# rust-bio/rust-bio

Measured on AMD Instinct MI355X. Metric: GCUPS (SW) + FM-index queries/sec, higher is better.
Workload: dtype int16; 1 GPU; 1000000 x 150 bp synthetic read pairs per GPU, Aligner::local affine-gap (-5,-1,+1,-1), score+coords+traceback ops (BASELINE configs[1]); pairs_per_gpu=1000000, read_len=150, parallelism=shard1

## Files before the change

include/biogpu.h:

```cpp
#ifndef BIOGPU_H
#define BIOGPU_H
#include <stdint.h>

#ifdef __cplusplus
extern "C" {
#endif

typedef enum {
    BG_OK = 0,
    BG_ERR_INVALID_ARG = -1,
    BG_ERR_NO_DEVICE = -2,
    BG_ERR_HIP = -3,
    BG_ERR_OOM = -4,
    BG_ERR_SENTINEL = -5,
    BG_ERR_POSITIVE_PENALTY = -6,
    BG_ERR_OUT_OF_ALPHABET = -7,
    BG_ERR_TOO_LARGE = -8,
    BG_ERR_OPS_CAP = -9,
    BG_ERR_TRACEBACK = -10,
    BG_ERR_UNSUPPORTED = -11,
    BG_ERR_IO = -12
} bg_status;

#define BG_MIN_SCORE (-858993459)
// ... 143 lines not shown
int bg_align_banded_batch(bg_ctx* ctx, const bg_scoring_t* sc, int mode, uint32_t k, uint32_t w,
                          uint64_t n_pairs, const uint8_t* x, const uint64_t* x_off,
                          const uint8_t* y, const uint64_t* y_off, bg_alignment_t* out,
                          uint8_t* ops_buf, uint64_t ops_cap, uint64_t* ops_used,
                          uint64_t* band_cells);

int bg_align_banded_batch_dev(bg_ctx* ctx, const bg_scoring_t* sc, int mode, uint32_t k, uint32_t w,
                              uint64_t n_pairs, const uint8_t* d_x, const uint64_t* d_x_off,
                              const uint8_t* d_y, const uint64_t* d_y_off, bg_alignment_t* d_out,
                              uint8_t* d_ops, uint64_t ops_stride, uint64_t* band_cells, void* stream);

int bg_band_create_batch(const bg_scoring_t* sc, int mode, uint32_t k, uint32_t w, uint64_t n_pairs,
                         const uint8_t* x, const uint64_t* x_off, const uint8_t* y, const uint64_t* y_off,
                         const uint64_t* band_off, uint32_t* start, uint32_t* end, uint64_t* band_cells);

int bg_align_banded_bands_batch(bg_ctx* ctx, const bg_scoring_t* sc, int mode, uint64_t n_pairs,
                                const uint8_t* x, const uint64_t* x_off, const uint8_t* y,
                                const uint64_t* y_off, const uint64_t* band_off,
                                const uint32_t* band_start, const uint32_t* band_end,
                                bg_alignment_t* out, uint8_t* ops_buf, uint64_t ops_cap,
                                uint64_t* ops_used, uint64_t* band_cells);

int bg_band_from_matches_batch(const bg_scoring_t* sc, int mode, uint32_t k, uint32_t w,
                               uint64_t n_pairs, const uint64_t* x_off, const uint64_t* y_off,
                               const uint32_t* matches_xy, const uint64_t* match_off,
                               const uint32_t* path, const uint64_t* path_off,
                               const uint64_t* band_off, uint32_t* start, uint32_t* end,
                               uint64_t* band_cells);

uint64_t bg_sparse_find_kmer_matches(const uint8_t* x, uint64_t m, const uint8_t* y, uint64_t n,
                                     uint32_t k, uint32_t* out_xy, uint64_t cap);
uint64_t bg_sparse_sdpkpp(const uint32_t* matches_xy, uint64_t n_matches, uint32_t k,
                          uint32_t match_score, int32_t gap_open, int32_t gap_extend,
                          uint32_t* path, uint64_t cap);
uint64_t bg_sparse_lcskpp(const uint32_t* matches_xy, uint64_t n_matches, uint32_t k, uint32_t* path,
                          uint64_t cap, uint32_t* score);
uint64_t bg_sparse_sdpkpp_union_lcskpp_path(const uint32_t* matches_xy, uint64_t n_matches, uint32_t k,
                                            uint32_t match_score, int32_t gap_open,
                                            int32_t gap_extend, uint32_t* path, uint64_t cap);
uint64_t bg_sparse_expand_kmer_matches(const uint8_t* x, uint64_t m, const uint8_t* y, uint64_t n,
                                       uint32_t k, const uint32_t* matches_xy, uint64_t n_matches,
                                       uint32_t allowed_mismatches, uint32_t* out_xy, uint64_t cap);

int bg_fm_set_text(bg_fm* fm, const uint8_t* text, uint64_t n);
int bg_fm_set_text_dev(bg_fm* fm, const uint8_t* d_text, uint64_t n);
typedef struct {
    uint32_t seed_len, stride;
    uint32_t max_occ;
    uint32_t pad;
} bg_seed_params_t;
typedef struct {
    bg_alignment_t aln;
    uint64_t window_start;
    uint64_t ref_start, ref_end;
    uint32_t n_candidates;
    uint32_t n_seed_hits;
} bg_seed_hit_t;
int bg_seed_extend_batch(bg_fm* fm, const bg_scoring_t* sc, const bg_seed_params_t* prm, uint64_t n_reads,
                         const uint8_t* reads, const uint64_t* read_off, bg_seed_hit_t* hits, uint8_t* ops_buf,
                         uint64_t ops_cap, uint64_t* ops_used);
int bg_seed_extend_batch_dev(bg_fm* fm, const bg_scoring_t* sc, const bg_seed_params_t* prm, uint64_t n_reads,
                             const uint8_t* d_reads, const uint64_t* d_read_off, uint32_t max_read_len,
                             bg_seed_hit_t* d_hits, uint8_t* d_ops, uint64_t ops_stride, uint64_t* totals,
                             void* stream);
enum { BG_STRAND_FORWARD = 1, BG_STRAND_REVERSE = 2, BG_STRAND_BOTH = 3 };
enum { BG_HIT_FORWARD = 0, BG_HIT_REVERSE = 1, BG_HIT_NONE = 255 };
int bg_seed_extend_strands_batch(bg_fm* fm, const bg_scoring_t* sc, const bg_seed_params_t* prm, uint32_t strands,
                                 uint64_t n_reads, const uint8_t* reads, const uint64_t* read_off, bg_seed_hit_t* hits,
                                 uint8_t* strand, uint8_t* ops_buf, uint64_t ops_cap, uint64_t* ops_used);
int bg_seed_extend_strands_batch_dev(bg_fm* fm, const bg_scoring_t* sc, const bg_seed_params_t* prm, uint32_t strands,
                                     uint64_t n_reads, const uint8_t* d_reads, const uint64_t* d_read_off,
                                     uint32_t max_read_len, bg_seed_hit_t* d_hits, uint8_t* d_strand, uint8_t* d_ops,
                                     uint64_t ops_stride, uint64_t* totals, void* stream);
typedef struct {
    uint32_t min_span, max_span;
    int32_t  pen_unpaired;
} bg_pair_params_t;
typedef struct {
    uint64_t span;
    uint32_t n_proper;
    uint8_t  proper;
    uint8_t  reserved[3];
} bg_pair_hit_t;
int bg_seed_extend_pairs_batch(bg_fm* fm, const bg_scoring_t* sc, const bg_seed_params_t* prm, const bg_pair_params_t* pp,
                               uint64_t n_pairs, const uint8_t* reads, const uint64_t* read_off, bg_seed_hit_t* hits,
                               uint8_t* strand, bg_pair_hit_t* pairs, uint8_t* ops_buf, uint64_t ops_cap, uint64_t* ops_used);
int bg_seed_extend_pairs_batch_dev(bg_fm* fm, const bg_scoring_t* sc, const bg_seed_params_t* prm, const bg_pair_params_t* pp,
                                   uint64_t n_pairs, const uint8_t* d_reads, const uint64_t* d_read_off, uint32_t max_read_len,
                                   bg_seed_hit_t* d_hits, uint8_t* d_strand, bg_pair_hit_t* d_pairs, uint8_t* d_ops,
                                   uint64_t ops_stride, uint64_t* totals, void* stream);
int bg_revcomp_batch_dev(bg_ctx* ctx, uint64_t n, const uint8_t* d_in, const uint64_t* d_off, uint8_t* d_out, void* stream);

enum { BG_FASTQ_OK = 0, BG_FASTQ_MISSING_AT = 1, BG_FASTQ_INCOMPLETE = 2, BG_FASTQ_IO = 3 };
enum { BG_FQCHECK_OK = 0, BG_FQCHECK_EMPTY_ID = 1, BG_FQCHECK_NONASCII_SEQ = 2, BG_FQCHECK_INVALID_SEQ = 3,
       BG_FQCHECK_NONASCII_QUAL = 4, BG_FQCHECK_UNEQUAL = 5 };
typedef struct {
    uint64_t id_off, desc_off;
    uint64_t seq_off, qual_off;
    uint32_t id_len, desc_len, seq_len, qual_len;
    int32_t has_desc;
    int32_t check;
} bg_fastq_record_t;
int bg_fastq_parse(bg_ctx* ctx, const uint8_t* text, uint64_t len, bg_fastq_record_t* recs, uint64_t rec_cap,
                   uint8_t* seq, uint64_t* seq_off, uint8_t* qual, uint64_t* qual_off, uint64_t* n_records,
                   int32_t* status, uint64_t* err_pos);
int bg_fastq_parse_dev(bg_ctx* ctx, const uint8_t* d_text, uint64_t len, bg_fastq_record_t* d_recs,
                       uint64_t rec_cap, uint8_t* d_seq, uint64_t* d_seq_off, uint8_t* d_qual,
                       uint64_t* d_qual_off, uint64_t* n_records, int32_t* status, uint64_t* err_pos,
                       void* stream);
int bg_cigar_batch(bg_ctx* ctx, uint64_t n, const bg_alignment_t* aln, const uint8_t* ops, uint64_t ops_bytes,
                   int hard_clip, char* out, uint64_t out_cap, uint64_t* out_off);
int bg_cigar_batch_dev(bg_ctx* ctx, uint64_t n, const bg_alignment_t* d_aln, const uint8_t* d_ops, int hard_clip,
                       char* d_out, uint64_t stride, int32_t* d_len, void* stream);

int bg_pretty_batch(bg_ctx* ctx, uint64_t n, const bg_alignment_t* aln, const uint8_t* ops, uint64_t ops_bytes,
                    const uint8_t* x, const uint64_t* x_off, const uint8_t* y, const uint64_t* y_off, uint32_t ncol,
                    char* out, uint64_t out_cap, uint64_t* out_off);

#define BG_COMM_ID_BYTES 128
typedef struct bg_comm bg_comm;
int bg_shard_range(uint64_t n_units, int rank, int world, uint64_t* lo, uint64_t* hi);
int bg_shard_balanced(const uint64_t* costs, uint64_t n, int world, uint64_t* bounds);
int bg_comm_unique_id(uint8_t* id );
int bg_comm_init(bg_ctx* ctx, int rank, int world, const uint8_t* id , bg_comm** out);
int bg_comm_init_host(bg_ctx* ctx, int rank, int world, const char* name, bg_comm** out);
int bg_gather_records(bg_comm* comm, const void* local, uint64_t n_local, uint32_t rec_bytes, void* all, uint64_t* counts_out,
                      void* stream);
int bg_gather_records_cap(bg_comm* comm, const void* local, uint64_t n_local, uint32_t rec_bytes, void* all, uint64_t all_cap,
                          uint64_t* counts_out, void* stream);
int bg_gather_records_host(bg_comm* comm, const void* local, uint64_t n_local, uint32_t rec_bytes, void* all, uint64_t all_cap,
                           uint64_t* counts_out);
int bg_comm_world(bg_comm* comm, int64_t* info);
int bg_comm_free(bg_comm* comm);

typedef struct {
    float fill_ms, traceback_ms, fm_ms;
    uint32_t fill_launches, traceback_launches, fm_launches;
} bg_timing_t;
int bg_get_timing(bg_ctx* ctx, bg_timing_t* out);
int bg_band_redo_pairs(bg_ctx* ctx, uint64_t* out);
enum {
    BG_FILL_K1_WIDE = 0x1,
    BG_FILL_K1_NARROW = 0x2,
    BG_FILL_K1_LF = 0x4,
    BG_FILL_K1P = 0x8,
    BG_FILL_K1P_LF = 0x10,
    BG_FILL_K3 = 0x20,
    BG_FILL_K3V2_WIDE = 0x40,
    BG_FILL_K3V2_NARROW = 0x80,
    BG_FILL_K3I = 0x100,
    BG_FILL_K3P = 0x200
};
int bg_last_fill_kernels(bg_ctx* ctx, uint32_t* mask);
int bg_enable_timing(bg_ctx* ctx, int on);

#ifdef __cplusplus
}
#endif
#endif
```

rust-bio_amd/_lib.py:

```python
import ctypes as C
import os
import subprocess

import numpy as np

_HERE = os.path.dirname(os.path.abspath(__file__))
SO_PATH = os.path.join(_HERE, "libbiogpu.so")
CSRC = os.path.join(_HERE, "csrc")

BG_OK = 0
ERRORS = {-1: "INVALID_ARG", -2: "NO_DEVICE", -3: "HIP", -4: "OOM", -5: "SENTINEL",
          -6: "POSITIVE_PENALTY", -7: "OUT_OF_ALPHABET", -8: "TOO_LARGE", -9: "OPS_CAP",
          -10: "TRACEBACK", -11: "UNSUPPORTED", -12: "IO"}
MIN_SCORE = -858993459
STRAND_FORWARD, STRAND_REVERSE, STRAND_BOTH = 1, 2, 3
HIT_FORWARD, HIT_REVERSE, HIT_NONE = 0, 1, 255
FILL = {"K1_WIDE": 0x1, "K1_NARROW": 0x2, "K1_LF": 0x4, "K1P": 0x8, "K1P_LF": 0x10, "K3": 0x20, "K3V2_WIDE": 0x40,
        "K3V2_NARROW": 0x80, "K3I": 0x100, "K3P": 0x200}


class BiogpuError(RuntimeError):
    def __init__(self, status, where=""):
        self.status = status
        msg = lib().bg_strerror(status).decode()
        last = lib().bg_last_error().decode()
        super().__init__(f"{where}: {ERRORS.get(status, status)}: {msg}" + (f" [{last}]" if last else ""))


class SentinelError(BiogpuError, ValueError):
    """suffix_array.rs:431-437 assert"""


class PenaltyError(BiogpuError, AssertionError):
    """pairwise/mod.rs:265-266,554-571 asserts"""


class AlphabetError(BiogpuError, IndexError):
    """fmindex.rs:229 / bwt.rs:158 index out of bounds"""


_EXC = {-5: SentinelError, -6: PenaltyError, -7: AlphabetError}


def check(status, where=""):
    if status != BG_OK:
        raise _EXC.get(status, BiogpuError)(status, where)


class ScoringC(C.Structure):
    _fields_ = [("gap_open", C.c_int32), ("gap_extend", C.c_int32),
                ("xclip_prefix", C.c_int32), ("xclip_suffix", C.c_int32),
                ("yclip_prefix", C.c_int32), ("yclip_suffix", C.c_int32),
                ("match_score", C.c_int32), ("mismatch_score", C.c_int32),
                ("match_scores_some", C.c_int32),
                ("matrix", C.POINTER(C.c_int32))]


class TimingC(C.Structure):
    _fields_ = [("fill_ms", C.c_float), ("traceback_ms", C.c_float), ("fm_ms", C.c_float),
                ("fill_launches", C.c_uint32), ("traceback_launches", C.c_uint32),
                ("fm_launches", C.c_uint32)]


ALN_DTYPE = np.dtype([("score", "<i4"), ("xstart", "<u4"), ("xend", "<u4"), ("ystart", "<u4"),
                      ("yend", "<u4"), ("xlen", "<u4"), ("ylen", "<u4"), ("n_ops", "<u4"),
                      ("ops_off", "<u8"), ("clip_len", "<u4", (4,)), ("n_clips", "u1"),
                      ("mode", "u1"), ("status", "i1"), ("_pad", "u1"), ("_tail", "<u4")])
assert ALN_DTYPE.itemsize == 64, ALN_DTYPE.itemsize
SEED_HIT_DTYPE = np.dtype([("aln", ALN_DTYPE), ("window_start", "<u8"), ("ref_start", "<u8"), ("ref_end", "<u8"),
                           ("n_candidates", "<u4"), ("n_seed_hits", "<u4")])
assert SEED_HIT_DTYPE.itemsize == 96, SEED_HIT_DTYPE.itemsize


class SeedParamsC(C.Structure):
    _fields_ = [("seed_len", C.c_uint32), ("stride", C.c_uint32), ("max_occ", C.c_uint32), ("pad", C.c_uint32)]


class PAIR_PARAMS(C.Structure):
    _fields_ = [("min_span", C.c_uint32), ("max_span", C.c_uint32), ("pen_unpaired", C.c_int32)]


assert C.sizeof(PAIR_PARAMS) == 12, C.sizeof(PAIR_PARAMS)
PAIR_HIT_DTYPE = np.dtype([("span", "<u8"), ("n_proper", "<u4"), ("proper", "u1"), ("reserved", "u1", (3,))])
assert PAIR_HIT_DTYPE.itemsize == 16, PAIR_HIT_DTYPE.itemsize


FQREC_DTYPE = np.dtype([("id_off", "<u8"), ("desc_off", "<u8"), ("seq_off", "<u8"), ("qual_off", "<u8"),
                        ("id_len", "<u4"), ("desc_len", "<u4"), ("seq_len", "<u4"), ("qual_len", "<u4"),
                        ("has_desc", "<i4"), ("check", "<i4")])
assert FQREC_DTYPE.itemsize == 56, FQREC_DTYPE.itemsize

SYMBOLS = ["bg_device_count", "bg_init", "bg_free", "bg_strerror", "bg_last_error",
           "bg_set_option", "bg_suffix_array", "bg_bwt", "bg_less", "bg_fm_build", "bg_fm_free",
           "bg_fm_device_bytes", "bg_fm_set_option", "bg_fm_backward_search_batch", "bg_fm_backward_search_batch_dev",
           "bg_fm_set_suffix_array", "bg_fm_set_sampled_suffix_array", "bg_sa_get_batch", "bg_sa_get_batch_dev",
           "bg_interval_occ_batch", "bg_interval_occ_batch_dev", "bg_fmd_smems_batch", "bg_fmd_smems_batch_dev", "bg_fmd_interval_batch",
           "bg_align_batch", "bg_align_batch_dev", "bg_align_banded_batch", "bg_align_banded_batch_dev", "bg_band_create_batch",
           "bg_align_banded_bands_batch", "bg_band_from_matches_batch", "bg_sparse_find_kmer_matches", "bg_sparse_sdpkpp",
           "bg_sparse_lcskpp", "bg_sparse_sdpkpp_union_lcskpp_path", "bg_sparse_expand_kmer_matches", "bg_fastq_parse",
           "bg_fastq_parse_dev", "bg_cigar_batch", "bg_cigar_batch_dev", "bg_get_timing", "bg_enable_timing", "bg_band_redo_pairs", "bg_last_fill_kernels", "bg_pack2_host",
           "bg_pretty_batch", "bg_suffix_array_dev", "bg_bwt_dev", "bg_sa_sample_dev", "bg_suffix_array_dev64", "bg_bwt_dev64", "bg_sa_sample_dev64", "bg_fm_build_dev", "bg_fm_set_text", "bg_fm_set_text_dev", "bg_seed_extend_batch", "bg_seed_extend_batch_dev",
           "bg_seed_extend_strands_batch", "bg_seed_extend_strands_batch_dev", "bg_revcomp_batch_dev",
           "bg_seed_extend_pairs_batch", "bg_seed_extend_pairs_batch_dev",
           "bg_pack2_dev", "bg_unpack2_dev", "bg_fm_pattern_codes", "bg_fm_backward_search_packed_dev",
           "bg_fm_backward_search_count_lines_dev", "bg_align_batch_packed_dev", "bg_fm_step2_bytes",
           "bg_shard_range", "bg_shard_balanced", "bg_comm_unique_id", "bg_comm_init", "bg_comm_init_host",
           "bg_gather_records", "bg_gather_records_cap", "bg_gather_records_host", "bg_comm_free", "bg_fm_save", "bg_fm_load",
           "bg_fm_len", "bg_fm_less", "bg_fm_bwt", "bg_fm_bwt_dev", "bg_comm_world",
           "bg_fmd_smems_batch64", "bg_fmd_smems_batch64_dev", "bg_fmd_interval_batch64"]


def build(force=False):
    if force:
        subprocess.check_call(["make", "-C", CSRC, "clean", "-s"])
    subprocess.check_call(["make", "-C", CSRC, "-j8", "-s"])
    return SO_PATH


_lib = None


def lib():
    global _lib
    if _lib is None:
        if not os.path.exists(SO_PATH):
            raise RuntimeError(f"{SO_PATH} is missing: run `python -c 'import __graft_entry__ as g; "
                               "g.build()'` (the engine has no CPU fallback)")
        L = C.CDLL(SO_PATH)
        vp, u64, u32, i32 = C.c_void_p, C.c_uint64, C.c_uint32, C.c_int
        L.bg_strerror.restype = C.c_char_p
        L.bg_strerror.argtypes = [i32]
        L.bg_last_error.restype = C.c_char_p
        L.bg_device_count.restype = i32
        L.bg_init.argtypes = [i32, C.POINTER(vp)]
        L.bg_free.argtypes = [vp]
        L.bg_set_option.argtypes = [vp, C.c_char_p, C.c_int64]
        L.bg_suffix_array.argtypes = [vp, u64, vp]
        L.bg_bwt.argtypes = [vp, vp, u64, vp]
        L.bg_less.argtypes = [vp, u64, vp, u32, vp, C.POINTER(u32)]
        L.bg_fm_build.argtypes = [vp, vp, u64, vp, u32, u32, vp, u32, C.POINTER(vp)]
        L.bg_fm_free.argtypes = [vp]
        L.bg_fm_save.argtypes = [vp, C.c_char_p]
        L.bg_fm_load.argtypes = [vp, C.c_char_p, C.POINTER(vp)]
        L.bg_fm_len.argtypes = [vp, C.POINTER(u64)]
        L.bg_fm_less.argtypes = [vp, vp, C.POINTER(u32)]
        L.bg_fm_bwt.argtypes = [vp, vp]
        L.bg_fm_bwt_dev.argtypes = [vp, vp, vp]
        L.bg_fm_build_dev.argtypes = [vp, vp, u64, u32, vp, u32, vp, C.POINTER(vp), vp]
        L.bg_fm_set_option.argtypes = [vp, C.c_char_p, C.c_int64]
        L.bg_fm_device_bytes.restype = u64
        L.bg_fm_device_bytes.argtypes = [vp]
        L.bg_fm_step2_bytes.restype = u64
        L.bg_fm_step2_bytes.argtypes = [vp]
        L.bg_shard_range.argtypes = [u64, i32, i32, C.POINTER(u64), C.POINTER(u64)]
        L.bg_shard_balanced.argtypes = [vp, u64, i32, vp]
        L.bg_comm_unique_id.argtypes = [vp]
        L.bg_comm_init.argtypes = [vp, i32, i32, vp, C.POINTER(vp)]
        L.bg_comm_init_host.argtypes = [vp, i32, i32, C.c_char_p, C.POINTER(vp)]
        L.bg_gather_records.argtypes = [vp, vp, u64, u32, vp, vp, vp]
        L.bg_gather_records_cap.argtypes = [vp, vp, u64, u32, vp, u64, vp, vp]
        L.bg_gather_records_host.argtypes = [vp, vp, u64, u32, vp, u64, vp]
        L.bg_comm_free.argtypes = [vp]
        L.bg_comm_world.argtypes = [vp, vp]
        L.bg_fm_backward_search_batch.argtypes = [vp, u64, vp, vp, vp, vp, vp, vp]
        L.bg_fm_backward_search_batch_dev.argtypes = [vp, u64, vp, vp, vp, vp, vp, vp, vp]
        L.bg_fmd_interval_batch.argtypes = [vp, u64, vp, vp, vp, vp]
        L.bg_fmd_smems_batch.argtypes = [vp, i32, u64, vp, vp, vp, u32, u32, vp, vp]
        L.bg_fmd_smems_batch_dev.argtypes = [vp, i32, u64, vp, vp, vp, u32, u32, u32, vp, vp, vp]
        L.bg_fmd_interval_batch64.argtypes = [vp, u64, vp, vp, vp, vp]
        L.bg_fmd_smems_batch64.argtypes = [vp, i32, u64, vp, vp, vp, u32, u32, vp, vp]
        L.bg_fmd_smems_batch64_dev.argtypes = [vp, i32, u64, vp, vp, vp, u32, u32, u32, vp, vp, vp]
        L.bg_fm_set_suffix_array.argtypes = [vp, vp, u64]
        L.bg_fm_set_sampled_suffix_array.argtypes = [vp, vp, u64, u32, C.c_uint8, vp, vp, u64]
        L.bg_sa_get_batch.argtypes = [vp, u64, vp, vp]
        L.bg_fastq_parse.argtypes = [vp, vp, u64, vp, u64, vp, vp, vp, vp, C.POINTER(u64), C.POINTER(i32), C.POINTER(u64)]
        L.bg_fastq_parse_dev.argtypes = [vp, vp, u64, vp, u64, vp, vp, vp, vp, C.POINTER(u64), C.POINTER(i32), C.POINTER(u64), vp]
        L.bg_cigar_batch.argtypes = [vp, u64, vp, vp, u64, i32, vp, u64, vp]
        L.bg_cigar_batch_dev.argtypes = [vp, u64, vp, vp, i32, vp, u64, vp, vp]
        L.bg_sa_get_batch_dev.argtypes = [vp, u64, vp, vp, vp]
        L.bg_interval_occ_batch.argtypes = [vp, u64, vp, vp, vp, vp, u64]
        L.bg_interval_occ_batch_dev.argtypes = [vp, u64, vp, vp, u64, vp, vp]
        L.bg_align_batch.argtypes = [vp, C.POINTER(ScoringC), i32, u64, vp, vp, vp, vp, vp, vp,
                                     u64, C.POINTER(u64)]
        L.bg_align_batch_dev.argtypes = [vp, C.POINTER(ScoringC), i32, u64, vp, vp, vp, vp, u32,
                                         u32, vp, vp, u64, vp]
        L.bg_align_banded_batch.argtypes = [vp, C.POINTER(ScoringC), i32, u32, u32, u64, vp, vp,
                                            vp, vp, vp, vp, u64, C.POINTER(u64), vp]
        L.bg_align_banded_batch_dev.argtypes = [vp, C.POINTER(ScoringC), i32, u32, u32, u64, vp, vp, vp, vp, vp, vp, u64, vp, vp]
        L.bg_band_create_batch.argtypes = [C.POINTER(ScoringC), i32, u32, u32, u64, vp, vp, vp, vp, vp, vp, vp, vp]
        L.bg_align_banded_bands_batch.argtypes = [vp, C.POINTER(ScoringC), i32, u64, vp, vp, vp, vp, vp, vp, vp, vp, vp,
                                                  u64, C.POINTER(u64), vp]
        L.bg_band_from_matches_batch.argtypes = [C.POINTER(ScoringC), i32, u32, u32, u64, vp, vp, vp, vp, vp, vp, vp, vp,
                                                 vp, vp]
        for name, args in [("bg_sparse_find_kmer_matches", [vp, u64, vp, u64, u32, vp, u64]),
                           ("bg_sparse_sdpkpp", [vp, u64, u32, u32, C.c_int32, C.c_int32, vp, u64]),
                           ("bg_sparse_lcskpp", [vp, u64, u32, vp, u64, C.POINTER(u32)]),
                           ("bg_sparse_sdpkpp_union_lcskpp_path", [vp, u64, u32, u32, C.c_int32, C.c_int32, vp, u64]),
                           ("bg_sparse_expand_kmer_matches", [vp, u64, vp, u64, u32, vp, u64, u32, vp, u64])]:
            getattr(L, name).restype = u64
            getattr(L, name).argtypes = args
        L.bg_pretty_batch.argtypes = [vp, u64, vp, vp, u64, vp, vp, vp, vp, u32, vp, u64, vp]
        L.bg_suffix_array_dev.argtypes = [vp, vp, u64, vp, vp]
        L.bg_bwt_dev.argtypes = [vp, vp, vp, u64, vp, vp]
        L.bg_sa_sample_dev.argtypes = [vp, vp, vp, u64, u32, C.c_uint8, vp, vp, vp, u64, C.POINTER(u64), vp]
        L.bg_suffix_array_dev64.argtypes = [vp, vp, u64, vp, vp]
        L.bg_bwt_dev64.argtypes = [vp, vp, vp, u64, vp, vp]
        L.bg_sa_sample_dev64.argtypes = [vp, vp, vp, u64, u32, C.c_uint8, vp, vp, vp, u64, C.POINTER(u64), vp]
        L.bg_fm_set_text.argtypes = [vp, vp, u64]
        L.bg_fm_set_text_dev.argtypes = [vp, vp, u64]
        L.bg_seed_extend_batch.argtypes = [vp, C.POINTER(ScoringC), C.POINTER(SeedParamsC), u64, vp, vp, vp, vp, u64, C.POINTER(u64)]
        L.bg_seed_extend_batch_dev.argtypes = [vp, C.POINTER(ScoringC), C.POINTER(SeedParamsC), u64, vp, vp, u32, vp, vp, u64, vp, vp]
        L.bg_seed_extend_strands_batch.argtypes = [vp, C.POINTER(ScoringC), C.POINTER(SeedParamsC), u32, u64, vp, vp, vp, vp, vp, u64,
                                                   C.POINTER(u64)]
        L.bg_seed_extend_strands_batch_dev.argtypes = [vp, C.POINTER(ScoringC), C.POINTER(SeedParamsC), u32, u64, vp, vp, u32, vp, vp,
                                                       vp, u64, vp, vp]
        L.bg_seed_extend_pairs_batch.argtypes = [vp, C.POINTER(ScoringC), C.POINTER(SeedParamsC), C.POINTER(PAIR_PARAMS), u64, vp, vp, vp,
                                                 vp, vp, vp, u64, C.POINTER(u64)]
        L.bg_seed_extend_pairs_batch_dev.argtypes = [vp, C.POINTER(ScoringC), C.POINTER(SeedParamsC), C.POINTER(PAIR_PARAMS), u64, vp, vp,
                                                     u32, vp, vp, vp, vp, u64, vp, vp]
        L.bg_revcomp_batch_dev.argtypes = [vp, u64, vp, vp, vp, vp]
        L.bg_pack2_dev.argtypes = [vp, vp, u64, vp, vp, vp, vp]
        L.bg_unpack2_dev.argtypes = [vp, vp, u64, vp, vp, vp]
        L.bg_fm_pattern_codes.argtypes = [vp, vp]
        L.bg_fm_backward_search_packed_dev.argtypes = [vp, u64, vp, vp, vp, vp, vp, vp, vp]
        L.bg_fm_backward_search_count_lines_dev.argtypes = [vp, u64, vp, vp, vp, vp, vp, vp, C.POINTER(u64), vp]
        L.bg_align_batch_packed_dev.argtypes = [vp, C.POINTER(ScoringC), i32, u64, vp, vp, vp, vp, vp, u32, u32, vp, vp, u64, vp]
        L.bg_get_timing.argtypes = [vp, C.POINTER(TimingC)]
        L.bg_enable_timing.argtypes = [vp, i32]
        L.bg_band_redo_pairs.argtypes = [vp, C.POINTER(u64)]
        L.bg_last_fill_kernels.argtypes = [vp, C.POINTER(u32)]
        L.bg_pack2_host.argtypes = [vp, u64, vp, vp]
        for s in SYMBOLS:
            if getattr(L, s).restype is C.c_int or s.startswith("bg_") and getattr(L, s).restype is None:
                pass
        _lib = L
    return _lib


class Context:

    def __init__(self, device=0):
        self.h = C.c_void_p()
        check(lib().bg_init(device, C.byref(self.h)), "bg_init")
        self.device = device

    def set_option(self, key, value):
        check(lib().bg_set_option(self.h, key.encode(), int(value)), "bg_set_option")

    def enable_timing(self, on=True):
        check(lib().bg_enable_timing(self.h, 1 if on else 0))

    def timing(self):
        t = TimingC()
        check(lib().bg_get_timing(self.h, C.byref(t)))
        return {k: getattr(t, k) for k, _ in TimingC._fields_}

    def band_redo_pairs(self):
        v = C.c_uint64(0)
        check(lib().bg_band_redo_pairs(self.h, C.byref(v)))
        return int(v.value)

    def last_fill_kernels(self):
        v = C.c_uint32(0)
        check(lib().bg_last_fill_kernels(self.h, C.byref(v)))
        return int(v.value)

    def close(self):
        if self.h:
            lib().bg_free(self.h)
            self.h = C.c_void_p()

    def __del__(self):
        try:
            self.close()
        except Exception:
            pass


_default_ctx = {}


def default_context(device=None):
    if device is None:
        device = int(os.environ.get("LOCAL_RANK", "0")) if lib().bg_device_count() > 1 else 0
    if device not in _default_ctx:
        _default_ctx[device] = Context(device)
    return _default_ctx[device]


def as_u8(b):
    if isinstance(b, np.ndarray):
        return np.ascontiguousarray(b, dtype=np.uint8)
    return np.frombuffer(bytes(b), dtype=np.uint8)


def concat(seqs):
    off = np.zeros(len(seqs) + 1, dtype=np.uint64)
    if seqs:
        off[1:] = np.cumsum([len(s) for s in seqs], dtype=np.uint64)
    buf = np.frombuffer(b"".join(bytes(s) for s in seqs), dtype=np.uint8)
    return buf, off
```

rust-bio_amd/csrc/banded_api.hip:

```cpp
#include <algorithm>
#include <atomic>
#include <functional>
#include <thread>

#include "band_host.h"
#include <sched.h>

#include <chrono>

#include "band_device.h"
#include "banded_kernels.h"

using namespace bgband_dev;

int bg_compact_matrix(const int32_t* matrix, std::vector<uint8_t>& code_map, std::vector<int32_t>& table);

namespace bgband { extern std::atomic<uint64_t> g_prof[4]; }
namespace {

constexpr uint64_t kMaxCells = 5000000;

struct HostPair {
    uint32_t m = 0, n = 0, flags = BP_OK;
    uint32_t start_0 = 0, end_0 = 0, start_n = 0, end_n = 0;
// ... 107 lines not shown
        size_t dc_pairs = 0, dc_rowc = 0, dc_roff = 0, dc_tb = 0, dc_aux = 0;
        hipEvent_t copied = nullptr, filled = nullptr, traced = nullptr, built = nullptr, matched = nullptr;
        bool built_valid = false;
        hipEvent_t fill_gone = nullptr;
        hipEvent_t pre_done = nullptr;
        hipEvent_t cleared = nullptr;
        bool busy = false;
    } set[2];
    void* db[2][17] = {};
    size_t db_cap[2][17] = {};
    hipStream_t build_stream = nullptr;
    hipEvent_t seq_ready = nullptr;
    void* h_state = nullptr;
    size_t h_state_cap = 0;
    void* io[6] = {};
    size_t io_cap[6] = {};
    void* h_ops = nullptr;
    size_t h_ops_cap = 0;
    void *d_cmp = nullptr, *d_cscan = nullptr;
    size_t d_cmp_cap = 0, d_cscan_cap = 0;
    uint64_t* d_cell = nullptr;
    uint64_t* d_dlslot = nullptr;
    hipStream_t dl_stream = nullptr;
    static constexpr uint64_t kDlSlots = 1024;
    hipStream_t tb_stream = nullptr;
    hipStream_t aux_stream = nullptr;
    hipStream_t copy_stream = nullptr;
    uint32_t* d_started = nullptr;
    uint32_t started_target = 0;
};

extern "C" int bg_band_redo_pairs(bg_ctx* ctx, uint64_t* out) {
    if (!ctx || !out) return BG_ERR_INVALID_ARG;
    *out = 0;
    if (!ctx->band || !ctx->band->d_started) return BG_OK;
    BG_HIP(hipSetDevice(ctx->device));
    BG_HIP(hipDeviceSynchronize());
    uint32_t v = 0;
    BG_HIP(hipMemcpy(&v, ctx->band->d_started + 1, 4, hipMemcpyDeviceToHost));
    *out = v;
    return BG_OK;
}

void bg_band_scratch_free(bg_band_scratch* b) {
    if (!b) return;
    for (auto& s : b->set) {
        hipHostFree(s.h_pairs); hipHostFree(s.h_rowc); hipHostFree(s.h_roff);
        hipFree(s.d_pairs); hipFree(s.d_rowc); hipFree(s.d_roff); hipFree(s.d_tb); hipFree(s.d_aux);
        hipFree(b->d_started);
        b->d_started = nullptr;
        if (s.copied) hipEventDestroy(s.copied);
        if (s.filled) hipEventDestroy(s.filled);
        if (s.traced) hipEventDestroy(s.traced);
        if (s.built) hipEventDestroy(s.built);
        if (s.matched) hipEventDestroy(s.matched);
        if (s.fill_gone) hipEventDestroy(s.fill_gone);
        if (s.pre_done) hipEventDestroy(s.pre_done);
        if (s.cleared) hipEventDestroy(s.cleared);
    }
    for (void* p : b->io) hipFree(p);
    hipFree(b->d_cmp);
    hipFree(b->d_cscan);
    hipFree(b->d_cell);
    hipFree(b->d_dlslot);
    if (b->dl_stream) hipStreamDestroy(b->dl_stream);
    for (auto& set : b->db)
        for (void* p : set) hipFree(p);
    hipHostFree(b->h_state);
    hipHostFree(b->h_ops);
    if (b->tb_stream) hipStreamDestroy(b->tb_stream);
    if (b->aux_stream) hipStreamDestroy(b->aux_stream);
    if (b->copy_stream) hipStreamDestroy(b->copy_stream);
    if (b->build_stream) hipStreamDestroy(b->build_stream);
    if (b->seq_ready) hipEventDestroy(b->seq_ready);
    delete b;
}

namespace {

template <typename F>
void parallel_for(uint64_t n, uint64_t grain, F&& fn) {
    unsigned nt = host_threads();
    nt = (unsigned)std::min<uint64_t>(nt, std::max<uint64_t>(1, n / grain));
    if (nt <= 1) {
        fn(0, 0, n);
        return;
    }
    std::atomic<uint64_t> next{0};
    bg_pool_run(nt, [&](unsigned t) {
        for (;;) {
            const uint64_t lo = next.fetch_add(grain);
            if (lo >= n) break;
            fn(t, lo, std::min<uint64_t>(n, lo + grain));
        }
    });
}

int check_scoring(const bg_scoring_t* sc) {
    if (sc->gap_open > 0 || sc->gap_extend > 0 || sc->xclip_prefix > 0 || sc->xclip_suffix > 0 ||
        sc->yclip_prefix > 0 || sc->yclip_suffix > 0)
        return BG_ERR_POSITIVE_PENALTY;
    return BG_OK;
}

}

extern "C" int bg_band_create_batch(const bg_scoring_t* sc, int mode, uint32_t k, uint32_t w, uint64_t n_pairs,
                                    const uint8_t* x, const uint64_t* x_off, const uint8_t* y, const uint64_t* y_off,
                                    const uint64_t* band_off, uint32_t* start, uint32_t* end, uint64_t* band_cells) {
    if (!sc || !x_off || !y_off || (n_pairs && (!band_off || !start || !end))) return BG_ERR_INVALID_ARG;
    int rc = check_scoring(sc);
    if (rc) return rc;
    const bgband::ClipScores cs = clip_scores(sc, mode);
    parallel_for(n_pairs, 4, [&](unsigned, uint64_t lo, uint64_t hi) {
        bgband::Band band;
        bgband::Workspace ws;
        for (uint64_t p = lo; p < hi; p++) {
            const uint32_t m = (uint32_t)(x_off[p + 1] - x_off[p]), n = (uint32_t)(y_off[p + 1] - y_off[p]);
            band.create(x + x_off[p], m, y + y_off[p], n, k, w, cs, ws);
            memcpy(start + band_off[p], band.start.data(), (size_t)(n + 1) * 4);
            memcpy(end + band_off[p], band.end.data(), (size_t)(n + 1) * 4);
            if (band_cells) band_cells[p] = band.num_cells();
        }
    });
    if (getenv("BG_TRACE")) fprintf(stderr, "[bg banded] cpu-ms: kmers %.1f sdp %.1f band %.1f (threads %u)\n", bgband::g_prof[0] / 1e6, bgband::g_prof[1] / 1e6, bgband::g_prof[2] / 1e6, host_threads());
    return BG_OK;
}

using BandMaker = std::function<bool(uint64_t, bgband::Band&, bgband::Workspace&)>;

int band_stream_create(hipStream_t* s, int level) {
    int lo = 0, hi = 0;
    if (level == 0 || hipDeviceGetStreamPriorityRange(&lo, &hi) != hipSuccess || lo == hi)
        return hipStreamCreateWithFlags(s, hipStreamNonBlocking) == hipSuccess ? BG_OK : BG_ERR_HIP;
    return hipStreamCreateWithPriority(s, hipStreamNonBlocking, level > 0 ? hi : lo) == hipSuccess ? BG_OK : BG_ERR_HIP;
}

struct BandDevIO {
    const uint8_t* d_x;
    const uint64_t* d_xo;
    const uint8_t* d_y;
    const uint64_t* d_yo;
    bg_alignment_t* d_out;
    uint8_t* d_ops;
    uint64_t ops_stride;
};

static int banded_batch_impl(bg_ctx* ctx, const bg_scoring_t* sc, int mode, uint64_t n_pairs, const uint8_t* x,
                             const uint64_t* x_off, const uint8_t* y, const uint64_t* y_off, bg_alignment_t* out,
                             uint8_t* ops_buf, uint64_t ops_cap, uint64_t* ops_used, uint64_t* band_cells,
                             const BandMaker& make_band, const uint32_t* dev_kw = nullptr, const BandDevIO* dio = nullptr) {
    if (!ctx || !sc || mode < BG_MODE_CUSTOM || mode > BG_MODE_LOCAL) return BG_ERR_INVALID_ARG;
    ctx->fill_mask = 0;
    int rc = check_scoring(sc);
    if (rc) return rc;
    if (ops_used) *ops_used = 0;
    if (n_pairs == 0) return BG_OK;
    if (!x_off || !y_off || (!out && !dio)) return BG_ERR_INVALID_ARG;
    BG_HIP(hipSetDevice(ctx->device));
    hipStream_t st = ctx->stream;
    if (!ctx->band) {
        ctx->band = new bg_band_scratch;
        BG_HIP(hipStreamCreateWithFlags(&ctx->band->tb_stream, hipStreamNonBlocking));
        for (auto& s : ctx->band->set) {
            BG_HIP(hipEventCreateWithFlags(&s.copied, hipEventDisableTiming));
            BG_HIP(hipEventCreateWithFlags(&s.filled, hipEventDisableTiming));
            BG_HIP(hipEventCreateWithFlags(&s.traced, hipEventDisableTiming));
        }
    }
    bg_band_scratch& B = *ctx->band;
    hipStream_t st_tb = B.tb_stream;

    const bgband::ClipScores cs = clip_scores(sc, mode);
    uint64_t max_x = 0, max_y = 0;
    for (uint64_t p = 0; p < n_pairs; p++) {
        max_x = std::max(max_x, x_off[p + 1] - x_off[p]);
        max_y = std::max(max_y, y_off[p + 1] - y_off[p]);
    }
    if (max_x > (1u << 24) || max_y > (1u << 24)) return BG_ERR_TOO_LARGE;
    const uint64_t stride = dio ? dio->ops_stride : ((max_x + max_y + 4 + 3) & ~3ull);
    if (dio && dio->d_ops && stride < max_x + max_y + 4) return BG_ERR_OPS_CAP;

    BandArgs a = {};
    a.sc = {cs.gap_open, cs.gap_extend, cs.xclip_prefix, cs.xclip_suffix, cs.yclip_prefix, cs.yclip_suffix,
            sc->match_score, sc->mismatch_score};
    a.mode = mode;
    a.filter_clips = (mode == BG_MODE_SEMIGLOBAL || mode == BG_MODE_LOCAL);
    a.ops_stride = stride;
    int sm = SCORE_PARAMS;
    std::vector<uint8_t> code_map;
    std::vector<int32_t> table;
    if (sc->matrix) {
        const int A = bg_compact_matrix(sc->matrix, code_map, table);
        sm = A <= kMaxLdsAlphabet ? SCORE_LDS : SCORE_GLOBAL;
        if ((rc = bg_reserve(&ctx->table, &ctx->table_bytes, 256 + table.size() * 4))) return rc;
        BG_HIP(hipMemcpy((uint8_t*)ctx->table + 256, table.data(), table.size() * 4, hipMemcpyHostToDevice));
        BG_HIP(hipMemcpy(ctx->table, code_map.data(), 256, hipMemcpyHostToDevice));
        a.code_map = (const uint8_t*)ctx->table;
        a.table = (const int32_t*)((uint8_t*)ctx->table + 256);
        a.alpha = A;
    }
    band_fill_fn fill = get_band_fill(sm);
    const int64_t mag = std::max<int64_t>({std::abs((int64_t)cs.gap_open), std::abs((int64_t)cs.gap_extend),
                                           std::abs((int64_t)sc->match_score), std::abs((int64_t)sc->mismatch_score), 1});
    auto clip_ok = [](int32_t c) { return c <= kNarrowNegClip || c >= -(1 << 22); };
    const bool narrow = !ctx->force_wide && mag * ((int64_t)max_x + (int64_t)max_y + 8) < (1 << 24) && clip_ok(cs.xclip_prefix) &&
                        clip_ok(cs.xclip_suffix) && clip_ok(cs.yclip_prefix) && clip_ok(cs.yclip_suffix);

    const bool trace = getenv("BG_TRACE") != nullptr;
    auto now = []() { return std::chrono::steady_clock::now(); };
    auto t_last = now();
    auto lap = [&](const char* what) {
        if (!trace) return;
        const auto t1 = now();
        fprintf(stderr, "[bg banded] %-18s %8.2f ms\n", what, std::chrono::duration<double, std::milli>(t1 - t_last).count());
        t_last = t1;
    };

    const uint64_t xb = x_off[n_pairs], yb = y_off[n_pairs];
    const uint8_t *d_x, *d_y;
    const uint64_t *d_xo, *d_yo;
    uint8_t* d_ops;
    bg_alignment_t* d_out;
    if (dio) {
        d_x = dio->d_x;
        d_y = dio->d_y;
        d_xo = dio->d_xo;
        d_yo = dio->d_yo;
        d_out = dio->d_out;
        d_ops = dio->d_ops;
    } else {
        const size_t io_need[6] = {std::max<uint64_t>(xb, 16), std::max<uint64_t>(yb, 16), (n_pairs + 1) * 8, (n_pairs + 1) * 8,
                                   n_pairs * sizeof(bg_alignment_t), ops_buf ? n_pairs * stride : 16};
        for (int i = 0; i < 6; i++)
            if ((rc = bg_reserve(&B.io[i], &B.io_cap[i], io_need[i]))) return rc;
        d_x = (uint8_t*)B.io[0];
        d_y = (uint8_t*)B.io[1];
        d_ops = ops_buf ? (uint8_t*)B.io[5] : nullptr;
        d_xo = (uint64_t*)B.io[2];
        d_yo = (uint64_t*)B.io[3];
        d_out = (bg_alignment_t*)B.io[4];
        BG_HIP(hipMemcpyAsync((void*)d_xo, x_off, (n_pairs + 1) * 8, hipMemcpyHostToDevice, st));
        BG_HIP(hipMemcpyAsync((void*)d_yo, y_off, (n_pairs + 1) * 8, hipMemcpyHostToDevice, st));
    }
    a.x = d_x;
    a.x_off = d_xo;
    a.y = d_y;
    a.y_off = d_yo;
    a.out = d_out;
    a.ops = d_ops;
    lap("h2d sequences");
    const bool compact_on_device = !dio && ops_buf != nullptr;
    if (compact_on_device) {
        if ((rc = bg_reserve(&B.d_cmp, &B.d_cmp_cap, xb + yb + 4 * n_pairs + 256))) return rc;
        if ((rc = bg_reserve(&B.d_cscan, &B.d_cscan_cap,
                             bg_compact_ops_scratch(std::min<uint64_t>(n_pairs, ctx->chunk_pairs > 0 ? (uint64_t)ctx->chunk_pairs : 16384)))))
            return rc;
        if (!B.d_cell) BG_HIP(hipMalloc((void**)&B.d_cell, 64));
        BG_HIP(hipMemsetAsync(B.d_cell, 0, 8, st));
        if ((rc = pinned_reserve(&B.h_ops, &B.h_ops_cap, xb + yb + 4 * n_pairs + 256))) return rc;
        if (!B.d_dlslot) BG_HIP(hipMalloc((void**)&B.d_dlslot, bg_band_scratch::kDlSlots * 16));
        if (!B.dl_stream) {
            int lo = 0, hi = 0;
            BG_HIP(hipDeviceGetStreamPriorityRange(&lo, &hi));
            BG_HIP(hipStreamCreateWithPriority(&B.dl_stream, hipStreamNonBlocking, hi));
        }
    }

    const uint64_t chunk_pairs = ctx->chunk_pairs > 0 ? (uint64_t)ctx->chunk_pairs : 16384;
    struct SliceEvents {
        std::vector<hipEvent_t> ev;
        ~SliceEvents() {
            for (hipEvent_t e : ev)
                if (e) hipEventDestroy(e);
        }
    } slices;
    const uint64_t n_slices = dio ? 0 : (n_pairs + chunk_pairs - 1) / chunk_pairs;
    uint64_t slices_up = 0, waited_fill = 0;
    if (n_slices && !B.copy_stream && (rc = band_stream_create(&B.copy_stream, -1))) return rc;
    auto upload_slices = [&](uint64_t upto) -> int {
        for (; slices_up < std::min(upto, n_slices); slices_up++) {
            const uint64_t q0 = slices_up * chunk_pairs, q1 = std::min(n_pairs, q0 + chunk_pairs);
            if (slices_up == 0) {
                hipEvent_t e0;
                BG_HIP(hipEventCreateWithFlags(&e0, hipEventDisableTiming));
                slices.ev.push_back(e0);
                BG_HIP(hipEventRecord(e0, st));
                BG_HIP(hipStreamWaitEvent(B.copy_stream, e0, 0));
            }
            if (x_off[q1] > x_off[q0])
                BG_HIP(bg_copy_pieces((uint8_t*)d_x + x_off[q0], x + x_off[q0], x_off[q1] - x_off[q0], hipMemcpyHostToDevice, B.copy_stream));
            if (y_off[q1] > y_off[q0])
                BG_HIP(bg_copy_pieces((uint8_t*)d_y + y_off[q0], y + y_off[q0], y_off[q1] - y_off[q0], hipMemcpyHostToDevice, B.copy_stream));
            hipEvent_t e;
            BG_HIP(hipEventCreateWithFlags(&e, hipEventDisableTiming));
            slices.ev.push_back(e);
            BG_HIP(hipEventRecord(e, B.copy_stream));
        }
        return BG_OK;
    };
    auto need_seq = [&](hipStream_t s, uint64_t& waited, uint64_t upto) -> int {
        if (!n_slices) return BG_OK;
        const uint64_t k1 = std::min(n_slices, (upto + chunk_pairs - 1) / chunk_pairs);
        int rcu = upload_slices(k1);
        if (rcu) return rcu;
        for (; waited < k1; waited++) BG_HIP(hipStreamWaitEvent(s, slices.ev[waited + 1], 0));
// ... 589 lines not shown
```

rust-bio_amd/csrc/bg_common.h:

```cpp
#ifndef BG_COMMON_H
#define BG_COMMON_H
#include <functional>
#include <hip/hip_runtime.h>

#include <cstdint>
#include <cstdlib>
#include <cstdio>
#include <cstring>
#include <string>
#include <vector>

#include "biogpu.h"

extern thread_local std::string bg_tls_error;

#define BG_HIP(call)                                                                     \
    do {                                                                                 \
        hipError_t e__ = (call);                                                         \
        if (e__ != hipSuccess) {                                                         \
            bg_tls_error = std::string(#call) + ": " + hipGetErrorString(e__);           \
            return e__ == hipErrorOutOfMemory ? BG_ERR_OOM : BG_ERR_HIP;                 \
        }                                                                                \
    } while (0)

struct bg_band_scratch;
void bg_band_scratch_free(bg_band_scratch*);
struct bg_seed_scratch;
void bg_seed_scratch_free(bg_seed_scratch*);
struct bg_host_pipe;
void bg_host_pipe_free(bg_host_pipe*);
struct bg_fm_pipe;
void bg_fm_pipe_free(bg_fm_pipe*);

struct bg_ctx {
    int device = 0;
    hipStream_t stream = nullptr;
    void* tb = nullptr;
    size_t tb_bytes = 0;
    void* aux = nullptr;
    size_t aux_bytes = 0;
    void* bnd = nullptr;
    size_t bnd_bytes = 0;
    void* io[6] = {};
    size_t io_cap[6] = {};
    void* h_ops = nullptr;
    size_t h_ops_cap = 0;
    void* unpk[2] = {};
    size_t unpk_cap[2] = {};
    void* table = nullptr;
    size_t table_bytes = 0;
    void* sw_table = nullptr;
    size_t sw_table_bytes = 0;
    uint64_t table_hash = 0;
    int table_alpha = 0;
    int32_t* table_matrix = nullptr;
    bg_band_scratch* band = nullptr;
    bg_host_pipe* pipe = nullptr;
    bg_seed_scratch* seed = nullptr;
    bg_fm_pipe* fm_pipe = nullptr;
    uint64_t fm_wide_from = 0xFFFFFFFFull;
    uint32_t fm_wide_sb_shift = 17;
    bool fm_host_bytes = false;
    int64_t host_chunk_pairs = 0;
    int64_t chunk_pairs = 0;
    int64_t seed_chunk_reads = 0;
    bool force_wide = false;
    bool no_pk16 = false;
    bool no_local_fast = false;
    bool no_couples = false;
    int band_chain_global = -1;
    bool fq_no_fused = false;
    int64_t sa_chunk_symbols = 0;
    bool band_chain_rows = true;
    bool band_join_global = false;
    int band_fill_v1 = 0;
    bool band_interior_off = false;
    bool band_packed_off = false;
    int64_t band_packed_thresh = 0;
    int64_t band_budget_gb = 0;
    bool band_on_host = false;
    hipEvent_t scratch_done = nullptr;
    hipStream_t scratch_stream = nullptr;
    bool scratch_used = false;
    bool timing = false;
    hipEvent_t ev[2] = {nullptr, nullptr};
    bg_timing_t last = {};
    uint32_t fill_mask = 0;
};

int bg_reserve(void** p, size_t* cur, size_t need);
int bg_scan_u32(const uint32_t* d_len, uint64_t n, uint64_t* d_off, uint64_t* d_sums, hipStream_t st);
int bg_align_batch_dev_hint(bg_ctx* ctx, const bg_scoring_t* sc, int mode, uint64_t n_pairs, const uint8_t* d_x,
                            const uint64_t* d_x_off, const uint8_t* d_y, const uint64_t* d_y_off, uint32_t max_xlen,
                            uint32_t max_ylen, bg_alignment_t* d_out, uint8_t* d_ops, uint64_t ops_stride, void* stream,
                            int len_hint);

size_t bg_compact_ops_scratch(uint64_t n);
int bg_range_to_host(const uint8_t* d_src, uint8_t* h_dst, const uint64_t* d_slot , hipStream_t st);
int bg_compact_ops_dev(bg_alignment_t* d_rec, uint64_t n, const uint8_t* d_ops, uint8_t* d_compact, bool global_offsets, uint64_t* d_cell,
                       uint64_t* d_batch_total, void* d_scratch, bool long_ops, hipStream_t st);

struct bg_scratch_guard {
    bg_ctx* ctx;
    hipStream_t st;
    bg_scratch_guard(bg_ctx* c, hipStream_t s) : ctx(c), st(s) {
        if (ctx->scratch_used && ctx->scratch_stream != st) hipStreamWaitEvent(st, ctx->scratch_done, 0);
    }
    ~bg_scratch_guard() {
        if (hipEventRecord(ctx->scratch_done, st) == hipSuccess) {
            ctx->scratch_stream = st;
            ctx->scratch_used = true;
        }
    }
};
inline hipError_t bg_copy_pieces(void* dst, const void* src, size_t bytes, hipMemcpyKind kind, hipStream_t st) {
    static const size_t piece = [] {
        const char* e = getenv("BG_COPY_PIECE");
        const long long v = e ? atoll(e) : 0;
        return v > 0 ? (size_t)v : (size_t)(8u << 20);
    }();
    for (size_t o = 0; o < bytes; o += piece) {
        const hipError_t rc = hipMemcpyAsync((uint8_t*)dst + o, (const uint8_t*)src + o, bytes - o < piece ? bytes - o : piece, kind, st);
        if (rc != hipSuccess) return rc;
    }
    return hipSuccess;
}
unsigned bg_host_threads();
namespace bgpack {
bool pack2_host(const uint8_t* src, uint64_t n, const uint8_t codes[4], uint32_t* dst);
}
void bg_pool_run(unsigned nt, const std::function<void(unsigned)>& fn);

__device__ __forceinline__ int wave_shr1(int v, int old = 0) {
    return __builtin_amdgcn_update_dpp(old, v, 0x138 , 0xf, 0xf, false);
}
__device__ __forceinline__ int wave_shl1(int v, int old = 0) {
    return __builtin_amdgcn_update_dpp(old, v, 0x130 , 0xf, 0xf, false);
}
__device__ __forceinline__ int wave_shr1z(int v) { return __builtin_amdgcn_update_dpp(0, v, 0x138, 0xf, 0xf, true); }
__device__ __forceinline__ int wave_shl1z(int v) { return __builtin_amdgcn_update_dpp(0, v, 0x130, 0xf, 0xf, true); }
__device__ __forceinline__ unsigned quad_sum(unsigned v) {
    v += (unsigned)__builtin_amdgcn_update_dpp(0, (int)v, 0xB1 , 0xf, 0xf, true);
    v += (unsigned)__builtin_amdgcn_update_dpp(0, (int)v, 0x4E , 0xf, 0xf, true);
    return v;
}

#endif
```

rust-bio_amd/csrc/core.hip:

```cpp
#include <sched.h>

#include <algorithm>
#include <condition_variable>
#include <deque>
#include <mutex>
#include <thread>

#include <cstdlib>

#include "bg_common.h"

thread_local std::string bg_tls_error;

int bg_reserve(void** p, size_t* cur, size_t need) {
    if (need <= *cur) return BG_OK;
    if (*p) {
        hipFree(*p);
        *p = nullptr;
        *cur = 0;
    }
    need = (need + 255) & ~(size_t)255;
    BG_HIP(hipMalloc(p, need));
    *cur = need;
    return BG_OK;
// ... 85 lines not shown
    hipDeviceProp_t prop;
    BG_HIP(hipGetDeviceProperties(&prop, device));
    if (std::string(prop.gcnArchName).rfind("gfx950", 0) != 0) {
        bg_tls_error = std::string("device is ") + prop.gcnArchName + ", library is built for gfx950";
        return BG_ERR_NO_DEVICE;
    }
    bg_ctx* ctx = new bg_ctx;
    ctx->device = device;
    if (const char* e = getenv("BG_BAND_FILL_V1")) ctx->band_fill_v1 = atoi(e) > 0 ? 1 : atoi(e) < 0 ? -1 : 0;
    {
        int lo = 0, hi = 0;
        const char* e = getenv("BG_STREAM_PRIO");
        if ((!e || atoi(e) != 0) && hipDeviceGetStreamPriorityRange(&lo, &hi) == hipSuccess && hi != lo)
            BG_HIP(hipStreamCreateWithPriority(&ctx->stream, hipStreamNonBlocking, hi));
        else
            BG_HIP(hipStreamCreateWithFlags(&ctx->stream, hipStreamNonBlocking));
    }
    BG_HIP(hipEventCreate(&ctx->ev[0]));
    BG_HIP(hipEventCreate(&ctx->ev[1]));
    BG_HIP(hipEventCreateWithFlags(&ctx->scratch_done, hipEventDisableTiming));
    *out = ctx;
    return BG_OK;
}

extern "C" int bg_free(bg_ctx* ctx) {
    if (!ctx) return BG_OK;
    hipSetDevice(ctx->device);
    hipFree(ctx->tb);
    hipFree(ctx->aux);
    hipFree(ctx->bnd);
    hipFree(ctx->table);
    hipFree(ctx->sw_table);
    free(ctx->table_matrix);
    hipFree(ctx->unpk[0]);
    hipFree(ctx->unpk[1]);
    for (void* p : ctx->io) hipFree(p);
    if (ctx->h_ops) hipHostFree(ctx->h_ops);
    bg_band_scratch_free(ctx->band);
    bg_host_pipe_free(ctx->pipe);
    bg_seed_scratch_free(ctx->seed);
    bg_fm_pipe_free(ctx->fm_pipe);
    if (ctx->ev[0]) hipEventDestroy(ctx->ev[0]);
    if (ctx->ev[1]) hipEventDestroy(ctx->ev[1]);
    if (ctx->scratch_done) hipEventDestroy(ctx->scratch_done);
    if (ctx->stream) hipStreamDestroy(ctx->stream);
    delete ctx;
    return BG_OK;
}

extern "C" const char* bg_strerror(int s) {
    switch (s) {
        case BG_OK: return "ok";
        case BG_ERR_INVALID_ARG: return "invalid argument";
        case BG_ERR_NO_DEVICE: return "no usable gfx950 device";
        case BG_ERR_HIP: return "HIP runtime error";
        case BG_ERR_OOM: return "out of device memory";
        case BG_ERR_SENTINEL:
            return "Expecting extra sentinel symbol being lexicographically smallest at the end of the text.";
        case BG_ERR_POSITIVE_PENALTY: return "gap/clip penalty can't be positive";
        case BG_ERR_OUT_OF_ALPHABET: return "symbol outside the alphabet (index out of bounds in the reference)";
        case BG_ERR_TOO_LARGE: return "input too large for the engine";
        case BG_ERR_OPS_CAP: return "operations buffer too small";
        case BG_ERR_TRACEBACK: return "traceback did not terminate";
        case BG_ERR_UNSUPPORTED: return "not supported by the device layout";
        case BG_ERR_IO: return "index file cannot be opened, is truncated or fails its checksum";
        default: return "unknown status";
    }
}

extern "C" const char* bg_last_error(void) { return bg_tls_error.c_str(); }

extern "C" int bg_set_option(bg_ctx* ctx, const char* key, int64_t value) {
    if (!ctx || !key) return BG_ERR_INVALID_ARG;
    if (!strcmp(key, "chunk_pairs")) {
        ctx->chunk_pairs = value;
        return BG_OK;
    }
    if (!strcmp(key, "seed_chunk_reads")) {
        ctx->seed_chunk_reads = value;
        return BG_OK;
    }
    if (!strcmp(key, "band_join_global")) {
        ctx->band_join_global = value != 0;
        return BG_OK;
    }
    if (!strcmp(key, "fm_wide_from")) {
        ctx->fm_wide_from = value > 0 ? (uint64_t)value : 0xFFFFFFFFull;
        return BG_OK;
    }
    if (!strcmp(key, "fm_wide_sb_shift")) {
        if (value < 0 || value > 24) return BG_ERR_INVALID_ARG;
        ctx->fm_wide_sb_shift = (uint32_t)value;
        return BG_OK;
    }
    if (!strcmp(key, "fq_no_fused")) {
        ctx->fq_no_fused = value != 0;
        return BG_OK;
    }
    if (!strcmp(key, "sa_chunk_symbols")) {
        if (value < 0) return BG_ERR_INVALID_ARG;
        ctx->sa_chunk_symbols = value;
        return BG_OK;
    }
    if (!strcmp(key, "band_chain_rows")) {
        ctx->band_chain_rows = value != 0;
        return BG_OK;
    }
    if (!strcmp(key, "band_chain_global")) {
        ctx->band_chain_global = (int)value;
        return BG_OK;
    }
    if (!strcmp(key, "band_fill_v1")) {
        ctx->band_fill_v1 = value > 0 ? 1 : value < 0 ? -1 : 0;
        return BG_OK;
    }
    if (!strcmp(key, "band_interior_off")) {
        ctx->band_interior_off = value != 0;
        return BG_OK;
    }
    if (!strcmp(key, "band_packed_off")) {
        ctx->band_packed_off = value != 0;
        return BG_OK;
    }
    if (!strcmp(key, "band_packed_thresh")) {
        if (value < 0 || value > 0xffff) return BG_ERR_INVALID_ARG;
        ctx->band_packed_thresh = value;
        return BG_OK;
    }
    if (!strcmp(key, "band_budget_gb")) {
        if (value < 0 || value > 256) return BG_ERR_INVALID_ARG;
        ctx->band_budget_gb = value;
        return BG_OK;
    }
    if (!strcmp(key, "band_on_host")) {
        ctx->band_on_host = value != 0;
        return BG_OK;
    }
    if (!strcmp(key, "fm_host_bytes")) {
        ctx->fm_host_bytes = value != 0;
        return BG_OK;
    }
    if (!strcmp(key, "host_chunk_pairs")) {
        ctx->host_chunk_pairs = value;
        return BG_OK;
    }
    if (!strcmp(key, "no_couples")) {
        ctx->no_couples = value != 0;
        return BG_OK;
    }
    if (!strcmp(key, "no_local_fast")) {
        ctx->no_local_fast = value != 0;
        return BG_OK;
    }
    if (!strcmp(key, "no_pk16")) {
        ctx->no_pk16 = value != 0;
        return BG_OK;
    }
    if (!strcmp(key, "force_wide")) {
        ctx->force_wide = value != 0;
        return BG_OK;
    }
    return BG_ERR_INVALID_ARG;
}

extern "C" int bg_enable_timing(bg_ctx* ctx, int on) {
    if (!ctx) return BG_ERR_INVALID_ARG;
    ctx->timing = on != 0;
    ctx->last = {};
    return BG_OK;
}

extern "C" int bg_last_fill_kernels(bg_ctx* ctx, uint32_t* mask) {
    if (!ctx || !mask) return BG_ERR_INVALID_ARG;
    *mask = ctx->fill_mask;
    return BG_OK;
}

extern "C" int bg_get_timing(bg_ctx* ctx, bg_timing_t* out) {
    if (!ctx || !out) return BG_ERR_INVALID_ARG;
    *out = ctx->last;
    ctx->last = {};
    return BG_OK;
}

namespace {
__global__ __launch_bounds__(256) void ops_counts_kernel(const bg_alignment_t* __restrict__ rec, uint64_t n, uint32_t* __restrict__ cnt) {
    const uint64_t p = (uint64_t)blockIdx.x * blockDim.x + threadIdx.x;
    if (p < n) cnt[p] = rec[p].status == BG_OK ? rec[p].n_ops : 0u;
}
template <int LANES>
__global__ __launch_bounds__(256) void ops_compact_kernel(bg_alignment_t* __restrict__ rec, uint64_t n, const uint8_t* __restrict__ ops,
                                                          const uint64_t* __restrict__ off, const uint64_t* __restrict__ cell,
                                                          uint8_t* __restrict__ compact, int global_offsets) {
    const uint64_t p = ((uint64_t)blockIdx.x * blockDim.x + threadIdx.x) / LANES;
    const uint32_t l = threadIdx.x % LANES;
    if (p >= n) return;
    const uint32_t k = rec[p].status == BG_OK ? rec[p].n_ops : 0u;
    const uint64_t base = *cell;
    const uint8_t* src = ops + rec[p].ops_off;
    uint8_t* dst = compact + (global_offsets ? base : 0ull) + off[p];
    for (uint32_t i = l; i < k; i += LANES) dst[i] = src[i];
    if (l == 0) rec[p].ops_off = base + off[p];
}
__global__ void ops_advance_kernel(uint64_t* cell, const uint64_t* __restrict__ off, uint64_t n, uint64_t* __restrict__ batch_total) {
    if (batch_total) *batch_total = off[n];
    cell[0] += off[n];
}
inline size_t a256(size_t v) { return (v + 255) & ~(size_t)255; }
}

typedef uint32_t bg_u32x4 __attribute__((ext_vector_type(4)));
__global__ __launch_bounds__(256) void range_to_host_kernel(const uint8_t* __restrict__ d_src, uint8_t* __restrict__ h_dst,
                                                            const uint64_t* __restrict__ slot) {
    const uint64_t end = slot[1], start = end - slot[0];
    const uint64_t a = start >> 4, b = (end + 15) >> 4;
    const bg_u32x4* src = (const bg_u32x4*)d_src;
    bg_u32x4* dst = (bg_u32x4*)h_dst;
    for (uint64_t i = a + (uint64_t)blockIdx.x * 256 + threadIdx.x; i < b; i += (uint64_t)gridDim.x * 256)
        __builtin_nontemporal_store(src[i], &dst[i]);
}
int bg_range_to_host(const uint8_t* d_src, uint8_t* h_dst, const uint64_t* d_slot, hipStream_t st) {
    range_to_host_kernel<<<dim3(8), dim3(256), 0, st>>>(d_src, h_dst, d_slot);
    BG_HIP(hipGetLastError());
    return BG_OK;
}

size_t bg_compact_ops_scratch(uint64_t n) { return a256(n * 4) + a256((n + 1) * 8) + 2 * (n / 2048 + 2) * 8 + 256; }

int bg_compact_ops_dev(bg_alignment_t* d_rec, uint64_t n, const uint8_t* d_ops, uint8_t* d_compact, bool global_offsets, uint64_t* d_cell,
                       uint64_t* d_batch_total, void* d_scratch, bool long_ops, hipStream_t st) {
    if (n == 0) {
        if (d_batch_total) BG_HIP(hipMemsetAsync(d_batch_total, 0, 8, st));
        return BG_OK;
    }
    uint32_t* d_cnt = (uint32_t*)d_scratch;
    uint64_t* d_off = (uint64_t*)((uint8_t*)d_scratch + a256(n * 4));
    uint64_t* d_sums = (uint64_t*)((uint8_t*)d_off + a256((n + 1) * 8));
    ops_counts_kernel<<<dim3((unsigned)((n + 255) / 256)), dim3(256), 0, st>>>(d_rec, n, d_cnt);
    int rc = bg_scan_u32(d_cnt, n, d_off, d_sums, st);
    if (rc) return rc;
    if (long_ops)
        ops_compact_kernel<64><<<dim3((unsigned)((n * 64 + 255) / 256)), dim3(256), 0, st>>>(d_rec, n, d_ops, d_off, d_cell, d_compact, global_offsets);
    else
        ops_compact_kernel<16><<<dim3((unsigned)((n * 16 + 255) / 256)), dim3(256), 0, st>>>(d_rec, n, d_ops, d_off, d_cell, d_compact, global_offsets);
    ops_advance_kernel<<<dim3(1), dim3(1), 0, st>>>(d_cell, d_off, n, d_batch_total);
    BG_HIP(hipGetLastError());
    return BG_OK;
}
```

rust-bio_amd/csrc/sw_api.hip:

```cpp
#include <algorithm>
#include <chrono>
#include <map>
#include <type_traits>

#include <atomic>
#include <condition_variable>
#include <mutex>
#include <thread>

#include "sw_kernels.h"

namespace bgsw {
sw_fill_fn get_fill_params_narrow(int lp, int r, bool local);
sw_fill_fn get_fill_params_wide(int lp, int r, bool local);
sw_fill_fn get_fill_params_lf(int lp, int r);
sw_fill_fn get_fill_matrix(int lp, int r, int sm, bool narrow, bool local);
sw_fill_fn get_fill_pk16_local(int lp, int r, int which);
sw_fill_fn get_fill_pk16_localfast(int lp, int r, int which);
sw_fill_fn get_fill_pk16_semiglobal(int lp, int r, int which);
sw_fill_fn get_fill_pk16_global(int lp, int r, int which);
sw_fill_fn get_fill_pk16_custom(int lp, int r, int which);
void launch_traceback(const SwArgs& a, int nw, hipStream_t st);

struct Config {
    int lp, r;
};
static Config pick_config(uint32_t m_cap, int sm) {
    if (sm == SCORE_PARAMS) {
        if (m_cap <= 192) return {16, std::max(2, 2 * (int)((m_cap + 31) / 32))};
        if (m_cap <= 384) return {32, std::max(8, 2 * (int)((m_cap + 63) / 64))};
        return {64, 8};
    }
    if (m_cap <= 96) return {16, 6};
    if (m_cap <= 128) return {16, 8};
    if (m_cap <= 160) return {16, 10};
    if (m_cap <= 192) return {16, 12};
    if (m_cap <= 384) return {32, 12};
    return {64, 8};
}

static int compact_matrix(const int32_t* matrix, std::vector<uint8_t>& code_map,
                          std::vector<int32_t>& table) {
    std::map<std::vector<int32_t>, int> classes;
    code_map.assign(256, 0);
    std::vector<int> rep;
    for (int b = 0; b < 256; b++) {
        std::vector<int32_t> sig(512);
        for (int c = 0; c < 256; c++) {
            sig[c] = matrix[b * 256 + c];
            sig[256 + c] = matrix[c * 256 + b];
        }
        auto it = classes.find(sig);
        if (it == classes.end()) {
            it = classes.emplace(std::move(sig), (int)rep.size()).first;
            rep.push_back(b);
        }
        code_map[b] = (uint8_t)it->second;
    }
    const int A = (int)rep.size();
    table.assign((size_t)A * A, 0);
    for (int p = 0; p < A; p++)
        for (int q = 0; q < A; q++) table[(size_t)p * A + q] = matrix[rep[p] * 256 + rep[q]];
    return A;
}
}

namespace bgsw {
constexpr uint32_t kLenKeys = 1u << 20;
__global__ __launch_bounds__(256) void sw_len_stats_kernel(const uint64_t* __restrict__ x_off, const uint64_t* __restrict__ y_off, uint64_t pair0,
                                                           uint32_t n, uint32_t* __restrict__ st ) {
    uint32_t m = 0, nn = 0, m_lo = ~0u, n_lo = ~0u;
    for (uint32_t p = blockIdx.x * blockDim.x + threadIdx.x; p < n; p += gridDim.x * blockDim.x) {
        const uint32_t a = (uint32_t)(x_off[pair0 + p + 1] - x_off[pair0 + p]), b = (uint32_t)(y_off[pair0 + p + 1] - y_off[pair0 + p]);
        m = max(m, a);
        m_lo = min(m_lo, a);
        nn = max(nn, b);
        n_lo = min(n_lo, b);
    }
#pragma unroll
    for (int o = 32; o; o >>= 1) {
        m = max(m, (uint32_t)__shfl_xor((int)m, o));
        nn = max(nn, (uint32_t)__shfl_xor((int)nn, o));
        m_lo = min(m_lo, (uint32_t)__shfl_xor((int)m_lo, o));
        n_lo = min(n_lo, (uint32_t)__shfl_xor((int)n_lo, o));
    }
    __shared__ uint32_t s[4][4];
    if ((threadIdx.x & 63) == 0) {
        s[threadIdx.x >> 6][0] = m_lo;
        s[threadIdx.x >> 6][1] = m;
        s[threadIdx.x >> 6][2] = n_lo;
        s[threadIdx.x >> 6][3] = nn;
    }
    __syncthreads();
    if (threadIdx.x == 0) {
        atomicMin(&st[0], min(min(s[0][0], s[1][0]), min(s[2][0], s[3][0])));
        atomicMax(&st[2], max(max(s[0][1], s[1][1]), max(s[2][1], s[3][1])));
        atomicMin(&st[1], min(min(s[0][2], s[1][2]), min(s[2][2], s[3][2])));
        atomicMax(&st[3], max(max(s[0][3], s[1][3]), max(s[2][3], s[3][3])));
    }
}
__device__ __forceinline__ uint32_t len_key(const uint64_t* x_off, const uint64_t* y_off, uint64_t r) {
    const uint32_t m = (uint32_t)(x_off[r + 1] - x_off[r]), n = (uint32_t)(y_off[r + 1] - y_off[r]);
    return min(m, 511u) << 11 | min(n, 2047u);
}
__device__ __forceinline__ uint32_t wave_key_add(uint32_t* counter, uint32_t key, bool valid, uint32_t& base) {
    const int lane = threadIdx.x & 63;
    uint32_t rank = 0;
    base = 0;
    uint64_t todo = __ballot(valid);
    while (todo) {
        const int leader = __ffsll((long long)todo) - 1;
        const uint32_t k = (uint32_t)__shfl((int)key, leader);
        const uint64_t same = __ballot(valid && key == k) & todo;
        uint32_t b = 0;
        if (lane == leader) b = atomicAdd(&counter[k], (uint32_t)__popcll(same));
        b = (uint32_t)__shfl((int)b, leader);
        if (valid && key == k) {
            base = b;
            rank = (uint32_t)__popcll(same & ((1ull << lane) - 1));
        }
        todo &= ~same;
    }
    return rank;
}
__global__ __launch_bounds__(256) void sw_key_hist_kernel(const uint64_t* __restrict__ x_off, const uint64_t* __restrict__ y_off, uint64_t pair0,
                                                          uint32_t n, uint32_t* __restrict__ cnt, const uint32_t* __restrict__ st) {
    if (st && st[0] == st[2] && st[1] == st[3]) return;
    const uint32_t p = blockIdx.x * blockDim.x + threadIdx.x;
    const bool valid = p < n;
    uint32_t base;
    wave_key_add(cnt, valid ? len_key(x_off, y_off, pair0 + p) : 0u, valid, base);
}
__global__ __launch_bounds__(256) void sw_key_block_sums_kernel(const uint32_t* __restrict__ cnt, uint32_t* __restrict__ sums,
                                                                const uint32_t* __restrict__ st) {
    if (st && st[0] == st[2] && st[1] == st[3]) return;
    uint32_t v = 0;
    for (int i = 0; i < 4; i++) v += cnt[blockIdx.x * 1024u + i * 256u + threadIdx.x];
    __shared__ uint32_t s[4];
#pragma unroll
    for (int o = 32; o; o >>= 1) v += __shfl_xor(v, o);
    if ((threadIdx.x & 63) == 0) s[threadIdx.x >> 6] = v;
    __syncthreads();
    if (threadIdx.x == 0) sums[blockIdx.x] = s[0] + s[1] + s[2] + s[3];
}
__global__ __launch_bounds__(1024) void sw_key_scan_kernel(uint32_t* __restrict__ cnt, const uint32_t* __restrict__ sums,
                                                           const uint32_t* __restrict__ st) {
    if (st && st[0] == st[2] && st[1] == st[3]) return;
    __shared__ uint32_t s[1024];
    s[threadIdx.x] = sums[threadIdx.x];
    __syncthreads();
    for (int o = 1; o < 1024; o <<= 1) {
        const uint32_t u = threadIdx.x >= (unsigned)o ? s[threadIdx.x - o] : 0;
        __syncthreads();
        s[threadIdx.x] += u;
        __syncthreads();
    }
    const uint32_t base = blockIdx.x ? s[blockIdx.x - 1] : 0;
    __syncthreads();
    const uint32_t v = cnt[blockIdx.x * 1024u + threadIdx.x];
    s[threadIdx.x] = v;
    __syncthreads();
    for (int o = 1; o < 1024; o <<= 1) {
        const uint32_t u = threadIdx.x >= (unsigned)o ? s[threadIdx.x - o] : 0;
        __syncthreads();
        s[threadIdx.x] += u;
        __syncthreads();
    }
    cnt[blockIdx.x * 1024u + threadIdx.x] = base + s[threadIdx.x] - v;
}
__global__ __launch_bounds__(256) void sw_key_scatter_kernel(const uint64_t* __restrict__ x_off, const uint64_t* __restrict__ y_off, uint64_t pair0,
                                                             uint32_t n, uint32_t* __restrict__ cursor, uint32_t* __restrict__ perm,
                                                             const uint32_t* __restrict__ st) {
    if (st && st[0] == st[2] && st[1] == st[3]) return;
    const uint32_t p = blockIdx.x * blockDim.x + threadIdx.x;
    const bool valid = p < n;
    uint32_t base;
    const uint32_t rank = wave_key_add(cursor, valid ? len_key(x_off, y_off, pair0 + p) : 0u, valid, base);
    if (valid) perm[base + rank] = p;
}
__global__ void sw_decide_kernel(const uint32_t* __restrict__ st, uint32_t n, int forced, uint32_t* __restrict__ n_eff) {
    const bool uniform = forced < 0 && st[0] == st[2] && st[1] == st[3];
    n_eff[0] = uniform ? n : 0u;
    n_eff[1] = uniform ? 0u : n;
}
}

using namespace bgsw;

int bg_compact_matrix(const int32_t* matrix, std::vector<uint8_t>& code_map, std::vector<int32_t>& table) {
    return compact_matrix(matrix, code_map, table);
}

static int check_scoring(const bg_scoring_t* sc) {
    if (sc->gap_open > 0 || sc->gap_extend > 0 || sc->xclip_prefix > 0 || sc->xclip_suffix > 0 ||
        sc->yclip_prefix > 0 || sc->yclip_suffix > 0)
        return BG_ERR_POSITIVE_PENALTY;
    return BG_OK;
}

static int align_batch_dev_impl(bg_ctx* ctx, const bg_scoring_t* sc, int mode, uint64_t n_pairs,
                                const uint8_t* d_x, const uint64_t* d_x_off, const uint8_t* d_y,
                                const uint64_t* d_y_off, uint32_t max_xlen, uint32_t max_ylen,
                                bg_alignment_t* d_out, uint8_t* d_ops, uint64_t ops_stride,
                                void* stream, int len_hint, const uint8_t* packed_codes = nullptr) {
    if (!ctx || !sc || mode < BG_MODE_CUSTOM || mode > BG_MODE_LOCAL) return BG_ERR_INVALID_ARG;
    int rc = check_scoring(sc);
    if (rc) return rc;
    if (n_pairs == 0) return BG_OK;
    if (!d_x_off || !d_y_off || !d_out) return BG_ERR_INVALID_ARG;
    if (d_ops && ops_stride < (uint64_t)max_xlen + max_ylen + 4) return BG_ERR_OPS_CAP;
    if (max_xlen > (1u << 24) || max_ylen > (1u << 24)) return BG_ERR_TOO_LARGE;
    hipStream_t st = (hipStream_t)stream;
    BG_HIP(hipSetDevice(ctx->device));
    bg_scratch_guard guard(ctx, st);

    SwArgs a = {};
    a.x = d_x;
    a.x_off = d_x_off;
    a.y = d_y;
    a.y_off = d_y_off;
    a.sc = {sc->gap_open,     sc->gap_extend,   sc->xclip_prefix, sc->xclip_suffix,
            sc->yclip_prefix, sc->yclip_suffix, sc->match_score,  sc->mismatch_score};
    if (mode == BG_MODE_GLOBAL) a.sc.xp = a.sc.xs = a.sc.yp = a.sc.ys = BG_MIN_SCORE;
    if (mode == BG_MODE_SEMIGLOBAL) {
        a.sc.xp = a.sc.xs = BG_MIN_SCORE;
        a.sc.yp = a.sc.ys = 0;
    }
    if (mode == BG_MODE_LOCAL) a.sc.xp = a.sc.xs = a.sc.yp = a.sc.ys = 0;
    a.mode = mode;
    a.filter_clips = (mode == BG_MODE_SEMIGLOBAL || mode == BG_MODE_LOCAL);
    a.out = d_out;
    a.ops = d_ops;
    a.ops_stride = ops_stride;

    int sm = SCORE_PARAMS;
    if (sc->matrix) {
        uint64_t h = 0xcbf29ce484222325ull;
        {
            const uint64_t* w = (const uint64_t*)sc->matrix;
            uint64_t h2 = 0x9e3779b97f4a7c15ull;
            for (size_t t = 0; t < 32768; t += 2) {
                h = (h ^ w[t]) * 0x100000001b3ull;
                h2 = (h2 + w[t + 1]) * 0xff51afd7ed558ccdull;
                h2 ^= h2 >> 32;
            }
            h ^= h2;
            if (h == 0) h = 1;
        }
        if (ctx->table_hash != h || !ctx->table_matrix || memcmp(ctx->table_matrix, sc->matrix, 65536 * sizeof(int32_t)) != 0) {
            std::vector<uint8_t> code_map;
            std::vector<int32_t> table;
            const int A = compact_matrix(sc->matrix, code_map, table);
            const size_t bytes = 256 + table.size() * 4;
            ctx->table_hash = 0;
            if (!ctx->table_matrix && !(ctx->table_matrix = (int32_t*)malloc(65536 * sizeof(int32_t)))) return BG_ERR_OOM;
            if ((rc = bg_reserve(&ctx->sw_table, &ctx->sw_table_bytes, bytes))) return rc;
            BG_HIP(hipMemcpyAsync((uint8_t*)ctx->sw_table + 256, table.data(), table.size() * 4,
                                  hipMemcpyHostToDevice, st));
            BG_HIP(hipMemcpyAsync(ctx->sw_table, code_map.data(), 256, hipMemcpyHostToDevice, st));
            BG_HIP(hipStreamSynchronize(st));
            memcpy(ctx->table_matrix, sc->matrix, 65536 * sizeof(int32_t));
            ctx->table_hash = h;
            ctx->table_alpha = A;
        }
        const int A = ctx->table_alpha;
        sm = A <= kMaxLdsAlphabet ? SCORE_LDS : SCORE_GLOBAL;
        a.code_map = (const uint8_t*)ctx->sw_table;
        a.table = (const int32_t*)((uint8_t*)ctx->sw_table + 256);
        a.alpha = A;
    }

    Config cfg = pick_config(max_xlen, sm);
    const bool all_zero_clips = a.sc.xp == 0 && a.sc.xs == 0 && a.sc.yp == 0 && a.sc.ys == 0;
    int64_t mag = std::max<int64_t>(std::abs((int64_t)a.sc.go), std::abs((int64_t)a.sc.ge));
    for (int32_t c : {a.sc.xp, a.sc.xs, a.sc.yp, a.sc.ys})
        if (c != BG_MIN_SCORE) mag = std::max<int64_t>(mag, std::abs((int64_t)c));
    if (sc->matrix) {
        for (size_t t = 0; t < 65536; t++) mag = std::max<int64_t>(mag, std::abs((int64_t)sc->matrix[t]));
    } else {
        mag = std::max<int64_t>(mag, std::max(std::abs((int64_t)a.sc.match), std::abs((int64_t)a.sc.mismatch)));
    }
    const bool narrow = !ctx->force_wide && mag * ((int64_t)max_xlen + max_ylen + 8) < (1 << 24);
    sw_fill_fn fill = sm == SCORE_PARAMS
                          ? (narrow ? get_fill_params_narrow(cfg.lp, cfg.r, all_zero_clips)
                                    : get_fill_params_wide(cfg.lp, cfg.r, all_zero_clips))
                          : get_fill_matrix(cfg.lp, cfg.r, sm, narrow, all_zero_clips);
    if (!fill && sm != SCORE_PARAMS && cfg.lp == 16 && cfg.r < 12) {
        cfg.r = 12;
        fill = get_fill_matrix(cfg.lp, cfg.r, sm, narrow, all_zero_clips);
    }
    a.g.tb_fmt = 0;
    if (fill && sm == SCORE_PARAMS && narrow && all_zero_clips && a.sc.go < 0 && a.sc.mismatch < 0 && a.sc.match >= 0 &&
        !ctx->no_local_fast && max_xlen <= (uint32_t)(cfg.lp * cfg.r)) {
        if (sw_fill_fn lf = get_fill_params_lf(cfg.lp, cfg.r)) {
            fill = lf;
            a.g.tb_fmt = 3;
        }
    }
    sw_fill_fn fill_rest = nullptr, fill_second = nullptr;
    bool pk16 = !ctx->no_pk16 && sm == SCORE_PARAMS && cfg.lp <= 32 && max_xlen >= 1 &&
                      mag * ((int64_t)std::max(max_xlen, max_ylen) + 2) <= 2040;
    if (pk16) {
        const SwScoring& c = a.sc;
        const int32_t M = BG_MIN_SCORE;
        const bool local_fast = all_zero_clips && c.go < 0 && c.mismatch < 0 && c.match >= 0 && !ctx->no_local_fast;
        auto getter = local_fast ? get_fill_pk16_localfast
                      : all_zero_clips ? get_fill_pk16_local
                      : (c.xp == M && c.xs == M && c.yp == 0 && c.ys == 0) ? get_fill_pk16_semiglobal
                      : (c.xp == M && c.xs == M && c.yp == M && c.ys == M) ? get_fill_pk16_global
                                                                           : get_fill_pk16_custom;
        int r_pick = 0;
        for (int r = (int)((max_xlen + cfg.lp - 1) / cfg.lp); r <= 12 && !r_pick; r++)
            if (max_xlen % r == 0 && getter(cfg.lp, r, 0)) r_pick = r;
        for (int r = (int)((max_xlen + cfg.lp - 1) / cfg.lp); r <= 12 && !r_pick; r++)
            if (getter(cfg.lp, r, 0)) r_pick = r;
        if (!r_pick) {
            pk16 = false;
        } else {
            cfg.r = r_pick;
            fill = getter(cfg.lp, cfg.r, 0);
            fill_rest = local_fast ? nullptr : getter(cfg.lp, cfg.r, 1);
            fill_second = getter(cfg.lp, cfg.r, 2);
            a.g.tb_fmt = local_fast ? 2 : 1;
        }
    }
    if (!fill) return BG_ERR_UNSUPPORTED;
    ctx->fill_mask |= pk16 ? (a.g.tb_fmt == 2 ? BG_FILL_K1P_LF : BG_FILL_K1P)
                           : a.g.tb_fmt == 3 ? BG_FILL_K1_LF : narrow ? BG_FILL_K1_NARROW : BG_FILL_K1_WIDE;
    if (packed_codes) {
        if (pk16) {
            a.packed = 1;
        } else {
            uint64_t tot[2] = {0, 0};
            BG_HIP(hipMemcpyAsync(&tot[0], d_x_off + n_pairs, 8, hipMemcpyDeviceToHost, st));
            BG_HIP(hipMemcpyAsync(&tot[1], d_y_off + n_pairs, 8, hipMemcpyDeviceToHost, st));
            BG_HIP(hipStreamSynchronize(st));
            for (int k = 0; k < 2; k++)
                if ((rc = bg_reserve(&ctx->unpk[k], &ctx->unpk_cap[k], std::max<uint64_t>(tot[k], 16)))) return rc;
            if ((rc = bg_unpack2_dev(ctx, (const uint32_t*)d_x, tot[0], packed_codes, (uint8_t*)ctx->unpk[0], st))) return rc;
            if ((rc = bg_unpack2_dev(ctx, (const uint32_t*)d_y, tot[1], packed_codes, (uint8_t*)ctx->unpk[1], st))) return rc;
            a.x = (const uint8_t*)ctx->unpk[0];
            a.y = (const uint8_t*)ctx->unpk[1];
        }
    }
    const int nw = tb_words(cfg.r);
    const uint32_t pw = 64 / cfg.lp;
    SwGeom& g = a.g;
    g.lp = cfg.lp;
    g.r = cfg.r;
    g.r_inv = (uint32_t)(((1ull << 32) + cfg.r - 1) / cfg.r);
    g.lp_shift = cfg.lp == 16 ? 4 : cfg.lp == 32 ? 5 : 6;
    g.m_cap = max_xlen;
    g.n_cap = max_ylen;
    g.nsteps = max_ylen ? max_ylen + cfg.lp - 1 : 0;
    g.nstrips = std::max<uint32_t>(1, (max_xlen + cfg.lp * cfg.r - 1) / (cfg.lp * cfg.r));
    g.aux_stride = SwGeom::stride_for(max_xlen, max_ylen);

    const size_t tb_per_job = (size_t)tb_job_words(g.nstrips, g.nsteps, nw) * 4;
    const size_t aux_per_pair = (size_t)g.aux_stride * 4;
    const size_t bnd_per_pair = g.nstrips > 1 ? (size_t)(g.n_cap + 1) * 16 : 0;
    const size_t per_pair = tb_per_job / pw + aux_per_pair + bnd_per_pair + 1;
    uint64_t chunk = ctx->chunk_pairs > 0 ? (uint64_t)ctx->chunk_pairs : (1u << 20);
    const uint64_t budget = 48ull << 30;
    chunk = std::min<uint64_t>(chunk, std::max<uint64_t>(pw, budget / per_pair));
    chunk = std::min<uint64_t>(chunk, n_pairs);
    chunk = (chunk + pw - 1) / pw * pw;
    const uint64_t jobs = chunk / pw;
    if ((rc = bg_reserve(&ctx->tb, &ctx->tb_bytes, std::max<size_t>(jobs * tb_per_job, 64)))) return rc;
    if ((rc = bg_reserve(&ctx->aux, &ctx->aux_bytes, chunk * aux_per_pair))) return rc;
    if ((rc = bg_reserve(&ctx->bnd, &ctx->bnd_bytes, std::max<size_t>(chunk * bnd_per_pair, 64)))) return rc;
    a.tb = ctx->tb;
    a.aux = (int32_t*)ctx->aux;
    a.bnd = (int4*)ctx->bnd;
    uint32_t *d_keycnt = nullptr, *d_keysum = nullptr, *d_perm = nullptr, *d_lenst = nullptr;
    if (pk16 && !ctx->no_couples) {
        const size_t need = (size_t)kLenKeys * 4 + 1024 * 4 + 64 + chunk * 4;
        if ((rc = bg_reserve(&ctx->bnd, &ctx->bnd_bytes, need))) return rc;
        a.bnd = (int4*)ctx->bnd;
        d_keycnt = (uint32_t*)ctx->bnd;
        d_keysum = d_keycnt + kLenKeys;
        d_lenst = d_keysum + 1024;
        d_perm = d_lenst + 16;
    }

    for (uint64_t p0 = 0; p0 < n_pairs; p0 += chunk) {
        a.pair0 = p0;
        a.n_pairs = (uint32_t)std::min<uint64_t>(chunk, n_pairs - p0);
        const uint32_t njobs = (a.n_pairs + pw - 1) / pw;
        a.perm = nullptr;
        a.len_stats = nullptr;
        a.n_eff = nullptr;
        if (d_perm && a.n_pairs >= 64 && len_hint != 1) {
            const uint32_t* d_st = nullptr;
            if (len_hint < 0) {
                BG_HIP(hipMemsetAsync(d_lenst, 0xff, 8, st));
                BG_HIP(hipMemsetAsync(d_lenst + 2, 0, 8, st));
                sw_len_stats_kernel<<<dim3(std::min<uint32_t>((a.n_pairs + 255) / 256, 256)), dim3(256), 0, st>>>(d_x_off, d_y_off, p0, a.n_pairs, d_lenst);
                d_st = d_lenst;
            }
            BG_HIP(hipMemsetAsync(d_keycnt, 0, (size_t)kLenKeys * 4, st));
            sw_key_hist_kernel<<<dim3((a.n_pairs + 255) / 256), dim3(256), 0, st>>>(d_x_off, d_y_off, p0, a.n_pairs, d_keycnt, d_st);
            sw_key_block_sums_kernel<<<dim3(1024), dim3(256), 0, st>>>(d_keycnt, d_keysum, d_st);
            sw_key_scan_kernel<<<dim3(1024), dim3(1024), 0, st>>>(d_keycnt, d_keysum, d_st);
            sw_key_scatter_kernel<<<dim3((a.n_pairs + 255) / 256), dim3(256), 0, st>>>(d_x_off, d_y_off, p0, a.n_pairs, d_keycnt, d_perm, d_st);
            BG_HIP(hipGetLastError());
            sw_decide_kernel<<<dim3(1), dim3(1), 0, st>>>(d_lenst, a.n_pairs, len_hint < 0 ? -1 : 0, d_lenst + 4);
            a.perm = d_perm;
            a.len_stats = d_st;
            a.n_eff = d_lenst + 4;
        }
        if (ctx->timing) BG_HIP(hipEventRecord(ctx->ev[0], st));
        const uint32_t nwaves = pk16 ? (njobs + 1) / 2 : njobs;
        fill<<<dim3((nwaves + 3) / 4), dim3(256), 0, st>>>(a);
        BG_HIP(hipGetLastError());
        if (ctx->timing) BG_HIP(hipEventRecord(ctx->ev[1], st));
        if (fill_rest) fill_rest<<<dim3((nwaves + 3) / 4), dim3(256), 0, st>>>(a);
        if (fill_second && len_hint != 1) fill_second<<<dim3((nwaves + 3) / 4), dim3(256), 0, st>>>(a);
        BG_HIP(hipGetLastError());
        if (ctx->timing) {
            BG_HIP(hipEventSynchronize(ctx->ev[1]));
            float ms = 0;
            BG_HIP(hipEventElapsedTime(&ms, ctx->ev[0], ctx->ev[1]));
            ctx->last.fill_ms += ms;
            ctx->last.fill_launches += 1;
            BG_HIP(hipEventRecord(ctx->ev[0], st));
        }
        launch_traceback(a, nw, st);
        BG_HIP(hipGetLastError());
        if (ctx->timing) {
            BG_HIP(hipEventRecord(ctx->ev[1], st));
            BG_HIP(hipEventSynchronize(ctx->ev[1]));
            float ms = 0;
            BG_HIP(hipEventElapsedTime(&ms, ctx->ev[0], ctx->ev[1]));
            ctx->last.traceback_ms += ms;
            ctx->last.traceback_launches += 1;
        }
    }
    return BG_OK;
}

int bg_align_batch_dev_hint(bg_ctx* ctx, const bg_scoring_t* sc, int mode, uint64_t n_pairs, const uint8_t* d_x,
                            const uint64_t* d_x_off, const uint8_t* d_y, const uint64_t* d_y_off, uint32_t max_xlen,
                            uint32_t max_ylen, bg_alignment_t* d_out, uint8_t* d_ops, uint64_t ops_stride, void* stream,
                            int len_hint) {
    return align_batch_dev_impl(ctx, sc, mode, n_pairs, d_x, d_x_off, d_y, d_y_off, max_xlen, max_ylen, d_out, d_ops, ops_stride,
                                stream, len_hint);
}

extern "C" int bg_align_batch_dev(bg_ctx* ctx, const bg_scoring_t* sc, int mode, uint64_t n_pairs,
                                  const uint8_t* d_x, const uint64_t* d_x_off, const uint8_t* d_y,
                                  const uint64_t* d_y_off, uint32_t max_xlen, uint32_t max_ylen,
                                  bg_alignment_t* d_out, uint8_t* d_ops, uint64_t ops_stride,
                                  void* stream) {
    if (ctx) ctx->fill_mask = 0;
    return align_batch_dev_impl(ctx, sc, mode, n_pairs, d_x, d_x_off, d_y, d_y_off, max_xlen, max_ylen, d_out, d_ops, ops_stride, stream, -1);
}

extern "C" int bg_align_batch_packed_dev(bg_ctx* ctx, const bg_scoring_t* sc, int mode, uint64_t n_pairs, const uint32_t* d_x,
                                         const uint64_t* d_x_off, const uint32_t* d_y, const uint64_t* d_y_off,
                                         const uint8_t codes[4], uint32_t max_xlen, uint32_t max_ylen, bg_alignment_t* d_out,
                                         uint8_t* d_ops, uint64_t ops_stride, void* stream) {
    if (!codes || (n_pairs && (!d_x || !d_y))) return BG_ERR_INVALID_ARG;
    for (int a = 0; a < 4; a++)
        for (int b = a + 1; b < 4; b++)
            if (codes[a] == codes[b]) return BG_ERR_INVALID_ARG;
    if (ctx) ctx->fill_mask = 0;
    return align_batch_dev_impl(ctx, sc, mode, n_pairs, (const uint8_t*)d_x, d_x_off, (const uint8_t*)d_y, d_y_off, max_xlen, max_ylen,
                                d_out, d_ops, ops_stride, stream, -1, codes);
}

struct bg_host_pipe {
    static constexpr int NSET = 3;
    struct Set {
        uint8_t *h_in = nullptr, *h_out = nullptr;
        uint8_t *d_in = nullptr, *d_out = nullptr;
        uint8_t *d_cmp = nullptr, *d_scan = nullptr;
        size_t in_cap = 0, out_cap = 0, cmp_cap = 0, scan_cap = 0;
        hipEvent_t in_done = nullptr, k_done = nullptr, out_done = nullptr;
    } set[NSET];
    uint64_t* d_cell = nullptr;
    hipStream_t s_in = nullptr, s_out = nullptr;
};
void bg_host_pipe_free(bg_host_pipe* p) {
    if (!p) return;
    for (auto& s : p->set) {
        if (s.h_in) hipHostFree(s.h_in);
        if (s.h_out) hipHostFree(s.h_out);
        hipFree(s.d_in);
        hipFree(s.d_out);
        hipFree(s.d_cmp);
        hipFree(s.d_scan);
        for (hipEvent_t e : {s.in_done, s.k_done, s.out_done})
            if (e) hipEventDestroy(e);
    }
    hipFree(p->d_cell);
    if (p->s_in) hipStreamDestroy(p->s_in);
    if (p->s_out) hipStreamDestroy(p->s_out);
    delete p;
}
namespace {
typedef uint32_t u32x4 __attribute__((ext_vector_type(4)));
template <bool NT>
__global__ __launch_bounds__(256) void stage_to_host_kernel(const u32x4* __restrict__ rec, u32x4* __restrict__ h_rec, uint64_t rec_n16,
                                                            const u32x4* __restrict__ ops, u32x4* __restrict__ h_ops,
                                                            const uint64_t* __restrict__ d_total, uint64_t* __restrict__ h_total) {
    const uint64_t tid = (uint64_t)blockIdx.x * 256 + threadIdx.x, nth = (uint64_t)gridDim.x * 256;
    for (uint64_t i = tid; i < rec_n16; i += nth) {
        if (NT) __builtin_nontemporal_store(rec[i], &h_rec[i]);
        else h_rec[i] = rec[i];
    }
    const uint64_t T = d_total ? *d_total : 0, n16 = (T + 15) / 16;
    for (uint64_t i = tid; i < n16; i += nth) {
        if (NT) __builtin_nontemporal_store(ops[i], &h_ops[i]);
        else h_ops[i] = ops[i];
    }
    if (tid == 0) *h_total = T;
}

template <typename F>
void parallel_for(uint64_t n, uint64_t grain, F&& f) {
    const unsigned nt = (unsigned)std::max<uint64_t>(1, std::min<uint64_t>(bg_host_threads(), n / std::max<uint64_t>(grain, 1) + 1));
    if (nt == 1) {
        f((uint64_t)0, n);
        return;
    }
    bg_pool_run(nt, [&](unsigned t) { f(n * t / nt, n * (t + 1) / nt); });
}
void parallel_memcpy(uint8_t* dst, const uint8_t* src, uint64_t n) {
    parallel_for(n, 1 << 20, [&](uint64_t a, uint64_t b) { memcpy(dst + a, src + a, b - a); });
}

int align_batch_pipelined(bg_ctx* ctx, const bg_scoring_t* sc, int mode, uint64_t n_pairs, const uint8_t* x, const uint64_t* x_off,
                          const uint8_t* y, const uint64_t* y_off, uint32_t max_x, uint32_t max_y, uint64_t chunk, bg_alignment_t* out,
                          uint8_t* ops_buf, uint64_t ops_cap, uint64_t* ops_used) {
    if (!ctx->pipe) {
        ctx->pipe = new bg_host_pipe();
        BG_HIP(hipStreamCreateWithFlags(&ctx->pipe->s_in, hipStreamNonBlocking));
        {
            int lo = 0, hi = 0;
            BG_HIP(hipDeviceGetStreamPriorityRange(&lo, &hi));
            BG_HIP(hipStreamCreateWithPriority(&ctx->pipe->s_out, hipStreamNonBlocking, hi));
        }
        BG_HIP(hipMalloc((void**)&ctx->pipe->d_cell, 64));
        for (auto& s : ctx->pipe->set)
            for (hipEvent_t* e : {&s.in_done, &s.k_done, &s.out_done}) BG_HIP(hipEventCreateWithFlags(e, hipEventDisableTiming));
    }
    bg_host_pipe& P = *ctx->pipe;
    const uint64_t stride = ops_buf ? (uint64_t)max_x + max_y + 4 : 0;
    std::vector<uint64_t> cut{0};
    while (cut.back() < n_pairs) cut.push_back(std::min(n_pairs, cut.back() + chunk));
    const uint64_t nch = cut.size() - 1;
    uint64_t max_xb = 0, max_yb = 0;
    for (uint64_t c = 0; c < nch; c++) {
        const uint64_t p0 = cut[c], p1 = cut[c + 1];
        max_xb = std::max(max_xb, x_off[p1] - x_off[p0]);
        max_yb = std::max(max_yb, y_off[p1] - y_off[p0]);
    }
    const uint64_t o_y = (max_xb + 255) & ~255ull, o_xo = o_y + ((max_yb + 255) & ~255ull), o_yo = o_xo + (chunk + 1) * 8;
    const size_t in_need = o_yo + (chunk + 1) * 8 + 256;
    const uint64_t o_tot = chunk * sizeof(bg_alignment_t), o_ops = o_tot + 256;
    const size_t out_need = o_ops + chunk * stride + 256;
    const size_t cmp_need = chunk * stride + 256;
    const size_t scan_need = bg_compact_ops_scratch(chunk);
    for (auto& s : P.set) {
        if (s.in_cap < in_need) {
            if (s.h_in) hipHostFree(s.h_in);
            hipFree(s.d_in);
            s.h_in = s.d_in = nullptr;
            s.in_cap = 0;
            BG_HIP(hipHostMalloc((void**)&s.h_in, in_need, hipHostMallocDefault));
            BG_HIP(hipMalloc((void**)&s.d_in, in_need));
            s.in_cap = in_need;
        }
        if (s.out_cap < out_need) {
            if (s.h_out) hipHostFree(s.h_out);
            hipFree(s.d_out);
            s.h_out = s.d_out = nullptr;
            s.out_cap = 0;
            BG_HIP(hipHostMalloc((void**)&s.h_out, out_need, hipHostMallocDefault));
            BG_HIP(hipMalloc((void**)&s.d_out, out_need));
            s.out_cap = out_need;
        }
        if (stride && s.cmp_cap < cmp_need) {
            hipFree(s.d_cmp);
            s.d_cmp = nullptr;
            s.cmp_cap = 0;
            BG_HIP(hipMalloc((void**)&s.d_cmp, cmp_need));
            s.cmp_cap = cmp_need;
        }
        if (stride && s.scan_cap < scan_need) {
            hipFree(s.d_scan);
            s.d_scan = nullptr;
            s.scan_cap = 0;
            BG_HIP(hipMalloc((void**)&s.d_scan, scan_need));
            s.scan_cap = scan_need;
        }
    }
    hipStream_t s_k = ctx->stream;
    BG_HIP(hipMemsetAsync(P.d_cell, 0, 8, s_k));
    uint64_t used = 0;
    int status = BG_OK;
    const bool trace = getenv("BG_TRACE_HOST") != nullptr;
    double t_pack = 0, t_launch = 0, t_wait_set = 0, t_d_wait_rec = 0, t_d_rec = 0, t_d_ops = 0;
    auto now = [] { return std::chrono::duration<double, std::milli>(std::chrono::steady_clock::now().time_since_epoch()).count(); };
    auto drain = [&](uint64_t c) -> int {
        bg_host_pipe::Set& S = P.set[c % bg_host_pipe::NSET];
        double t0 = now();
        BG_HIP(hipEventSynchronize(S.out_done));
        t_d_wait_rec += now() - t0;
        const uint64_t p0 = cut[c], np = cut[c + 1] - p0;
        const bg_alignment_t* h_rec = (const bg_alignment_t*)S.h_out;
        const uint64_t T = stride ? *(const uint64_t*)(S.h_out + o_tot) : 0;
        std::atomic<int> st_rec{BG_OK};
        t0 = now();
        parallel_for(np, 16384, [&](uint64_t a, uint64_t b) {
            memcpy(out + p0 + a, h_rec + a, (b - a) * sizeof(bg_alignment_t));
            int sr = BG_OK;
            for (uint64_t p = a; p < b; p++)
                if (h_rec[p].status) sr = h_rec[p].status;
            if (sr) st_rec = sr;
        });
        if (st_rec) status = st_rec;
        t_d_rec += now() - t0;
        if (T) {
            t0 = now();
            uint64_t fit = T;
            if (used + T > ops_cap) {
                if (status == BG_OK) status = BG_ERR_OPS_CAP;
                fit = 0;
                for (uint64_t p = 0; p < np; p++) {
                    if (h_rec[p].ops_off + h_rec[p].n_ops > ops_cap) break;
                    fit = h_rec[p].ops_off + h_rec[p].n_ops - used;
                }
            }
            if (fit) parallel_memcpy(ops_buf + used, S.h_out + o_ops, fit);
            t_d_ops += now() - t0;
        }
        used += T;
        return BG_OK;
    };
    std::mutex mu;
    std::condition_variable cv;
    uint64_t submitted = 0, drained = 0;
    bool abort_drain = false;
    int drain_rc = BG_OK;
    std::string drain_err;
    const int device = ctx->device;
    std::thread drainer([&] {
        if (hipSetDevice(device) != hipSuccess) {
            std::lock_guard<std::mutex> lk(mu);
            drain_rc = BG_ERR_HIP;
            drained = nch;
            cv.notify_all();
            return;
        }
        for (uint64_t c = 0; c < nch; c++) {
            {
                std::unique_lock<std::mutex> lk(mu);
                cv.wait(lk, [&] { return submitted > c || abort_drain; });
                if (submitted <= c) break;
            }
            const int r = drain(c);
            std::lock_guard<std::mutex> lk(mu);
            if (r && drain_rc == BG_OK) {
                drain_rc = r;
                drain_err = bg_tls_error;
            }
            drained = c + 1;
            cv.notify_all();
        }
        std::lock_guard<std::mutex> lk(mu);
        drained = nch;
        cv.notify_all();
    });
    auto stop_drainer = [&] {
        {
            std::lock_guard<std::mutex> lk(mu);
            abort_drain = true;
        }
        cv.notify_all();
        drainer.join();
    };
    int rc;
    for (uint64_t c = 0; c < nch; c++) {
        double t0 = now();
        if (c >= bg_host_pipe::NSET) {
            std::unique_lock<std::mutex> lk(mu);
            cv.wait(lk, [&] { return drained >= c - bg_host_pipe::NSET + 1; });
        }
        t_wait_set += now() - t0;
        t0 = now();
        bg_host_pipe::Set& S = P.set[c % bg_host_pipe::NSET];
        const uint64_t p0 = cut[c], np = cut[c + 1] - p0;
        const uint64_t xb = x_off[p0 + np] - x_off[p0], yb = y_off[p0 + np] - y_off[p0];
        parallel_memcpy(S.h_in, x + x_off[p0], xb);
        parallel_memcpy(S.h_in + o_y, y + y_off[p0], yb);
        uint64_t *hxo = (uint64_t*)(S.h_in + o_xo), *hyo = (uint64_t*)(S.h_in + o_yo);
        std::atomic<bool> ragged{false};
        const uint64_t len_x = np ? x_off[p0 + 1] - x_off[p0] : 0, len_y = np ? y_off[p0 + 1] - y_off[p0] : 0;
        parallel_for(np + 1, 16384, [&](uint64_t a, uint64_t b) {
            bool rag = false;
            for (uint64_t p = a; p < b; p++) {
                hxo[p] = x_off[p0 + p] - x_off[p0];
                hyo[p] = y_off[p0 + p] - y_off[p0];
                if (p < np) rag = rag || x_off[p0 + p + 1] - x_off[p0 + p] != len_x || y_off[p0 + p + 1] - y_off[p0 + p] != len_y;
            }
            if (rag) ragged = true;
        });
        t_pack += now() - t0;
        t0 = now();
        bool in_ok = true;
        if (xb) in_ok = in_ok && bg_copy_pieces(S.d_in, S.h_in, xb, hipMemcpyHostToDevice, P.s_in) == hipSuccess;
        if (yb) in_ok = in_ok && bg_copy_pieces(S.d_in + o_y, S.h_in + o_y, yb, hipMemcpyHostToDevice, P.s_in) == hipSuccess;
        in_ok = in_ok && hipMemcpyAsync(S.d_in + o_xo, S.h_in + o_xo, 2 * (chunk + 1) * 8, hipMemcpyHostToDevice, P.s_in) == hipSuccess;
        in_ok = in_ok && hipEventRecord(S.in_done, P.s_in) == hipSuccess && hipStreamWaitEvent(s_k, S.in_done, 0) == hipSuccess;
        const bool uniform = !ragged;
        bg_alignment_t* d_rec = (bg_alignment_t*)S.d_out;
        rc = !in_ok ? BG_ERR_HIP : align_batch_dev_impl(ctx, sc, mode, np, S.d_in, (const uint64_t*)(S.d_in + o_xo), S.d_in + o_y, (const uint64_t*)(S.d_in + o_yo),
                                  max_x, max_y, d_rec, stride ? S.d_out + o_ops : nullptr, stride, s_k, uniform ? 1 : 0);
        if (rc == BG_OK && stride)
            rc = bg_compact_ops_dev(d_rec, np, S.d_out + o_ops, S.d_cmp, false, P.d_cell, (uint64_t*)(S.d_out + o_tot), S.d_scan, false, s_k);
        if (rc == BG_OK && (hipEventRecord(S.k_done, s_k) != hipSuccess || hipStreamWaitEvent(P.s_out, S.k_done, 0) != hipSuccess))
            rc = BG_ERR_HIP;
        if (rc == BG_OK) {
            static const int d2h_blocks = getenv("BG_D2H_BLOCKS") ? std::max(1, atoi(getenv("BG_D2H_BLOCKS"))) : 8;
            static const bool d2h_nt = !(getenv("BG_D2H_NT") && atoi(getenv("BG_D2H_NT")) == 0);
            (d2h_nt ? stage_to_host_kernel<true> : stage_to_host_kernel<false>)<<<dim3(d2h_blocks), dim3(256), 0, P.s_out>>>((const u32x4*)S.d_out, (u32x4*)S.h_out, np * sizeof(bg_alignment_t) / 16,
                                                                     (const u32x4*)S.d_cmp, (u32x4*)(S.h_out + o_ops),
                                                                     stride ? (const uint64_t*)(S.d_out + o_tot) : nullptr, (uint64_t*)(S.h_out + o_tot));
            if (hipGetLastError() != hipSuccess || hipEventRecord(S.out_done, P.s_out) != hipSuccess) rc = BG_ERR_HIP;
        }
        if (rc) {
            hipDeviceSynchronize();
            stop_drainer();
            return rc;
        }
        t_launch += now() - t0;
        {
            std::lock_guard<std::mutex> lk(mu);
            submitted = c + 1;
        }
        cv.notify_all();
    }
    double t0j = now();
    drainer.join();
    if (trace)
        fprintf(stderr, "[bg host] %llu stages: pack %.2f launch %.2f wait-for-set %.2f join %.2f | drainer: wait-stage %.2f copy-records %.2f copy-ops %.2f ms\n",
                (unsigned long long)nch, t_pack, t_launch, t_wait_set, now() - t0j, t_d_wait_rec, t_d_rec, t_d_ops);
    if (drain_rc) {
        bg_tls_error = drain_err;
        return drain_rc;
    }
    if (ops_used) *ops_used = used;
    return status;
}
}

extern "C" int bg_align_batch(bg_ctx* ctx, const bg_scoring_t* sc, int mode, uint64_t n_pairs,
                              const uint8_t* x, const uint64_t* x_off, const uint8_t* y,
                              const uint64_t* y_off, bg_alignment_t* out, uint8_t* ops_buf,
                              uint64_t ops_cap, uint64_t* ops_used) {
    if (!ctx || !sc) return BG_ERR_INVALID_ARG;
    ctx->fill_mask = 0;
    int rc = check_scoring(sc);
    if (rc) return rc;
    if (ops_used) *ops_used = 0;
    if (n_pairs == 0) return BG_OK;
    if (!x_off || !y_off || !out) return BG_ERR_INVALID_ARG;
    BG_HIP(hipSetDevice(ctx->device));
    uint64_t max_x = 0, max_y = 0, max_sum = 0;
    bool uniform_len = true;
    {
        std::mutex mu;
        bool bad = false;
        parallel_for(n_pairs, 1 << 16, [&](uint64_t a, uint64_t b) {
            uint64_t mx = 0, my = 0, ms = 0;
            bool uni = true, neg = false;
            for (uint64_t p = a; p < b; p++) {
                neg = neg || x_off[p + 1] < x_off[p] || y_off[p + 1] < y_off[p];
                const uint64_t lx = x_off[p + 1] - x_off[p], ly = y_off[p + 1] - y_off[p];
                mx = std::max(mx, lx);
                my = std::max(my, ly);
                ms = std::max(ms, lx + ly);
                uni = uni && lx == x_off[1] - x_off[0] && ly == y_off[1] - y_off[0];
            }
            std::lock_guard<std::mutex> lk(mu);
            max_x = std::max(max_x, mx);
            max_y = std::max(max_y, my);
            max_sum = std::max(max_sum, ms);
            uniform_len = uniform_len && uni;
            bad = bad || neg;
        });
        if (bad) return BG_ERR_INVALID_ARG;
    }
    if (max_x > (1u << 24) || max_y > (1u << 24)) return BG_ERR_TOO_LARGE;
    {
        const uint64_t chunk = ctx->host_chunk_pairs > 0 ? (uint64_t)ctx->host_chunk_pairs : 122880;
        if (n_pairs >= 2 * chunk && !sc->matrix)
            return align_batch_pipelined(ctx, sc, mode, n_pairs, x, x_off, y, y_off, (uint32_t)max_x, (uint32_t)max_y, chunk, out, ops_buf, ops_cap,
                                         ops_used);
    }
    const uint64_t xb = x_off[n_pairs], yb = y_off[n_pairs];
    const uint64_t stride = ops_buf ? max_x + max_y + 4 : 0;
    (void)max_sum;
    const size_t need[6] = {std::max<uint64_t>(xb, 16), std::max<uint64_t>(yb, 16), (n_pairs + 1) * 8, (n_pairs + 1) * 8,
                            n_pairs * sizeof(bg_alignment_t), std::max<uint64_t>(n_pairs * stride, 16)};
    for (int i = 0; i < 6; i++)
        if ((rc = bg_reserve(&ctx->io[i], &ctx->io_cap[i], need[i]))) return rc;
    uint8_t *d_x = (uint8_t*)ctx->io[0], *d_y = (uint8_t*)ctx->io[1], *d_ops = stride ? (uint8_t*)ctx->io[5] : nullptr;
    uint64_t *d_xo = (uint64_t*)ctx->io[2], *d_yo = (uint64_t*)ctx->io[3];
    bg_alignment_t* d_out = (bg_alignment_t*)ctx->io[4];
    if (stride && n_pairs * stride > ctx->h_ops_cap) {
        if (ctx->h_ops) hipHostFree(ctx->h_ops);
        ctx->h_ops = nullptr;
        ctx->h_ops_cap = 0;
        BG_HIP(hipHostMalloc(&ctx->h_ops, n_pairs * stride, hipHostMallocDefault));
        ctx->h_ops_cap = n_pairs * stride;
    }
    hipStream_t st = ctx->stream;
    if (xb) BG_HIP(hipMemcpyAsync(d_x, x, xb, hipMemcpyHostToDevice, st));
    if (yb) BG_HIP(hipMemcpyAsync(d_y, y, yb, hipMemcpyHostToDevice, st));
    BG_HIP(hipMemcpyAsync(d_xo, x_off, (n_pairs + 1) * 8, hipMemcpyHostToDevice, st));
    BG_HIP(hipMemcpyAsync(d_yo, y_off, (n_pairs + 1) * 8, hipMemcpyHostToDevice, st));
    rc = align_batch_dev_impl(ctx, sc, mode, n_pairs, d_x, d_xo, d_y, d_yo, (uint32_t)max_x, (uint32_t)max_y, d_out, d_ops, stride, st,
                              uniform_len ? 1 : 0);
    if (rc) return rc;
    BG_HIP(hipMemcpyAsync(out, d_out, n_pairs * sizeof(bg_alignment_t), hipMemcpyDeviceToHost, st));
    if (stride) BG_HIP(hipMemcpyAsync(ctx->h_ops, d_ops, n_pairs * stride, hipMemcpyDeviceToHost, st));
    BG_HIP(hipStreamSynchronize(st));
    const uint8_t* h_ops = (const uint8_t*)ctx->h_ops;
    uint64_t used = 0;
    int status = BG_OK;
    std::vector<uint64_t> src(n_pairs);
    for (uint64_t p = 0; p < n_pairs; p++) {
        if (out[p].status) status = out[p].status;
        src[p] = out[p].ops_off;
        out[p].ops_off = used;
        if (ops_buf && used + out[p].n_ops > ops_cap && status == BG_OK) status = BG_ERR_OPS_CAP;
        used += out[p].n_ops;
    }
    if (ops_buf) {
        unsigned nt = std::max(1u, std::min(bg_host_threads(), (unsigned)(n_pairs / 4096 + 1)));
        std::vector<std::thread> th;
        for (unsigned t = 0; t < nt; t++)
            th.emplace_back([&, t] {
                for (uint64_t p = n_pairs * t / nt, pe = n_pairs * (t + 1) / nt; p < pe; p++)
                    if (out[p].ops_off + out[p].n_ops <= ops_cap) memcpy(ops_buf + out[p].ops_off, h_ops + src[p], out[p].n_ops);
            });
        for (auto& t : th) t.join();
    }
    if (ops_used) *ops_used = used;
    return status;
}
```

rust-bio_amd/csrc/sw_fill_pk16.inc:

```
#include <type_traits>

#include "sw_kernels.h"

namespace bgsw {
namespace pk16 {

typedef uint32_t pk;

typedef short s16x2 __attribute__((ext_vector_type(2)));
typedef unsigned short u16x2 __attribute__((ext_vector_type(2)));
__device__ __forceinline__ s16x2 as_s(pk v) { return __builtin_bit_cast(s16x2, v); }
__device__ __forceinline__ u16x2 as_u(pk v) { return __builtin_bit_cast(u16x2, v); }
__device__ __forceinline__ pk bits(s16x2 v) { return __builtin_bit_cast(pk, v); }
__device__ __forceinline__ pk bits(u16x2 v) { return __builtin_bit_cast(pk, v); }
__device__ __forceinline__ pk pk_adds(pk a, pk b) { return bits(__builtin_elementwise_add_sat(as_s(a), as_s(b))); }
__device__ __forceinline__ pk pk_max(pk a, pk b) { return bits(__builtin_elementwise_max(as_s(a), as_s(b))); }
__device__ __forceinline__ pk pk_min(pk a, pk b) { return bits(__builtin_elementwise_min(as_s(a), as_s(b))); }
__device__ __forceinline__ pk pk_add_u16(pk a, pk b) { return bits((u16x2)(as_u(a) + as_u(b))); }
__device__ __forceinline__ pk pk_sub_u16(pk a, pk b) { return bits((u16x2)(as_u(a) - as_u(b))); }
__device__ __forceinline__ pk pk_subs_u16(pk a, pk b) { return bits(__builtin_elementwise_sub_sat(as_u(a), as_u(b))); }
__device__ __forceinline__ pk pk_mad_u16(pk a, pk b, pk c) { return bits((u16x2)(as_u(a) * as_u(b) + as_u(c))); }
__device__ __forceinline__ pk dup16(int32_t v) { return ((uint32_t)v & 0xffffu) | ((uint32_t)v << 16); }
__device__ __forceinline__ pk bfi(pk mask, pk a, pk b) { return (a & mask) | (b & ~mask); }
__device__ __forceinline__ pk nz_mask(pk v, pk one) { return pk_sub_u16(pk_subs_u16(one, v), one); }

template <int LP>
__device__ __forceinline__ void scan_first_max(int ll, int64_t& v, uint32_t& idx) {
#pragma unroll
    for (int off = 1; off < LP; off <<= 1) {
        const int64_t ov = __shfl_up(v, off, LP);
        const uint32_t oi = (uint32_t)__shfl_up((int)idx, off, LP);
        if (ll >= off && !(v > ov)) {
            v = ov;
            idx = oi;
        }
    }
}

constexpr int32_t kFloor16 = -2048;

enum { CZ = 0, CF = 1, CI = 2 };
template <int R, int LP, int MODE, int XP, int XS, int YP, int YS, bool LF = false>
__device__ __forceinline__ void sw_fill_pk16_body(const SwArgs& a) {
    constexpr bool FAST = MODE == 0;
    constexpr int PW = 64 / LP;
    constexpr int NW = tb_words(R);
    constexpr int NH = (R + 2) / 3;
    constexpr bool NARROW = true, LOCAL = XP == CZ && XS == CZ && YP == CZ && YS == CZ;
    constexpr bool ROW0_ZERO = YP == CZ && YS == CZ;
    constexpr int SH = 4;
    constexpr int32_t NEGS = kFloor16 * 16;
    constexpr pk CLEAN = 0xfff0fff0u, FLOORK = 0x80008000u, ONE = 0x00010001u;
    static_assert(LP == 16 || LP == 32, "lanes per pair");
    static_assert(R >= 1 && R <= 12, "rows per lane");
    static_assert(!LF || LOCAL, "LF is a flavour of the local kernel");
    (void)NARROW;
    (void)LOCAL;
    constexpr int kTileStride = 20;
    constexpr int kParkDw = 64 * (4 * R + NH + 1), kTileDw = 2 * 64 * kTileStride;
    constexpr int kWaveDw = kParkDw > kTileDw ? kParkDw : kTileDw;
    __shared__ __align__(16) pk s_lds[4 * kWaveDw];
    pk* const wave_lds = s_lds + (threadIdx.x >> 6) * kWaveDw;

    const int lane = threadIdx.x & 63;
    const uint32_t wv = blockIdx.x * (blockDim.x >> 6) + (threadIdx.x >> 6);
    if ((uint64_t)wv * 2 * PW >= a.n_pairs) return;
    if (MODE == 2 && a.len_stats && a.len_stats[0] == a.len_stats[2] && a.len_stats[1] == a.len_stats[3]) return;
    const int g = lane / LP, ll = lane % LP;
    const SwScoring sc = a.sc;
    const SwGeom geo = a.g;
    auto scl = [](int32_t v) -> int32_t { return max(v, kFloor16) * 16; };
    const int32_t go_s = sc.go * 16, xs_s = sc.xs <= kFloor16 ? -(1 << 30) : sc.xs * 16;
    (void)xs_s;
    constexpr int32_t K_XS = C_XS << 1, K_MATCH = C_MATCH << 1, K_SUBST = C_SUBST << 1, K_INS = C_INS << 1,
                      K_DEL = C_DEL << 1, K_XP = C_XP << 1;
    constexpr pk NOFLAG = 0xfffefffeu;
    const pk GE = dup16(sc.ge * 16);
    const pk GOT_I = dup16(sc.go * 16 + K_INS + 1), GOT_D = dup16(sc.go * 16 + K_DEL + 1);
    const pk MISK = dup16((sc.mismatch * 16) | K_SUBST);
    const pk DELTA = dup16(((sc.match * 16) | K_MATCH) - ((sc.mismatch * 16) | K_SUBST));
    const pk XS16 = dup16(scl(sc.xs)), YS16 = dup16(scl(sc.ys));
    const pk XSCAP = sc.xs <= kFloor16 ? FLOORK : 0x7fff7fffu, YSCAP = sc.ys <= kFloor16 ? FLOORK : 0x7fff7fffu;
    (void)XS16; (void)YS16; (void)XSCAP; (void)YSCAP;
    const pk MISC = dup16(-((sc.mismatch * 16) | K_SUBST));
    (void)MISC;
    pk C16 = dup16(16), C32 = dup16(32), C1024 = dup16(1024);
    asm volatile("" : "+s"(C16), "+s"(C32), "+s"(C1024));

    const uint32_t pA = (2 * wv) * PW + g, pB = (2 * wv + 1) * PW + g;
    const bool okA = pA < a.n_pairs, okB = pB < a.n_pairs;
    uint32_t mA = 0, nA = 0, mB = 0, nB = 0;
    uint64_t xoA = 0, yoA = 0, xoB = 0, yoB = 0;
    const uint32_t* perm = a.slot_perm();
    if (okA) {
        const uint64_t r = a.pair0 + (perm ? perm[pA] : pA);
        xoA = a.x_off[r];
        yoA = a.y_off[r];
        mA = (uint32_t)(a.x_off[r + 1] - xoA);
        nA = (uint32_t)(a.y_off[r + 1] - yoA);
        if (len_over(geo, mA, nA)) mA = nA = 0;
    }
    if (okB) {
        const uint64_t r = a.pair0 + (perm ? perm[pB] : pB);
        xoB = a.x_off[r];
        yoB = a.y_off[r];
        mB = (uint32_t)(a.x_off[r + 1] - xoB);
        nB = (uint32_t)(a.y_off[r + 1] - yoB);
        if (len_over(geo, mB, nB)) mB = nB = 0;
    }
    const bool same = okA && okB && mA == mB && nA == nB;
    const bool two = okA && okB && !same;
    const bool m_last0 = LF || __all(!okA || mA % R == 0);
    if (MODE == 0 && !m_last0) return;
    if (MODE == 1 && m_last0) return;
    if (MODE == 2 && !__any(two)) return;
    const uint64_t job_words = tb_job_words(geo.nstrips, geo.nsteps, NW);

    auto do_pass = [&](const int pass) {
        const bool pair_ok = pass == 0 ? okA : two;
        const uint32_t P0 = pass == 0 ? pA : pB, P1 = (pass == 0 && !same) ? pA : pB;
        const uint32_t m = !pair_ok ? 0 : (pass == 0 ? mA : mB), n = !pair_ok ? 0 : (pass == 0 ? nA : nB);
        const uint64_t xs0 = pass == 0 ? xoA : xoB, ys0 = pass == 0 ? yoA : yoB;
        const uint64_t xs1 = (pass == 0 && !same) ? xoA : xoB, ys1 = (pass == 0 && !same) ? yoA : yoB;
        const uint8_t* x0 = a.x + xs0;
        const uint8_t* x1 = a.x + xs1;
        const bool packed = a.packed != 0;
        auto y_pair = [&](uint32_t col) -> pk {
            if (packed) return sym2(a.y, ys0 + col) | (sym2(a.y, ys1 + col) << 16);
            return (uint32_t)a.y[ys0 + col] | ((uint32_t)a.y[ys1 + col] << 16);
        };
        const uint32_t Q0 = pair_ok ? P0 : 0, Q1 = pair_ok ? P1 : 0;
        uint32_t* tb0 = (uint32_t*)a.tb + (size_t)(Q0 / PW) * job_words + ((Q0 % PW) * LP + ll) * 16u;
        uint32_t* tb1 = (uint32_t*)a.tb + (size_t)(Q1 / PW) * job_words + ((Q1 % PW) * LP + ll) * 16u;
        int32_t* aux0 = a.aux + (size_t)Q0 * geo.aux_stride;
        int32_t* aux1 = a.aux + (size_t)Q1 * geo.aux_stride;
        int32_t* gLx0 = aux0 + geo.off_Lx();
        int32_t* gLx1 = aux1 + geo.off_Lx();

        uint32_t m_w = m, n_w = n;
#pragma unroll
        for (int o = 32; o; o >>= 1) {
            m_w = max(m_w, (uint32_t)__shfl_xor((int)m_w, o));
            n_w = max(n_w, (uint32_t)__shfl_xor((int)n_w, o));
        }
        (void)m_w;
        n_w = (uint32_t)__builtin_amdgcn_readfirstlane((int)n_w);
        const uint32_t nsteps_w = n_w ? n_w + LP - 1 : 0;

        int32_t fold0;
        uint32_t lx0;
        col0_fold(sc, m, fold0, lx0);
        int32_t Sn0 = sc.ys;
        uint32_t Ly0 = n;
        int32_t S0n = 0;
        uint32_t sb0n = (ROW0_ZERO && n) ? row0_cell(sc, n).sbits : (uint32_t)TB_START;
        if (pair_ok && ll == 0) {
            const int32_t v = m ? (int32_t)col0_cell(sc, m, m, fold0).sbits : (int32_t)TB_START;
            aux0[0] = v;
            aux1[0] = v;
            if (m == 0) {
                if (LP == 16) {
                    *(uint8_t*)gLx0 = (uint8_t)lx0;
                    *(uint8_t*)gLx1 = (uint8_t)lx0;
                } else {
                    *(uint16_t*)gLx0 = (uint16_t)lx0;
                    *(uint16_t*)gLx1 = (uint16_t)lx0;
                }
            }
        }

        const uint32_t rb = (uint32_t)ll * R;
        const int32_t mrow = (int32_t)m - (int32_t)rb - 1;
        pk Sl[R], Dl[R], Il[R], SnR[R], SnB[R], Ly[R], px[R];
        uint64_t nib0S = 0, nib0I = 0;
        uint64_t xw0 = 0, xw1 = 0;
        if (packed && pair_ok && rb < m) {
            const uint32_t* p0 = (const uint32_t*)a.x + ((xs0 + rb) >> 4);
            const uint32_t* p1 = (const uint32_t*)a.x + ((xs1 + rb) >> 4);
            xw0 = (((uint64_t)p0[1] << 32) | p0[0]) >> (2 * ((uint32_t)(xs0 + rb) & 15u));
            xw1 = (((uint64_t)p1[1] << 32) | p1[0]) >> (2 * ((uint32_t)(xs1 + rb) & 15u));
        }
#pragma unroll
        for (int r = 0; r < R; r++) {
            const uint32_t i = rb + r + 1;
            px[r] = 0;
            Sl[r] = Dl[r] = Il[r] = SnR[r] = SnB[r] = FLOORK;
            Ly[r] = 0;
            if (pair_ok && i <= m) {
                px[r] = packed ? (((uint32_t)(xw0 >> (2 * r)) & 3u) | (((uint32_t)(xw1 >> (2 * r)) & 3u) << 16))
                               : ((uint32_t)x0[i - 1] | ((uint32_t)x1[i - 1] << 16));
                const Col0 c = col0_cell(sc, i, m, fold0);
                Sl[r] = dup16(scl(c.S));
                Il[r] = dup16(scl(c.I) | K_INS);
                nib0S |= (uint64_t)c.sbits << (4 * r);
                nib0I |= (uint64_t)c.ibits << (4 * r);
                if (YS != CI && c.S + sc.ys > NEG) {
                    SnR[r] = dup16(scl(c.S + sc.ys));
                    Ly[r] = dup16((int32_t)n);
                }
            }
        }
        pk diag0 = dup16((pair_ok && rb < m) ? scl(col0_S(sc, rb, m, fold0)) : NEGS);

        pk S_out = FLOORK, I_out = FLOORK, cm_out = FLOORK, ca_out = 0, q_out = 0;
        pk ychunk = 0, ychunk_nx = 0;
        pk hwlast[NH];
#pragma unroll
        for (int k = 0; k < NH; k++) hwlast[k] = 0;
        pk lx_n = dup16((int32_t)lx0);
        pk* tileA = wave_lds + (0 * 64 + lane) * kTileStride;
        pk* tileB = wave_lds + (1 * 64 + lane) * kTileStride;
        uint32_t lxaccA = lx0 << (LP == 16 ? 24 : 16), lxaccB = lxaccA;
        if (pair_ok && (uint32_t)ll < n) ychunk_nx = y_pair((uint32_t)ll);

        auto merge_rows = [&](uint32_t blockbase) {
            const pk lybase = dup16((int32_t)(n - blockbase - 16u + (uint32_t)ll));
#pragma unroll
            for (int r = 0; r < R; r++) {
                const pk nr = pk_max(SnR[r], SnB[r] & CLEAN);
                const pk msk = nz_mask(nr ^ SnR[r], ONE);
                Ly[r] = bfi(msk, pk_add_u16(lybase, SnB[r] & 0x000f000fu), Ly[r]);
                SnR[r] = nr;
                SnB[r] = FLOORK;
            }
        };

        constexpr uint32_t tsteps = tb_tile_steps(NW);
        auto store_tile = [&](uint32_t s_any) {
            if (!pair_ok) return;
            const uint32_t off = (s_any / tsteps) * 1024u;
#pragma unroll
            for (int k = 0; k < 4; k++) {
                *(uint4*)&tb0[off + 4 * k] = *(const uint4*)&tileA[4 * k];
                *(uint4*)&tb1[off + 4 * k] = *(const uint4*)&tileB[4 * k];
            }
        };
        uint32_t s_all = pair_ok ? n + (uint32_t)ll : 0u;
#pragma unroll
        for (int o = 32; o; o >>= 1) s_all = min(s_all, (uint32_t)__shfl_xor((int)s_all, o));
        s_all = (uint32_t)__builtin_amdgcn_readfirstlane((int)s_all);
        auto run_steps = [&](auto mr_tag) {
        constexpr int MRk = decltype(mr_tag)::value;
        auto step = [&](auto allon_tag, auto fast_tag, const uint32_t s) {
            constexpr bool ALLON = decltype(allon_tag)::value;
            constexpr bool FB = decltype(fast_tag)::value;
            constexpr bool FOLD = XS != CI && !FB;
            if ((s & (LP - 1)) == 0) {
                ychunk = ychunk_nx;
                const uint32_t nb = s + LP + ll;
                if (pair_ok && nb < n) ychunk_nx = y_pair(nb);
            }
            pk S_up = (pk)wave_shr1((int)S_out, (int)S_out), I_up = (pk)wave_shr1((int)I_out, (int)I_out);
            pk cm = FLOORK, ca = 0;
            if (FOLD) {
                cm = (pk)wave_shr1((int)cm_out, (int)cm_out);
                ca = (pk)wave_shr1((int)ca_out, (int)ca_out);
            }
            pk q = (pk)wave_shr1((int)q_out, (int)q_out);
            const uint32_t j = s + 1 - (uint32_t)ll;
            const bool col_ok = ALLON || (pair_ok && (j - 1) < n);
            if (ll == 0) {
                q = ychunk;
                S_up = 0;
                I_up = FLOORK;
                cm = FLOORK;
                ca = 0;
                if (!ROW0_ZERO && col_ok) {
                    const Row0 c = row0_cell(sc, j);
                    int32_t S0 = c.S;
                    uint32_t sb = c.sbits;
                    if (j == n && Sn0 > S0) {
                        S0 = Sn0;
                        sb = TB_YCLIP_SUFFIX;
                    } else if (S0 + sc.ys > Sn0) {
                        Sn0 = S0 + sc.ys;
                        Ly0 = n - j;
                    }
                    S0n = S0;
                    sb0n = sb;
                    S_up = dup16(scl(S0));
                }
            }
            ychunk = (pk)wave_shl1((int)ychunk, (int)ychunk);

            if (col_ok) {
                const pk sprio = dup16((int32_t)(15u - (s & 15u)));
                pk diag = diag0;
                diag0 = S_up;
                pk hw[NH];
                const pk ca_in = ca;
                pk cmk = cm | 0x000f000fu;
                pk snap = cmk;
                pk XKEY = dup16(K_XP);
                if (XP == CF || (XP == CZ && YP != CZ))
                    XKEY = dup16(scl(sc.xp + max(sc.yp, sc.go + sc.ge * ((int32_t)j - 1))) | K_XP);
#pragma unroll
                    for (int r = 0; r < R; r++) {
                        const bool maybe_m = MRk < 0 || r == MRk;
                        const bool is_m = MRk < 0 ? (r == mrow) : (r == MRk && mrow == MRk);
                        const pk e = pk_subs_u16(ONE, px[r] ^ q);
                        const pk m_key = LF ? pk_subs_u16(pk_mad_u16(e, DELTA, diag), MISC) : pk_adds(diag, pk_mad_u16(e, DELTA, MISK));
                        const pk Iv_t = pk_max(pk_adds(I_up, GE), pk_adds(S_up, GOT_I));
                        const pk Dv_t = pk_max(pk_adds(Dl[r], GE), pk_adds(Sl[r], GOT_D));
                        const pk Iv = Iv_t & NOFLAG, Dv = Dv_t & NOFLAG;
                        pk kb = pk_max(m_key, Dv_t);
                        if (XP != CI && !LF) kb = pk_max(kb, XKEY);
                        kb = pk_max(kb, Iv_t);
                        if (FOLD && maybe_m)
                            kb = pk_max(kb, is_m ? ((cmk & CLEAN) | (0x00010001u * K_XS)) : FLOORK);
                        const pk best = kb & CLEAN;
                        diag = Sl[r];
                        Sl[r] = best;
                        Dl[r] = Dv;
                        Il[r] = Iv;
                        S_up = best;
                        I_up = Iv;
                        if (FOLD) {
                            if (maybe_m) snap = is_m ? cmk : snap;
                            const pk fv = XS == CZ ? best : pk_min(pk_adds(best, XS16), XSCAP);
                            cmk = pk_max(cmk, fv | (0x00010001u * (uint32_t)(14 - r)));
                        }
                        if (YS != CI) {
                            const pk t1 = YS == CZ ? best : pk_min(pk_adds(best, YS16), YSCAP);
                            SnB[r] = pk_max(SnB[r], t1 | sprio);
                        }
                        const pk c5 = pk_mad_u16(Dv_t & ONE, C16, (kb & 0x000e000eu) | (Iv_t & ONE));
                        if (r % 3 == 0)
                            hw[r / 3] = c5;
                        else
                            hw[r / 3] = pk_mad_u16(c5, r % 3 == 1 ? C32 : C1024, hw[r / 3]);
                    }
                if (FOLD) {
                    const pk mbase = dup16(mrow - 14);
                    const pk lo = cmk & 0x000f000fu, slo = snap & 0x000f000fu;
                    if (mrow >= 0 && mrow < R) {
                        const pk is15 = nz_mask(slo ^ 0x000f000fu, ONE);
                        lx_n = bfi(is15, pk_add_u16(slo, mbase), ca_in);
                        if (LP == 16) {
                            lxaccA = __builtin_amdgcn_perm(lx_n, lxaccA, 0x04030201u);
                            lxaccB = __builtin_amdgcn_perm(lx_n, lxaccB, 0x06030201u);
                            if ((j & 3u) == 3u || j == n) {
                                const uint32_t sh = 8u * (3u - (j & 3u));
                                ((uint32_t*)gLx0)[j >> 2] = lxaccA >> sh;
                                ((uint32_t*)gLx1)[j >> 2] = lxaccB >> sh;
                            }
                        } else {
                            lxaccA = __builtin_amdgcn_perm(lx_n, lxaccA, 0x05040302u);
                            lxaccB = __builtin_amdgcn_perm(lx_n, lxaccB, 0x07060302u);
                            if ((j & 1u) == 1u || j == n) {
                                const uint32_t sh = 16u * (1u - (j & 1u));
                                ((uint32_t*)gLx0)[j >> 1] = lxaccA >> sh;
                                ((uint32_t*)gLx1)[j >> 1] = lxaccB >> sh;
                            }
                        }
                    }
                    {
                        const pk is15 = nz_mask(lo ^ 0x000f000fu, ONE);
                        ca = bfi(is15, pk_add_u16(lo, mbase), ca_in);
                    }
                    cm = cmk & CLEAN;
                }
                constexpr pk INV = 0x00010001u * (17u | (17u << 5) | (17u << 10));
                constexpr pk INV_LAST = 0x00010001u * ((R % 3 == 0) ? (17u | (17u << 5) | (17u << 10))
                                                      : (R % 3 == 1) ? 17u : (17u | (17u << 5)));
#pragma unroll
                for (int k = 0; k < NH; k++) {
                    hw[k] ^= (k == NH - 1) ? INV_LAST : INV;
                    hwlast[k] = hw[k];
                }
                const pk h0 = hw[0], h1 = NH > 1 ? hw[NH > 1 ? 1 : 0] : 0u;
                const uint32_t slot = (s % tsteps) * NW;
                if (NW == 1) {
                    tileA[slot] = __builtin_amdgcn_perm(h1, h0, 0x05040100u);
                    tileB[slot] = __builtin_amdgcn_perm(h1, h0, 0x07060302u);
                } else {
                    const pk h2 = hw[NH > 2 ? 2 : 0], h3 = NH > 3 ? hw[NH > 3 ? 3 : 0] : 0u;
                    *(uint2*)&tileA[slot] = make_uint2(__builtin_amdgcn_perm(h1, h0, 0x05040100u),
                                                       __builtin_amdgcn_perm(h3, h2, 0x05040100u));
                    *(uint2*)&tileB[slot] = make_uint2(__builtin_amdgcn_perm(h1, h0, 0x07060302u),
                                                       __builtin_amdgcn_perm(h3, h2, 0x07060302u));
                }
                S_out = S_up;
                I_out = I_up;
                if (FOLD) {
                    cm_out = cm;
                    ca_out = ca;
                }
                q_out = q;
            }
            if (s % tsteps == tsteps - 1) store_tile(s);
            if (YS != CI && (s & 15u) == 15u) merge_rows(s & ~15u);
        };
        uint32_t s = 0;
        const uint32_t s_on = min((uint32_t)(LP - 1), nsteps_w), s_off = max(s_on, min(s_all, nsteps_w));
        constexpr std::false_type no{};
        constexpr std::true_type yes{};
        constexpr std::bool_constant<LF> fast{};
        for (; s < s_on; s++) step(no, fast, s);
        for (; s + 1 < s_off; s += 2) {
            step(yes, fast, s);
            step(yes, fast, s + 1);
        }
        for (; s < s_off; s++) step(yes, fast, s);
        for (; s < nsteps_w; s++) step(no, fast, s);
        };
        run_steps(std::integral_constant<int, (FAST && !LF) ? R - 1 : -1>{});
        if (nsteps_w % tsteps) store_tile(nsteps_w - 1);
        if (YS != CI && nsteps_w) merge_rows((nsteps_w - 1) & ~15u);

        pk* park = wave_lds + lane;
#pragma unroll
        for (int r = 0; r < R; r++) {
            park[(0 * R + r) * 64] = Sl[r];
            park[(1 * R + r) * 64] = Il[r];
            park[(2 * R + r) * 64] = SnR[r];
            park[(3 * R + r) * 64] = Ly[r];
        }
#pragma unroll
        for (int k = 0; k < NH; k++) park[(4 * R + k) * 64] = hwlast[k];
        park[(4 * R + NH) * 64] = lx_n;
        const int nhalf = (pair_ok && P1 != P0) ? 2 : 1;
        const int nhalf_w = __any(nhalf == 2) ? 2 : 1;
#pragma unroll 1
        for (int h = 0; h < nhalf_w; h++) {
            if (h >= nhalf) continue;
            const uint32_t hs = 16u * (uint32_t)h;
            int32_t* aux = h ? aux1 : aux0;
            int32_t* gLy = aux + geo.off_Ly();
            uint8_t* gBits = (uint8_t*)(aux + geo.off_bits());
            const uint32_t strip = 0;
            struct HalfS {
                const pk* p;
                uint32_t hs;
                __device__ int32_t operator[](int r) const { return (int32_t)(int16_t)(p[r * 64] >> hs); }
            };
            struct HalfU {
                const pk* p;
                uint32_t hs;
                __device__ uint32_t operator[](int r) const { return (p[r * 64] >> hs) & 0xffffu; }
            };
            int32_t Sl_u[R];
#pragma unroll
            for (int r = 0; r < R; r++) Sl_u[r] = (int32_t)(int16_t)(park[r * 64] >> hs);
            const HalfS Il_u{park + 1 * R * 64, hs}, Sn_u{park + 2 * R * 64, hs};
            const HalfU Ly_u{park + 3 * R * 64, hs};
            const uint32_t lx_n_u = (park[(4 * R + NH) * 64] >> hs) & 0xffffu;
            int64_t e_carry = INT64_MIN;
            uint32_t sbf_carry = TB_START, sb2_carry = TB_START;
            int64_t c1v = INT64_MIN, c2v = INT64_MIN;
            uint32_t c1i = 0, c2i = 0;
            auto cell_of = [&](int r) -> uint32_t {
                const uint32_t c = (park[(4 * R + r / 3) * 64] >> (hs + 5 * (r % 3))) & 31u;
                const uint32_t mv = (c >> 1) & 7u;
                return ((LF && mv == 0) ? (uint32_t)C_XP : mv) | ((c & 1u) << 3) | (c & 16u);
            };
            {
                constexpr bool EPI_FOLD_PRE = LF;
                int32_t(&Sl)[R] = Sl_u;
                const HalfS& Il = Il_u;
                const HalfS& Sn = Sn_u;
                const HalfU& Ly = Ly_u;
                const uint32_t lx_n = lx_n_u;
#include "sw_epilogue.inc"
            }
        }
    };
    do_pass(MODE == 2 ? 1 : 0);
}

template <int R, int LP, int XP, int XS, int YP, int YS, bool LF>
__global__ __launch_bounds__(256) __attribute__((amdgpu_waves_per_eu(R <= 10 ? 3 : 2, R <= 10 ? 3 : 2))) void sw_fill_pk16_kernel(const SwArgs a) {
    sw_fill_pk16_body<R, LP, 0, XP, XS, YP, YS, LF>(a);
}
template <int R, int LP, int XP, int XS, int YP, int YS, bool LF>
__global__ __launch_bounds__(256) __attribute__((amdgpu_waves_per_eu(R <= 10 ? 3 : 2, R <= 10 ? 3 : 2))) void sw_fill_pk16_rest_kernel(const SwArgs a) {
    sw_fill_pk16_body<R, LP, 1, XP, XS, YP, YS, LF>(a);
}
template <int R, int LP, int XP, int XS, int YP, int YS, bool LF>
__global__ __launch_bounds__(256) __attribute__((amdgpu_waves_per_eu(R <= 10 ? 3 : 2, R <= 10 ? 3 : 2))) void sw_fill_pk16_second_kernel(const SwArgs a) {
    sw_fill_pk16_body<R, LP, 2, XP, XS, YP, YS, LF>(a);
}

}
}

#define BG_PK16_CASE(LP_, R_)                                                                          \
    if (lp == LP_ && r == R_)                                                                         \
        return which == 0   ? pk16::sw_fill_pk16_kernel<R_, LP_, XP_, XS_, YP_, YS_, LF_>             \
               : which == 1 ? pk16::sw_fill_pk16_rest_kernel<R_, LP_, XP_, XS_, YP_, YS_, LF_>        \
                            : pk16::sw_fill_pk16_second_kernel<R_, LP_, XP_, XS_, YP_, YS_, LF_>;
```

rust-bio_amd/csrc/sw_fill_pk16_custom.hip:

```cpp
#include "sw_fill_pk16.inc"
namespace bgsw {
sw_fill_fn get_fill_pk16_custom(int lp, int r, int which) {
    constexpr int XP_ = pk16::CF, XS_ = pk16::CF, YP_ = pk16::CF, YS_ = pk16::CF;
    constexpr bool LF_ = false;
    BG_PK16_CASE(16, 2) BG_PK16_CASE(16, 4) BG_PK16_CASE(16, 5) BG_PK16_CASE(16, 6) BG_PK16_CASE(16, 8) BG_PK16_CASE(16, 10) BG_PK16_CASE(16, 12)
    BG_PK16_CASE(32, 8) BG_PK16_CASE(32, 10) BG_PK16_CASE(32, 12)
    return nullptr;
}
}
```

rust-bio_amd/csrc/sw_fill_pk16_global.hip:

```cpp
#include "sw_fill_pk16.inc"
namespace bgsw {
sw_fill_fn get_fill_pk16_global(int lp, int r, int which) {
    constexpr int XP_ = pk16::CI, XS_ = pk16::CI, YP_ = pk16::CI, YS_ = pk16::CI;
    constexpr bool LF_ = false;
    BG_PK16_CASE(16, 2) BG_PK16_CASE(16, 4) BG_PK16_CASE(16, 5) BG_PK16_CASE(16, 6) BG_PK16_CASE(16, 8) BG_PK16_CASE(16, 10) BG_PK16_CASE(16, 12)
    BG_PK16_CASE(32, 8) BG_PK16_CASE(32, 10) BG_PK16_CASE(32, 12)
    return nullptr;
}
}
```

rust-bio_amd/csrc/sw_fill_pk16_local.hip:

```cpp
#include "sw_fill_pk16.inc"
namespace bgsw {
sw_fill_fn get_fill_pk16_local(int lp, int r, int which) {
    constexpr int XP_ = pk16::CZ, XS_ = pk16::CZ, YP_ = pk16::CZ, YS_ = pk16::CZ;
    constexpr bool LF_ = false;
    BG_PK16_CASE(16, 2) BG_PK16_CASE(16, 3) BG_PK16_CASE(16, 4) BG_PK16_CASE(16, 5) BG_PK16_CASE(16, 6) BG_PK16_CASE(16, 7)
    BG_PK16_CASE(16, 8) BG_PK16_CASE(16, 9) BG_PK16_CASE(16, 10) BG_PK16_CASE(16, 11) BG_PK16_CASE(16, 12)
    BG_PK16_CASE(32, 7) BG_PK16_CASE(32, 8) BG_PK16_CASE(32, 9) BG_PK16_CASE(32, 10) BG_PK16_CASE(32, 11) BG_PK16_CASE(32, 12)
    return nullptr;
}
}
```

rust-bio_amd/csrc/sw_fill_pk16_localfast.hip:

```cpp
#include "sw_fill_pk16.inc"
namespace bgsw {
sw_fill_fn get_fill_pk16_localfast(int lp, int r, int which) {
    constexpr int XP_ = pk16::CZ, XS_ = pk16::CZ, YP_ = pk16::CZ, YS_ = pk16::CZ;
    constexpr bool LF_ = true;
    BG_PK16_CASE(16, 2) BG_PK16_CASE(16, 3) BG_PK16_CASE(16, 4) BG_PK16_CASE(16, 5) BG_PK16_CASE(16, 6) BG_PK16_CASE(16, 7)
    BG_PK16_CASE(16, 8) BG_PK16_CASE(16, 9) BG_PK16_CASE(16, 10) BG_PK16_CASE(16, 11) BG_PK16_CASE(16, 12)
    BG_PK16_CASE(32, 7) BG_PK16_CASE(32, 8) BG_PK16_CASE(32, 9) BG_PK16_CASE(32, 10) BG_PK16_CASE(32, 11) BG_PK16_CASE(32, 12)
    return nullptr;
}
}
```

rust-bio_amd/csrc/sw_fill_pk16_semiglobal.hip:

```cpp
#include "sw_fill_pk16.inc"
namespace bgsw {
sw_fill_fn get_fill_pk16_semiglobal(int lp, int r, int which) {
    constexpr int XP_ = pk16::CI, XS_ = pk16::CI, YP_ = pk16::CZ, YS_ = pk16::CZ;
    constexpr bool LF_ = false;
    BG_PK16_CASE(16, 2) BG_PK16_CASE(16, 4) BG_PK16_CASE(16, 5) BG_PK16_CASE(16, 6) BG_PK16_CASE(16, 8) BG_PK16_CASE(16, 10) BG_PK16_CASE(16, 12)
    BG_PK16_CASE(32, 8) BG_PK16_CASE(32, 10) BG_PK16_CASE(32, 12)
    return nullptr;
}
}
```

rust-bio_amd/csrc/sw_kernels.h:

```cpp
#ifndef BG_SW_KERNELS_H
#define BG_SW_KERNELS_H
#include <type_traits>

#include "bg_common.h"

namespace bgsw {

constexpr int32_t NEG = BG_MIN_SCORE;

enum : uint32_t {
    TB_START = 0, TB_INS = 1, TB_DEL = 2, TB_SUBST = 3, TB_MATCH = 4,
    TB_XCLIP_PREFIX = 5, TB_XCLIP_SUFFIX = 6, TB_YCLIP_PREFIX = 7, TB_YCLIP_SUFFIX = 8
};
enum : uint32_t { C_XS = 7, C_MATCH = 6, C_SUBST = 5, C_INS = 3, C_DEL = 2, C_XP = 1, C_YP = 0 };
constexpr int32_t kNarrowFloor = -(1 << 26);
constexpr int32_t kNarrowKeyFloor = (int32_t)0x80000000;

enum { SCORE_PARAMS = 0, SCORE_LDS = 1, SCORE_GLOBAL = 2 };
constexpr int kMaxLdsAlphabet = 64;

struct SwScoring {
    int32_t go, ge, xp, xs, yp, ys;
    int32_t match, mismatch;
};

struct SwGeom {
    uint32_t lp, r, nsteps, nstrips, m_cap, n_cap, aux_stride;
    uint32_t tb_fmt;
    uint32_t r_inv;
    uint32_t lp_shift;
    __host__ __device__ uint32_t off_Ly() const { return 4; }
    __host__ __device__ uint32_t off_Lx() const { return 4 + (m_cap + 1); }
    __host__ __device__ uint32_t off_bits() const { return 4 + (m_cap + 1) + (n_cap + 1); }
    __host__ __device__ static uint32_t stride_for(uint32_t m_cap, uint32_t n_cap) {
        return 4 + (m_cap + 1) + (n_cap + 1) + (m_cap + 1 + 3) / 4;
    }
};

__device__ __forceinline__ bool len_over(const SwGeom& g, uint32_t m, uint32_t n) { return m > g.m_cap || n > g.n_cap; }

__host__ __device__ constexpr int tb_words(int r) { return (r + 5) / 6; }
__host__ __device__ constexpr uint32_t tb_tile_steps(int nw) { return 16u / (uint32_t)nw; }
__host__ __device__ inline uint64_t tb_job_words(uint32_t nstrips, uint32_t nsteps, int nw) {
    const uint64_t g = (uint64_t)nstrips * nsteps, t = tb_tile_steps(nw);
    return (g + t - 1) / t * 1024ull;
}
__host__ __device__ inline uint64_t tb_word_off(uint64_t g, uint32_t lane, int nw) {
    const uint32_t t = tb_tile_steps(nw);
    return (g / t) * 1024ull + lane * 16u + (uint32_t)(g % t) * (uint32_t)nw;
}

struct SwArgs {
    const uint8_t* x;
    const uint64_t* x_off;
    const uint8_t* y;
    const uint64_t* y_off;
    uint64_t pair0;
    uint32_t n_pairs;
    SwScoring sc;
    const int32_t* table;
    const uint8_t* code_map;
    int32_t alpha;
    void* tb;
    int32_t* aux;
    int4* bnd;
    const uint32_t* perm;
    const uint32_t* len_stats;
    const uint32_t* n_eff;
    __device__ const uint32_t* slot_perm() const {
        if (!perm) return nullptr;
        if (len_stats && len_stats[0] == len_stats[2] && len_stats[1] == len_stats[3]) return nullptr;
        return perm;
    }
    SwGeom g;
    bg_alignment_t* out;
    uint8_t* ops;
    uint64_t ops_stride;
    int32_t mode;
    int32_t filter_clips;
    int32_t packed;
};
__device__ __forceinline__ uint32_t sym2(const uint8_t* stream, uint64_t s) {
    return (((const uint32_t*)stream)[s >> 4] >> (2 * ((uint32_t)s & 15u))) & 3u;
}

struct Col0 {
    int32_t S, I;
    uint32_t sbits, ibits;
};
__device__ __forceinline__ Col0 col0_cell(const SwScoring& sc, uint32_t i, uint32_t m, int32_t fold) {
    Col0 c;
    if (i == 1) {
        c.I = sc.go;
        c.ibits = TB_START;
    } else {
        const int32_t i_score = sc.go + sc.ge * ((int32_t)i - 1);
        const int32_t c_score = sc.xp + sc.go;
        if (i_score > c_score) {
            c.I = i_score;
            c.ibits = TB_INS;
        } else {
            c.I = c_score;
            c.ibits = TB_XCLIP_PREFIX;
        }
    }
    if (i == m) {
        c.S = fold;
        c.sbits = TB_XCLIP_SUFFIX;
    } else {
        c.S = NEG;
        c.sbits = TB_START;
    }
    if (c.I > c.S) {
        c.S = c.I;
        c.sbits = TB_INS;
    }
    if (sc.xp > c.S) {
        c.S = sc.xp;
        c.sbits = TB_XCLIP_PREFIX;
    }
    return c;
}
__device__ __forceinline__ void col0_fold(const SwScoring& sc, uint32_t m, int32_t& fold, uint32_t& lx0) {
    fold = NEG;
    lx0 = 0;
    if (m >= 2) {
        const Col0 c = col0_cell(sc, 1, m, NEG);
        if (c.S + sc.xs > fold) {
            fold = c.S + sc.xs;
            lx0 = m - 1;
        }
    }
}
__device__ __forceinline__ int32_t col0_S(const SwScoring& sc, uint32_t i, uint32_t m, int32_t fold0) {
    if (i == 0) return 0;
    return col0_cell(sc, i, m, fold0).S;
}

struct Row0 {
    int32_t S, D;
    uint32_t sbits, dbits;
};
__device__ __forceinline__ Row0 row0_cell(const SwScoring& sc, uint32_t j) {
    Row0 c;
    if (j == 1) {
        c.D = sc.go;
        c.dbits = TB_START;
    } else {
        const int32_t d_score = sc.go + sc.ge * ((int32_t)j - 1);
        const int32_t c_score = sc.yp + sc.go;
        if (d_score > c_score) {
            c.D = d_score;
            c.dbits = TB_DEL;
        } else {
            c.D = c_score;
            c.dbits = TB_YCLIP_PREFIX;
        }
    }
    if (c.D > sc.yp) {
        c.S = c.D;
        c.sbits = TB_DEL;
    } else {
        c.S = sc.yp;
        c.sbits = TB_YCLIP_PREFIX;
    }
    return c;
}

__device__ __forceinline__ uint32_t s_nibble_of_code(uint32_t code) {
    switch (code) {
        case C_MATCH: return TB_MATCH;
        case C_SUBST: return TB_SUBST;
        case C_INS: return TB_INS;
        case C_DEL: return TB_DEL;
        case C_XP: return TB_XCLIP_PREFIX;
        case C_YP: return TB_YCLIP_PREFIX;
        default: return TB_XCLIP_SUFFIX;
// ... 8 lines not shown
```

rust/biogpu-sys/src/lib.rs:

```rust
#![allow(non_camel_case_types, non_upper_case_globals)]
use std::os::raw::{c_char, c_int, c_void};

#[repr(C)]
pub struct bg_ctx {
    _private: [u8; 0],
}
#[repr(C)]
pub struct bg_fm {
    _private: [u8; 0],
}

pub const BG_OK: c_int = 0;
pub const BG_ERR_INVALID_ARG: c_int = -1;
pub const BG_ERR_NO_DEVICE: c_int = -2;
pub const BG_ERR_HIP: c_int = -3;
pub const BG_ERR_OOM: c_int = -4;
pub const BG_ERR_SENTINEL: c_int = -5;
pub const BG_ERR_POSITIVE_PENALTY: c_int = -6;
pub const BG_ERR_OUT_OF_ALPHABET: c_int = -7;
pub const BG_ERR_TOO_LARGE: c_int = -8;
pub const BG_ERR_OPS_CAP: c_int = -9;
pub const BG_ERR_TRACEBACK: c_int = -10;
pub const BG_ERR_UNSUPPORTED: c_int = -11;
pub const BG_ERR_IO: c_int = -12;
// ... 78 lines not shown

#[repr(C)]
#[derive(Clone, Copy)]
pub struct bg_seed_params_t {
    pub seed_len: u32,
    pub stride: u32,
    pub max_occ: u32,
    pub pad: u32,
}

#[repr(C)]
#[derive(Clone, Copy)]
pub struct bg_seed_hit_t {
    pub aln: bg_alignment_t,
    pub window_start: u64,
    pub ref_start: u64,
    pub ref_end: u64,
    pub n_candidates: u32,
    pub n_seed_hits: u32,
}

#[repr(C)]
#[derive(Clone, Copy)]
pub struct bg_pair_params_t {
    pub min_span: u32,
    pub max_span: u32,
    pub pen_unpaired: i32,
}

#[repr(C)]
#[derive(Clone, Copy)]
pub struct bg_pair_hit_t {
    pub span: u64,
    pub n_proper: u32,
    pub proper: u8,
    pub reserved: [u8; 3],
}

#[repr(C)]
#[derive(Clone, Copy)]
pub struct bg_fastq_record_t {
    pub id_off: u64,
    pub desc_off: u64,
    pub seq_off: u64,
    pub qual_off: u64,
    pub id_len: u32,
    pub desc_len: u32,
    pub seq_len: u32,
    pub qual_len: u32,
    pub has_desc: i32,
    pub check: i32,
}

#[repr(C)]
#[derive(Clone, Copy)]
pub struct bg_timing_t {
    pub fill_ms: f32,
    pub traceback_ms: f32,
    pub fm_ms: f32,
    pub fill_launches: u32,
    pub traceback_launches: u32,
    pub fm_launches: u32,
}

#[link(name = "biogpu")]
extern "C" {
    pub fn bg_device_count() -> c_int;
    pub fn bg_init(device: c_int, out: *mut *mut bg_ctx) -> c_int;
    pub fn bg_free(ctx: *mut bg_ctx) -> c_int;
    pub fn bg_strerror(status: c_int) -> *const c_char;
    pub fn bg_last_error() -> *const c_char;
    pub fn bg_set_option(ctx: *mut bg_ctx, key: *const c_char, value: i64) -> c_int;
    pub fn bg_suffix_array(text: *const u8, n: u64, sa_out: *mut u64) -> c_int;
    pub fn bg_bwt(text: *const u8, sa: *const u64, n: u64, bwt_out: *mut u8) -> c_int;
    pub fn bg_less(bwt: *const u8, n: u64, alphabet: *const u8, n_sym: u32, less_out: *mut u64, less_len: *mut u32) -> c_int;
    pub fn bg_suffix_array_dev(ctx: *mut bg_ctx, d_text: *const u8, n: u64, d_sa: *mut u32, stream: *mut c_void) -> c_int;
    pub fn bg_bwt_dev(ctx: *mut bg_ctx, d_text: *const u8, d_sa: *const u32, n: u64, d_bwt: *mut u8, stream: *mut c_void) -> c_int;
    pub fn bg_sa_sample_dev(ctx: *mut bg_ctx, d_sa: *const u32, d_bwt: *const u8, n: u64, sampling_rate: u32, sentinel: u8, sample: *mut u64, extra_rows: *mut u64, extra_pos: *mut u64, extra_cap: u64, n_extra: *mut u64, stream: *mut c_void) -> c_int;
    pub fn bg_suffix_array_dev64(ctx: *mut bg_ctx, d_text: *const u8, n: u64, d_sa: *mut u64, stream: *mut c_void) -> c_int;
    pub fn bg_bwt_dev64(ctx: *mut bg_ctx, d_text: *const u8, d_sa: *const u64, n: u64, d_bwt: *mut u8, stream: *mut c_void) -> c_int;
    pub fn bg_sa_sample_dev64(ctx: *mut bg_ctx, d_sa: *const u64, d_bwt: *const u8, n: u64, sampling_rate: u32, sentinel: u8, sample: *mut u64, extra_rows: *mut u64, extra_pos: *mut u64, extra_cap: u64, n_extra: *mut u64, stream: *mut c_void) -> c_int;
    pub fn bg_fm_build(ctx: *mut bg_ctx, bwt: *const u8, n: u64, less: *const u64, less_len: u32, occ_k: u32, alphabet: *const u8, n_sym: u32, out: *mut *mut bg_fm) -> c_int;
    pub fn bg_fm_build_dev(ctx: *mut bg_ctx, d_bwt: *const u8, n: u64, occ_k: u32, alphabet: *const u8, n_sym: u32, less_out: *mut u64, out: *mut *mut bg_fm, stream: *mut c_void) -> c_int;
    pub fn bg_fm_free(fm: *mut bg_fm) -> c_int;
    pub fn bg_fm_device_bytes(fm: *const bg_fm) -> u64;
    pub fn bg_fm_save(fm: *const bg_fm, path: *const c_char) -> c_int;
    pub fn bg_fm_load(ctx: *mut bg_ctx, path: *const c_char, out: *mut *mut bg_fm) -> c_int;
    pub fn bg_fm_len(fm: *const bg_fm, n: *mut u64) -> c_int;
    pub fn bg_fm_less(fm: *const bg_fm, less_out: *mut u64, less_len: *mut u32) -> c_int;
    pub fn bg_fm_bwt(fm: *const bg_fm, bwt: *mut u8) -> c_int;
    pub fn bg_fm_bwt_dev(fm: *const bg_fm, d_bwt: *mut u8, stream: *mut c_void) -> c_int;
    pub fn bg_fm_step2_bytes(fm: *const bg_fm) -> u64;
    pub fn bg_fm_set_option(fm: *mut bg_fm, key: *const c_char, value: i64) -> c_int;
    pub fn bg_fm_backward_search_batch(fm: *mut bg_fm, n_q: u64, pat: *const u8, pat_off: *const u64, tag: *mut u8, lower: *mut u64, upper: *mut u64, matched_len: *mut u32) -> c_int;
    pub fn bg_fm_backward_search_batch_dev(fm: *mut bg_fm, n_q: u64, d_pat: *const u8, d_pat_off: *const u64, d_tag: *mut u8, d_lower: *mut u64, d_upper: *mut u64, d_matched_len: *mut u32, stream: *mut c_void) -> c_int;
    pub fn bg_pack2_dev(ctx: *mut bg_ctx, d_bytes: *const u8, n: u64, codes: *const u8, d_packed: *mut u32, d_n_invalid: *mut u64, stream: *mut c_void) -> c_int;
    pub fn bg_unpack2_dev(ctx: *mut bg_ctx, d_packed: *const u32, n: u64, codes: *const u8, d_bytes: *mut u8, stream: *mut c_void) -> c_int;
    pub fn bg_pack2_host(bytes: *const u8, n: u64, codes: *const u8, packed: *mut u32) -> c_int;
    pub fn bg_fm_pattern_codes(fm: *const bg_fm, codes: *mut u8) -> c_int;
    pub fn bg_fm_backward_search_packed_dev(fm: *mut bg_fm, n_q: u64, d_packed: *const u32, d_sym_off: *const u64, d_tag: *mut u8, d_lower: *mut u64, d_upper: *mut u64, d_matched_len: *mut u32, stream: *mut c_void) -> c_int;
    pub fn bg_fm_backward_search_count_lines_dev(fm: *mut bg_fm, n_q: u64, d_pat: *const u8, d_pat_off: *const u64, d_tag: *mut u8, d_lower: *mut u64, d_upper: *mut u64, d_matched_len: *mut u32, lines_out: *mut u64, stream: *mut c_void) -> c_int;
    pub fn bg_fm_set_suffix_array(fm: *mut bg_fm, sa: *const u64, n: u64) -> c_int;
    pub fn bg_fm_set_sampled_suffix_array(fm: *mut bg_fm, sample: *const u64, n_sample: u64, sampling_rate: u32, sentinel: u8, extra_rows: *const u64, extra_pos: *const u64, n_extra: u64) -> c_int;
    pub fn bg_sa_get_batch(fm: *mut bg_fm, n_idx: u64, index: *const u64, pos: *mut u64) -> c_int;
    pub fn bg_sa_get_batch_dev(fm: *mut bg_fm, n_idx: u64, d_index: *const u64, d_pos: *mut u64, stream: *mut c_void) -> c_int;
    pub fn bg_interval_occ_batch(fm: *mut bg_fm, n_iv: u64, lower: *const u64, upper: *const u64, out_off: *mut u64, pos: *mut u64, pos_cap: u64) -> c_int;
    pub fn bg_interval_occ_batch_dev(fm: *mut bg_fm, n_iv: u64, d_lower: *const u64, d_out_off: *const u64, total: u64, d_pos: *mut u64, stream: *mut c_void) -> c_int;
    pub fn bg_fmd_smems_batch(fm: *mut bg_fm, all: c_int, n_p: u64, pat: *const u8, pat_off: *const u64, i_pos: *const u32, min_len: u32, cap: u32, count: *mut u32, out: *mut u32) -> c_int;
    pub fn bg_fmd_interval_batch(fm: *mut bg_fm, n_req: u64, op: *const u8, iv_in: *const u32, sym: *const u8, iv_out: *mut u32) -> c_int;
    pub fn bg_fmd_smems_batch_dev(fm: *mut bg_fm, all: c_int, n_p: u64, d_pat: *const u8, d_pat_off: *const u64, d_i_pos: *const u32, min_len: u32, max_pattern_len: u32, cap: u32, d_count: *mut u32, d_out: *mut u32, stream: *mut c_void) -> c_int;
    pub fn bg_fmd_smems_batch64(fm: *mut bg_fm, all: c_int, n_p: u64, pat: *const u8, pat_off: *const u64, i_pos: *const u32, min_len: u32, cap: u32, count: *mut u32, out: *mut u64) -> c_int;
    pub fn bg_fmd_interval_batch64(fm: *mut bg_fm, n_req: u64, op: *const u8, iv_in: *const u64, sym: *const u8, iv_out: *mut u64) -> c_int;
    pub fn bg_fmd_smems_batch64_dev(fm: *mut bg_fm, all: c_int, n_p: u64, d_pat: *const u8, d_pat_off: *const u64, d_i_pos: *const u32, min_len: u32, max_pattern_len: u32, cap: u32, d_count: *mut u32, d_out: *mut u64, stream: *mut c_void) -> c_int;
    pub fn bg_align_batch(ctx: *mut bg_ctx, sc: *const bg_scoring_t, mode: c_int, n_pairs: u64, x: *const u8, x_off: *const u64, y: *const u8, y_off: *const u64, out: *mut bg_alignment_t, ops_buf: *mut u8, ops_cap: u64, ops_used: *mut u64) -> c_int;
    pub fn bg_align_batch_dev(ctx: *mut bg_ctx, sc: *const bg_scoring_t, mode: c_int, n_pairs: u64, d_x: *const u8, d_x_off: *const u64, d_y: *const u8, d_y_off: *const u64, max_xlen: u32, max_ylen: u32, d_out: *mut bg_alignment_t, d_ops: *mut u8, ops_stride: u64, stream: *mut c_void) -> c_int;
    pub fn bg_align_batch_packed_dev(ctx: *mut bg_ctx, sc: *const bg_scoring_t, mode: c_int, n_pairs: u64, d_x: *const u32, d_x_off: *const u64, d_y: *const u32, d_y_off: *const u64, codes: *const u8, max_xlen: u32, max_ylen: u32, d_out: *mut bg_alignment_t, d_ops: *mut u8, ops_stride: u64, stream: *mut c_void) -> c_int;
    pub fn bg_align_banded_batch(ctx: *mut bg_ctx, sc: *const bg_scoring_t, mode: c_int, k: u32, w: u32, n_pairs: u64, x: *const u8, x_off: *const u64, y: *const u8, y_off: *const u64, out: *mut bg_alignment_t, ops_buf: *mut u8, ops_cap: u64, ops_used: *mut u64, band_cells: *mut u64) -> c_int;
    pub fn bg_align_banded_batch_dev(ctx: *mut bg_ctx, sc: *const bg_scoring_t, mode: c_int, k: u32, w: u32, n_pairs: u64, d_x: *const u8, d_x_off: *const u64, d_y: *const u8, d_y_off: *const u64, d_out: *mut bg_alignment_t, d_ops: *mut u8, ops_stride: u64, band_cells: *mut u64, stream: *mut c_void) -> c_int;
    pub fn bg_band_create_batch(sc: *const bg_scoring_t, mode: c_int, k: u32, w: u32, n_pairs: u64, x: *const u8, x_off: *const u64, y: *const u8, y_off: *const u64, band_off: *const u64, start: *mut u32, end: *mut u32, band_cells: *mut u64) -> c_int;
    pub fn bg_align_banded_bands_batch(ctx: *mut bg_ctx, sc: *const bg_scoring_t, mode: c_int, n_pairs: u64, x: *const u8, x_off: *const u64, y: *const u8, y_off: *const u64, band_off: *const u64, band_start: *const u32, band_end: *const u32, out: *mut bg_alignment_t, ops_buf: *mut u8, ops_cap: u64, ops_used: *mut u64, band_cells: *mut u64) -> c_int;
    pub fn bg_band_from_matches_batch(sc: *const bg_scoring_t, mode: c_int, k: u32, w: u32, n_pairs: u64, x_off: *const u64, y_off: *const u64, matches_xy: *const u32, match_off: *const u64, path: *const u32, path_off: *const u64, band_off: *const u64, start: *mut u32, end: *mut u32, band_cells: *mut u64) -> c_int;
    pub fn bg_sparse_find_kmer_matches(x: *const u8, m: u64, y: *const u8, n: u64, k: u32, out_xy: *mut u32, cap: u64) -> u64;
    pub fn bg_sparse_sdpkpp(matches_xy: *const u32, n_matches: u64, k: u32, match_score: u32, gap_open: i32, gap_extend: i32, path: *mut u32, cap: u64) -> u64;
    pub fn bg_sparse_lcskpp(matches_xy: *const u32, n_matches: u64, k: u32, path: *mut u32, cap: u64, score: *mut u32) -> u64;
    pub fn bg_sparse_sdpkpp_union_lcskpp_path(matches_xy: *const u32, n_matches: u64, k: u32, match_score: u32, gap_open: i32, gap_extend: i32, path: *mut u32, cap: u64) -> u64;
    pub fn bg_sparse_expand_kmer_matches(x: *const u8, m: u64, y: *const u8, n: u64, k: u32, matches_xy: *const u32, n_matches: u64, allowed_mismatches: u32, out_xy: *mut u32, cap: u64) -> u64;
    pub fn bg_fm_set_text(fm: *mut bg_fm, text: *const u8, n: u64) -> c_int;
    pub fn bg_fm_set_text_dev(fm: *mut bg_fm, d_text: *const u8, n: u64) -> c_int;
    pub fn bg_seed_extend_batch(fm: *mut bg_fm, sc: *const bg_scoring_t, prm: *const bg_seed_params_t, n_reads: u64, reads: *const u8, read_off: *const u64, hits: *mut bg_seed_hit_t, ops_buf: *mut u8, ops_cap: u64, ops_used: *mut u64) -> c_int;
    pub fn bg_seed_extend_batch_dev(fm: *mut bg_fm, sc: *const bg_scoring_t, prm: *const bg_seed_params_t, n_reads: u64, d_reads: *const u8, d_read_off: *const u64, max_read_len: u32, d_hits: *mut bg_seed_hit_t, d_ops: *mut u8, ops_stride: u64, totals: *mut u64, stream: *mut c_void) -> c_int;
    pub fn bg_seed_extend_strands_batch(fm: *mut bg_fm, sc: *const bg_scoring_t, prm: *const bg_seed_params_t, strands: u32, n_reads: u64, reads: *const u8, read_off: *const u64, hits: *mut bg_seed_hit_t, strand: *mut u8, ops_buf: *mut u8, ops_cap: u64, ops_used: *mut u64) -> c_int;
    pub fn bg_seed_extend_strands_batch_dev(fm: *mut bg_fm, sc: *const bg_scoring_t, prm: *const bg_seed_params_t, strands: u32, n_reads: u64, d_reads: *const u8, d_read_off: *const u64, max_read_len: u32, d_hits: *mut bg_seed_hit_t, d_strand: *mut u8, d_ops: *mut u8, ops_stride: u64, totals: *mut u64, stream: *mut c_void) -> c_int;
    pub fn bg_seed_extend_pairs_batch(fm: *mut bg_fm, sc: *const bg_scoring_t, prm: *const bg_seed_params_t, pp: *const bg_pair_params_t, n_pairs: u64, reads: *const u8, read_off: *const u64, hits: *mut bg_seed_hit_t, strand: *mut u8, pairs: *mut bg_pair_hit_t, ops_buf: *mut u8, ops_cap: u64, ops_used: *mut u64) -> c_int;
    pub fn bg_seed_extend_pairs_batch_dev(fm: *mut bg_fm, sc: *const bg_scoring_t, prm: *const bg_seed_params_t, pp: *const bg_pair_params_t, n_pairs: u64, d_reads: *const u8, d_read_off: *const u64, max_read_len: u32, d_hits: *mut bg_seed_hit_t, d_strand: *mut u8, d_pairs: *mut bg_pair_hit_t, d_ops: *mut u8, ops_stride: u64, totals: *mut u64, stream: *mut c_void) -> c_int;
    pub fn bg_revcomp_batch_dev(ctx: *mut bg_ctx, n: u64, d_in: *const u8, d_off: *const u64, d_out: *mut u8, stream: *mut c_void) -> c_int;
    pub fn bg_fastq_parse(ctx: *mut bg_ctx, text: *const u8, len: u64, recs: *mut bg_fastq_record_t, rec_cap: u64, seq: *mut u8, seq_off: *mut u64, qual: *mut u8, qual_off: *mut u64, n_records: *mut u64, status: *mut i32, err_pos: *mut u64) -> c_int;
    pub fn bg_fastq_parse_dev(ctx: *mut bg_ctx, d_text: *const u8, len: u64, d_recs: *mut bg_fastq_record_t, rec_cap: u64, d_seq: *mut u8, d_seq_off: *mut u64, d_qual: *mut u8, d_qual_off: *mut u64, n_records: *mut u64, status: *mut i32, err_pos: *mut u64, stream: *mut c_void) -> c_int;
    pub fn bg_cigar_batch(ctx: *mut bg_ctx, n: u64, aln: *const bg_alignment_t, ops: *const u8, ops_bytes: u64, hard_clip: c_int, out: *mut c_char, out_cap: u64, out_off: *mut u64) -> c_int;
    pub fn bg_cigar_batch_dev(ctx: *mut bg_ctx, n: u64, d_aln: *const bg_alignment_t, d_ops: *const u8, hard_clip: c_int, d_out: *mut c_char, stride: u64, d_len: *mut i32, stream: *mut c_void) -> c_int;
    pub fn bg_pretty_batch(ctx: *mut bg_ctx, n: u64, aln: *const bg_alignment_t, ops: *const u8, ops_bytes: u64, x: *const u8, x_off: *const u64, y: *const u8, y_off: *const u64, ncol: u32, out: *mut c_char, out_cap: u64, out_off: *mut u64) -> c_int;
    pub fn bg_shard_range(n_units: u64, rank: c_int, world: c_int, lo: *mut u64, hi: *mut u64) -> c_int;
    pub fn bg_shard_balanced(costs: *const u64, n: u64, world: c_int, bounds: *mut u64) -> c_int;
    pub fn bg_comm_unique_id(id: *mut u8) -> c_int;
    pub fn bg_comm_init(ctx: *mut bg_ctx, rank: c_int, world: c_int, id: *const u8, out: *mut *mut bg_comm) -> c_int;
    pub fn bg_comm_init_host(ctx: *mut bg_ctx, rank: c_int, world: c_int, name: *const c_char, out: *mut *mut bg_comm) -> c_int;
    pub fn bg_gather_records(comm: *mut bg_comm, local: *const c_void, n_local: u64, rec_bytes: u32, all: *mut c_void, counts_out: *mut u64, stream: *mut c_void) -> c_int;
    pub fn bg_gather_records_cap(comm: *mut bg_comm, local: *const c_void, n_local: u64, rec_bytes: u32, all: *mut c_void, all_cap: u64, counts_out: *mut u64, stream: *mut c_void) -> c_int;
    pub fn bg_gather_records_host(comm: *mut bg_comm, local: *const c_void, n_local: u64, rec_bytes: u32, all: *mut c_void, all_cap: u64, counts_out: *mut u64) -> c_int;
    pub fn bg_comm_world(comm: *mut bg_comm, info: *mut i64) -> c_int;
    pub fn bg_comm_free(comm: *mut bg_comm) -> c_int;
    pub fn bg_get_timing(ctx: *mut bg_ctx, out: *mut bg_timing_t) -> c_int;
    pub fn bg_band_redo_pairs(ctx: *mut bg_ctx, out: *mut u64) -> c_int;
    pub fn bg_last_fill_kernels(ctx: *mut bg_ctx, mask: *mut u32) -> c_int;
    pub fn bg_enable_timing(ctx: *mut bg_ctx, on: c_int) -> c_int;
}
```

Measured before the change: 2112 GCUPS.

## Add framed offset variant of pk16 local-fast SW fill to drop saturating adds

```diff
diff --git a/include/biogpu.h b/include/biogpu.h
--- a/include/biogpu.h
+++ b/include/biogpu.h
@@ -319,6 +319,7 @@
     BG_FILL_K3P = 0x200
 };
 int bg_last_fill_kernels(bg_ctx* ctx, uint32_t* mask);
+int bg_last_fill_framed(bg_ctx* ctx, int* framed);
 int bg_enable_timing(bg_ctx* ctx, int on);
 
 #ifdef __cplusplus
diff --git a/rust-bio_amd/_lib.py b/rust-bio_amd/_lib.py
--- a/rust-bio_amd/_lib.py
+++ b/rust-bio_amd/_lib.py
@@ -98,7 +98,7 @@
            "bg_align_batch", "bg_align_batch_dev", "bg_align_banded_batch", "bg_align_banded_batch_dev", "bg_band_create_batch",
            "bg_align_banded_bands_batch", "bg_band_from_matches_batch", "bg_sparse_find_kmer_matches", "bg_sparse_sdpkpp",
            "bg_sparse_lcskpp", "bg_sparse_sdpkpp_union_lcskpp_path", "bg_sparse_expand_kmer_matches", "bg_fastq_parse",
-           "bg_fastq_parse_dev", "bg_cigar_batch", "bg_cigar_batch_dev", "bg_get_timing", "bg_enable_timing", "bg_band_redo_pairs", "bg_last_fill_kernels", "bg_pack2_host",
+           "bg_fastq_parse_dev", "bg_cigar_batch", "bg_cigar_batch_dev", "bg_get_timing", "bg_enable_timing", "bg_band_redo_pairs", "bg_last_fill_kernels", "bg_last_fill_framed", "bg_pack2_host",
            "bg_pretty_batch", "bg_suffix_array_dev", "bg_bwt_dev", "bg_sa_sample_dev", "bg_suffix_array_dev64", "bg_bwt_dev64", "bg_sa_sample_dev64", "bg_fm_build_dev", "bg_fm_set_text", "bg_fm_set_text_dev", "bg_seed_extend_batch", "bg_seed_extend_batch_dev",
            "bg_seed_extend_strands_batch", "bg_seed_extend_strands_batch_dev", "bg_revcomp_batch_dev",
            "bg_seed_extend_pairs_batch", "bg_seed_extend_pairs_batch_dev",
@@ -229,6 +229,7 @@
         L.bg_enable_timing.argtypes = [vp, i32]
         L.bg_band_redo_pairs.argtypes = [vp, C.POINTER(u64)]
         L.bg_last_fill_kernels.argtypes = [vp, C.POINTER(u32)]
+        L.bg_last_fill_framed.argtypes = [vp, C.POINTER(i32)]
         L.bg_pack2_host.argtypes = [vp, u64, vp, vp]
         for s in SYMBOLS:
             if getattr(L, s).restype is C.c_int or s.startswith("bg_") and getattr(L, s).restype is None:
@@ -265,6 +266,11 @@
         check(lib().bg_last_fill_kernels(self.h, C.byref(v)))
         return int(v.value)
 
+    def last_fill_framed(self):
+        v = C.c_int(0)
+        check(lib().bg_last_fill_framed(self.h, C.byref(v)))
+        return bool(v.value)
+
     def close(self):
         if self.h:
             lib().bg_free(self.h)
diff --git a/rust-bio_amd/csrc/banded_api.hip b/rust-bio_amd/csrc/banded_api.hip
--- a/rust-bio_amd/csrc/banded_api.hip
+++ b/rust-bio_amd/csrc/banded_api.hip
@@ -283,6 +283,7 @@
                              const BandMaker& make_band, const uint32_t* dev_kw = nullptr, const BandDevIO* dio = nullptr) {
     if (!ctx || !sc || mode < BG_MODE_CUSTOM || mode > BG_MODE_LOCAL) return BG_ERR_INVALID_ARG;
     ctx->fill_mask = 0;
+    ctx->fill_framed = false;
     int rc = check_scoring(sc);
     if (rc) return rc;
     if (ops_used) *ops_used = 0;
diff --git a/rust-bio_amd/csrc/bg_common.h b/rust-bio_amd/csrc/bg_common.h
--- a/rust-bio_amd/csrc/bg_common.h
+++ b/rust-bio_amd/csrc/bg_common.h
@@ -67,6 +67,7 @@
     bool force_wide = false;
     bool no_pk16 = false;
     bool no_local_fast = false;
+    bool no_pk16_frame = false;
     bool no_couples = false;
     int band_chain_global = -1;
     bool fq_no_fused = false;
@@ -86,6 +87,7 @@
     hipEvent_t ev[2] = {nullptr, nullptr};
     bg_timing_t last = {};
     uint32_t fill_mask = 0;
+    bool fill_framed = false;
 };
 
 int bg_reserve(void** p, size_t* cur, size_t need);
diff --git a/rust-bio_amd/csrc/core.hip b/rust-bio_amd/csrc/core.hip
--- a/rust-bio_amd/csrc/core.hip
+++ b/rust-bio_amd/csrc/core.hip
@@ -261,6 +261,10 @@
         ctx->no_local_fast = value != 0;
         return BG_OK;
     }
+    if (!strcmp(key, "no_pk16_frame")) {
+        ctx->no_pk16_frame = value != 0;
+        return BG_OK;
+    }
     if (!strcmp(key, "no_pk16")) {
         ctx->no_pk16 = value != 0;
         return BG_OK;
@@ -282,6 +286,12 @@
 extern "C" int bg_last_fill_kernels(bg_ctx* ctx, uint32_t* mask) {
     if (!ctx || !mask) return BG_ERR_INVALID_ARG;
     *mask = ctx->fill_mask;
+    return BG_OK;
+}
+
+extern "C" int bg_last_fill_framed(bg_ctx* ctx, int* framed) {
+    if (!ctx || !framed) return BG_ERR_INVALID_ARG;
+    *framed = ctx->fill_framed ? 1 : 0;
     return BG_OK;
 }
 
diff --git a/rust-bio_amd/csrc/sw_api.hip b/rust-bio_amd/csrc/sw_api.hip
--- a/rust-bio_amd/csrc/sw_api.hip
+++ b/rust-bio_amd/csrc/sw_api.hip
@@ -17,6 +17,7 @@
 sw_fill_fn get_fill_matrix(int lp, int r, int sm, bool narrow, bool local);
 sw_fill_fn get_fill_pk16_local(int lp, int r, int which);
 sw_fill_fn get_fill_pk16_localfast(int lp, int r, int which);
+sw_fill_fn get_fill_pk16_localframe(int lp, int r, int which);
 sw_fill_fn get_fill_pk16_semiglobal(int lp, int r, int which);
 sw_fill_fn get_fill_pk16_global(int lp, int r, int which);
 sw_fill_fn get_fill_pk16_custom(int lp, int r, int which);
@@ -318,6 +319,10 @@
             pk16 = false;
         } else {
             cfg.r = r_pick;
+            if (local_fast && !ctx->no_pk16_frame && pk16_frame_fits(c, max_ylen, cfg.r, cfg.lp)) {
+                getter = get_fill_pk16_localframe;
+                ctx->fill_framed = true;
+            }
             fill = getter(cfg.lp, cfg.r, 0);
             fill_rest = local_fast ? nullptr : getter(cfg.lp, cfg.r, 1);
             fill_second = getter(cfg.lp, cfg.r, 2);
@@ -452,7 +457,10 @@
                                   const uint64_t* d_y_off, uint32_t max_xlen, uint32_t max_ylen,
                                   bg_alignment_t* d_out, uint8_t* d_ops, uint64_t ops_stride,
                                   void* stream) {
-    if (ctx) ctx->fill_mask = 0;
+    if (ctx) {
+        ctx->fill_mask = 0;
+        ctx->fill_framed = false;
+    }
     return align_batch_dev_impl(ctx, sc, mode, n_pairs, d_x, d_x_off, d_y, d_y_off, max_xlen, max_ylen, d_out, d_ops, ops_stride, stream, -1);
 }
 
@@ -464,7 +472,10 @@
     for (int a = 0; a < 4; a++)
         for (int b = a + 1; b < 4; b++)
             if (codes[a] == codes[b]) return BG_ERR_INVALID_ARG;
-    if (ctx) ctx->fill_mask = 0;
+    if (ctx) {
+        ctx->fill_mask = 0;
+        ctx->fill_framed = false;
+    }
     return align_batch_dev_impl(ctx, sc, mode, n_pairs, (const uint8_t*)d_x, d_x_off, (const uint8_t*)d_y, d_y_off, max_xlen, max_ylen,
                                 d_out, d_ops, ops_stride, stream, -1, codes);
 }
@@ -762,6 +773,7 @@
                               uint64_t ops_cap, uint64_t* ops_used) {
     if (!ctx || !sc) return BG_ERR_INVALID_ARG;
     ctx->fill_mask = 0;
+    ctx->fill_framed = false;
     int rc = check_scoring(sc);
     if (rc) return rc;
     if (ops_used) *ops_used = 0;
diff --git a/rust-bio_amd/csrc/sw_fill_pk16.inc b/rust-bio_amd/csrc/sw_fill_pk16.inc
--- a/rust-bio_amd/csrc/sw_fill_pk16.inc
+++ b/rust-bio_amd/csrc/sw_fill_pk16.inc
@@ -40,7 +40,7 @@
 constexpr int32_t kFloor16 = -2048;
 
 enum { CZ = 0, CF = 1, CI = 2 };
-template <int R, int LP, int MODE, int XP, int XS, int YP, int YS, bool LF = false>
+template <int R, int LP, int MODE, int XP, int XS, int YP, int YS, bool LF = false, bool FR = false>
 __device__ __forceinline__ void sw_fill_pk16_body(const SwArgs& a) {
     constexpr bool FAST = MODE == 0;
     constexpr int PW = 64 / LP;
@@ -54,6 +54,7 @@
     static_assert(LP == 16 || LP == 32, "lanes per pair");
     static_assert(R >= 1 && R <= 12, "rows per lane");
     static_assert(!LF || LOCAL, "LF is a flavour of the local kernel");
+    static_assert(!FR || LF, "the frame is a cell of the LF flavour");
     (void)NARROW;
     (void)LOCAL;
     constexpr int kTileStride = 20;
@@ -84,6 +85,13 @@
     (void)XS16; (void)YS16; (void)XSCAP; (void)YSCAP;
     const pk MISC = dup16(-((sc.mismatch * 16) | K_SUBST));
     (void)MISC;
+    auto fr = [](int32_t c) -> pk { return (uint32_t)c * 0x10001u; };
+    const int32_t gF = -16 * sc.ge, BF = pk16_frame_bias(sc);
+    const pk GF = fr(gF);
+    const pk KGOI = fr(sc.go * 16 + K_INS + 1 + gF), KGOD = fr(sc.go * 16 + K_DEL + 1 + gF);
+    const pk KSUB = fr(((sc.mismatch * 16) | K_SUBST) + 2 * gF);
+    const pk KREB = fr(gF * (R - 1));
+    (void)GF; (void)KGOI; (void)KGOD; (void)KSUB; (void)KREB;
     pk C16 = dup16(16), C32 = dup16(32), C1024 = dup16(1024);
     asm volatile("" : "+s"(C16), "+s"(C32), "+s"(C1024));
 
@@ -201,6 +209,17 @@
             }
         }
         pk diag0 = dup16((pair_ok && rb < m) ? scl(col0_S(sc, rb, m, fold0)) : NEGS);
+        if (FR) {
+            const int32_t off0 = BF + gF * ((int32_t)ll - 1);
+#pragma unroll
+            for (int r = 0; r < R; r++) {
+                const pk o = fr(off0 + gF * r);
+                Sl[r] = (pair_ok && rb + r + 1 <= m) ? Sl[r] + o : o;
+                Il[r] += o;
+                Dl[r] = 0;
+            }
+            diag0 = fr(off0 - gF) + ((pair_ok && rb < m) ? dup16(scl(col0_S(sc, rb, m, fold0))) : 0u);
+        }
 
         pk S_out = FLOORK, I_out = FLOORK, cm_out = FLOORK, ca_out = 0, q_out = 0;
         pk ychunk = 0, ychunk_nx = 0;
@@ -251,6 +270,10 @@
                 if (pair_ok && nb < n) ychunk_nx = y_pair(nb);
             }
             pk S_up = (pk)wave_shr1((int)S_out, (int)S_out), I_up = (pk)wave_shr1((int)I_out, (int)I_out);
+            if (FR) {
+                S_up -= KREB;
+                I_up -= KREB;
+            }
             pk cm = FLOORK, ca = 0;
             if (FOLD) {
                 cm = (pk)wave_shr1((int)cm_out, (int)cm_out);
@@ -259,10 +282,12 @@
             pk q = (pk)wave_shr1((int)q_out, (int)q_out);
             const uint32_t j = s + 1 - (uint32_t)ll;
             const bool col_ok = ALLON || (pair_ok && (j - 1) < n);
+            const pk F0 = fr(BF + gF * (int32_t)s);
+            (void)F0;
             if (ll == 0) {
                 q = ychunk;
-                S_up = 0;
-                I_up = FLOORK;
+                S_up = FR ? F0 - GF : 0u;
+                I_up = FR ? 0u : FLOORK;
                 cm = FLOORK;
                 ca = 0;
                 if (!ROW0_ZERO && col_ok) {
@@ -299,9 +324,13 @@
                         const bool maybe_m = MRk < 0 || r == MRk;
                         const bool is_m = MRk < 0 ? (r == mrow) : (r == MRk && mrow == MRk);
                         const pk e = pk_subs_u16(ONE, px[r] ^ q);
-                        const pk m_key = LF ? pk_subs_u16(pk_mad_u16(e, DELTA, diag), MISC) : pk_adds(diag, pk_mad_u16(e, DELTA, MISK));
-                        const pk Iv_t = pk_max(pk_adds(I_up, GE), pk_adds(S_up, GOT_I));
-                        const pk Dv_t = pk_max(pk_adds(Dl[r], GE), pk_adds(Sl[r], GOT_D));
+                        const pk Fr = F0 + (uint32_t)r * GF;
+                        (void)Fr;
+                        const pk m_key = FR   ? pk_max(pk_mad_u16(e, DELTA, diag) + KSUB, Fr)
+                                         : LF ? pk_subs_u16(pk_mad_u16(e, DELTA, diag), MISC)
+                                              : pk_adds(diag, pk_mad_u16(e, DELTA, MISK));
+                        const pk Iv_t = FR ? pk_max(I_up, S_up + KGOI) : pk_max(pk_adds(I_up, GE), pk_adds(S_up, GOT_I));
+                        const pk Dv_t = FR ? pk_max(Dl[r], Sl[r] + KGOD) : pk_max(pk_adds(Dl[r], GE), pk_adds(Sl[r], GOT_D));
                         const pk Iv = Iv_t & NOFLAG, Dv = Dv_t & NOFLAG;
                         pk kb = pk_max(m_key, Dv_t);
                         if (XP != CI && !LF) kb = pk_max(kb, XKEY);
@@ -322,7 +351,7 @@
                         }
                         if (YS != CI) {
                             const pk t1 = YS == CZ ? best : pk_min(pk_adds(best, YS16), YSCAP);
-                            SnB[r] = pk_max(SnB[r], t1 | sprio);
+                            SnB[r] = pk_max(SnB[r], FR ? best - (Fr - sprio) : t1 | sprio);
                         }
                         const pk c5 = pk_mad_u16(Dv_t & ONE, C16, (kb & 0x000e000eu) | (Iv_t & ONE));
                         if (r % 3 == 0)
@@ -409,10 +438,11 @@
         if (YS != CI && nsteps_w) merge_rows((nsteps_w - 1) & ~15u);
 
         pk* park = wave_lds + lane;
+        const pk offl = FR ? fr(BF + gF * ((int32_t)ll + (int32_t)n - 1)) : 0u;
 #pragma unroll
         for (int r = 0; r < R; r++) {
-            park[(0 * R + r) * 64] = Sl[r];
-            park[(1 * R + r) * 64] = Il[r];
+            park[(0 * R + r) * 64] = FR ? Sl[r] - (offl + (uint32_t)r * GF) : Sl[r];
+            park[(1 * R + r) * 64] = FR ? Il[r] - (offl + (uint32_t)r * GF) : Il[r];
             park[(2 * R + r) * 64] = SnR[r];
             park[(3 * R + r) * 64] = Ly[r];
         }
@@ -468,17 +498,17 @@
     do_pass(MODE == 2 ? 1 : 0);
 }
 
-template <int R, int LP, int XP, int XS, int YP, int YS, bool LF>
+template <int R, int LP, int XP, int XS, int YP, int YS, bool LF, bool FR = false>
 __global__ __launch_bounds__(256) __attribute__((amdgpu_waves_per_eu(R <= 10 ? 3 : 2, R <= 10 ? 3 : 2))) void sw_fill_pk16_kernel(const SwArgs a) {
-    sw_fill_pk16_body<R, LP, 0, XP, XS, YP, YS, LF>(a);
-}
-template <int R, int LP, int XP, int XS, int YP, int YS, bool LF>
+    sw_fill_pk16_body<R, LP, 0, XP, XS, YP, YS, LF, FR>(a);
+}
+template <int R, int LP, int XP, int XS, int YP, int YS, bool LF, bool FR = false>
 __global__ __launch_bounds__(256) __attribute__((amdgpu_waves_per_eu(R <= 10 ? 3 : 2, R <= 10 ? 3 : 2))) void sw_fill_pk16_rest_kernel(const SwArgs a) {
-    sw_fill_pk16_body<R, LP, 1, XP, XS, YP, YS, LF>(a);
-}
-template <int R, int LP, int XP, int XS, int YP, int YS, bool LF>
+    sw_fill_pk16_body<R, LP, 1, XP, XS, YP, YS, LF, FR>(a);
+}
+template <int R, int LP, int XP, int XS, int YP, int YS, bool LF, bool FR = false>
 __global__ __launch_bounds__(256) __attribute__((amdgpu_waves_per_eu(R <= 10 ? 3 : 2, R <= 10 ? 3 : 2))) void sw_fill_pk16_second_kernel(const SwArgs a) {
-    sw_fill_pk16_body<R, LP, 2, XP, XS, YP, YS, LF>(a);
+    sw_fill_pk16_body<R, LP, 2, XP, XS, YP, YS, LF, FR>(a);
 }
 
 }
@@ -486,6 +516,6 @@
 
 #define BG_PK16_CASE(LP_, R_)                                                                          \
     if (lp == LP_ && r == R_)                                                                         \
-        return which == 0   ? pk16::sw_fill_pk16_kernel<R_, LP_, XP_, XS_, YP_, YS_, LF_>             \
-               : which == 1 ? pk16::sw_fill_pk16_rest_kernel<R_, LP_, XP_, XS_, YP_, YS_, LF_>        \
-                            : pk16::sw_fill_pk16_second_kernel<R_, LP_, XP_, XS_, YP_, YS_, LF_>;
+        return which == 0   ? pk16::sw_fill_pk16_kernel<R_, LP_, XP_, XS_, YP_, YS_, LF_, FR_>        \
+               : which == 1 ? pk16::sw_fill_pk16_rest_kernel<R_, LP_, XP_, XS_, YP_, YS_, LF_, FR_>   \
+                            : pk16::sw_fill_pk16_second_kernel<R_, LP_, XP_, XS_, YP_, YS_, LF_, FR_>;
diff --git a/rust-bio_amd/csrc/sw_fill_pk16_custom.hip b/rust-bio_amd/csrc/sw_fill_pk16_custom.hip
--- a/rust-bio_amd/csrc/sw_fill_pk16_custom.hip
+++ b/rust-bio_amd/csrc/sw_fill_pk16_custom.hip
@@ -2,7 +2,7 @@
 namespace bgsw {
 sw_fill_fn get_fill_pk16_custom(int lp, int r, int which) {
     constexpr int XP_ = pk16::CF, XS_ = pk16::CF, YP_ = pk16::CF, YS_ = pk16::CF;
-    constexpr bool LF_ = false;
+    constexpr bool LF_ = false, FR_ = false;
     BG_PK16_CASE(16, 2) BG_PK16_CASE(16, 4) BG_PK16_CASE(16, 5) BG_PK16_CASE(16, 6) BG_PK16_CASE(16, 8) BG_PK16_CASE(16, 10) BG_PK16_CASE(16, 12)
     BG_PK16_CASE(32, 8) BG_PK16_CASE(32, 10) BG_PK16_CASE(32, 12)
     return nullptr;
diff --git a/rust-bio_amd/csrc/sw_fill_pk16_global.hip b/rust-bio_amd/csrc/sw_fill_pk16_global.hip
--- a/rust-bio_amd/csrc/sw_fill_pk16_global.hip
+++ b/rust-bio_amd/csrc/sw_fill_pk16_global.hip
@@ -2,7 +2,7 @@
 namespace bgsw {
 sw_fill_fn get_fill_pk16_global(int lp, int r, int which) {
     constexpr int XP_ = pk16::CI, XS_ = pk16::CI, YP_ = pk16::CI, YS_ = pk16::CI;
-    constexpr bool LF_ = false;
+    constexpr bool LF_ = false, FR_ = false;
     BG_PK16_CASE(16, 2) BG_PK16_CASE(16, 4) BG_PK16_CASE(16, 5) BG_PK16_CASE(16, 6) BG_PK16_CASE(16, 8) BG_PK16_CASE(16, 10) BG_PK16_CASE(16, 12)
     BG_PK16_CASE(32, 8) BG_PK16_CASE(32, 10) BG_PK16_CASE(32, 12)
     return nullptr;
diff --git a/rust-bio_amd/csrc/sw_fill_pk16_local.hip b/rust-bio_amd/csrc/sw_fill_pk16_local.hip
--- a/rust-bio_amd/csrc/sw_fill_pk16_local.hip
+++ b/rust-bio_amd/csrc/sw_fill_pk16_local.hip
@@ -2,7 +2,7 @@
 namespace bgsw {
 sw_fill_fn get_fill_pk16_local(int lp, int r, int which) {
     constexpr int XP_ = pk16::CZ, XS_ = pk16::CZ, YP_ = pk16::CZ, YS_ = pk16::CZ;
-    constexpr bool LF_ = false;
+    constexpr bool LF_ = false, FR_ = false;
     BG_PK16_CASE(16, 2) BG_PK16_CASE(16, 3) BG_PK16_CASE(16, 4) BG_PK16_CASE(16, 5) BG_PK16_CASE(16, 6) BG_PK16_CASE(16, 7)
     BG_PK16_CASE(16, 8) BG_PK16_CASE(16, 9) BG_PK16_CASE(16, 10) BG_PK16_CASE(16, 11) BG_PK16_CASE(16, 12)
     BG_PK16_CASE(32, 7) BG_PK16_CASE(32, 8) BG_PK16_CASE(32, 9) BG_PK16_CASE(32, 10) BG_PK16_CASE(32, 11) BG_PK16_CASE(32, 12)
diff --git a/rust-bio_amd/csrc/sw_fill_pk16_localfast.hip b/rust-bio_amd/csrc/sw_fill_pk16_localfast.hip
--- a/rust-bio_amd/csrc/sw_fill_pk16_localfast.hip
+++ b/rust-bio_amd/csrc/sw_fill_pk16_localfast.hip
@@ -1,11 +1,19 @@
 #include "sw_fill_pk16.inc"
 namespace bgsw {
+#define BG_PK16_LF_CASES                                                                                                    \
+    BG_PK16_CASE(16, 2) BG_PK16_CASE(16, 3) BG_PK16_CASE(16, 4) BG_PK16_CASE(16, 5) BG_PK16_CASE(16, 6) BG_PK16_CASE(16, 7) \
+    BG_PK16_CASE(16, 8) BG_PK16_CASE(16, 9) BG_PK16_CASE(16, 10) BG_PK16_CASE(16, 11) BG_PK16_CASE(16, 12)                  \
+    BG_PK16_CASE(32, 7) BG_PK16_CASE(32, 8) BG_PK16_CASE(32, 9) BG_PK16_CASE(32, 10) BG_PK16_CASE(32, 11) BG_PK16_CASE(32, 12)
 sw_fill_fn get_fill_pk16_localfast(int lp, int r, int which) {
     constexpr int XP_ = pk16::CZ, XS_ = pk16::CZ, YP_ = pk16::CZ, YS_ = pk16::CZ;
-    constexpr bool LF_ = true;
-    BG_PK16_CASE(16, 2) BG_PK16_CASE(16, 3) BG_PK16_CASE(16, 4) BG_PK16_CASE(16, 5) BG_PK16_CASE(16, 6) BG_PK16_CASE(16, 7)
-    BG_PK16_CASE(16, 8) BG_PK16_CASE(16, 9) BG_PK16_CASE(16, 10) BG_PK16_CASE(16, 11) BG_PK16_CASE(16, 12)
-    BG_PK16_CASE(32, 7) BG_PK16_CASE(32, 8) BG_PK16_CASE(32, 9) BG_PK16_CASE(32, 10) BG_PK16_CASE(32, 11) BG_PK16_CASE(32, 12)
+    constexpr bool LF_ = true, FR_ = false;
+    BG_PK16_LF_CASES
+    return nullptr;
+}
+sw_fill_fn get_fill_pk16_localframe(int lp, int r, int which) {
+    constexpr int XP_ = pk16::CZ, XS_ = pk16::CZ, YP_ = pk16::CZ, YS_ = pk16::CZ;
+    constexpr bool LF_ = true, FR_ = true;
+    BG_PK16_LF_CASES
     return nullptr;
 }
 }
diff --git a/rust-bio_amd/csrc/sw_fill_pk16_semiglobal.hip b/rust-bio_amd/csrc/sw_fill_pk16_semiglobal.hip
--- a/rust-bio_amd/csrc/sw_fill_pk16_semiglobal.hip
+++ b/rust-bio_amd/csrc/sw_fill_pk16_semiglobal.hip
@@ -2,7 +2,7 @@
 namespace bgsw {
 sw_fill_fn get_fill_pk16_semiglobal(int lp, int r, int which) {
     constexpr int XP_ = pk16::CI, XS_ = pk16::CI, YP_ = pk16::CZ, YS_ = pk16::CZ;
-    constexpr bool LF_ = false;
+    constexpr bool LF_ = false, FR_ = false;
     BG_PK16_CASE(16, 2) BG_PK16_CASE(16, 4) BG_PK16_CASE(16, 5) BG_PK16_CASE(16, 6) BG_PK16_CASE(16, 8) BG_PK16_CASE(16, 10) BG_PK16_CASE(16, 12)
     BG_PK16_CASE(32, 8) BG_PK16_CASE(32, 10) BG_PK16_CASE(32, 12)
     return nullptr;
diff --git a/rust-bio_amd/csrc/sw_kernels.h b/rust-bio_amd/csrc/sw_kernels.h
--- a/rust-bio_amd/csrc/sw_kernels.h
+++ b/rust-bio_amd/csrc/sw_kernels.h
@@ -23,6 +23,20 @@
     int32_t go, ge, xp, xs, yp, ys;
     int32_t match, mismatch;
 };
+
+__host__ __device__ inline int32_t pk16_frame_bias(const SwScoring& sc) {
+    const int32_t g = -16 * sc.ge;
+    int32_t b = 2 * g;
+    const int32_t lows[3] = {-((sc.mismatch * 16) | (int32_t)(C_SUBST << 1)), -(sc.go * 16 + (int32_t)(C_INS << 1)),
+                             -(sc.go * 16 + (int32_t)(C_DEL << 1))};
+    for (int32_t v : lows) b = b > v ? b : v;
+    return (b + 15) & ~15;
+}
+inline bool pk16_frame_fits(const SwScoring& sc, uint32_t max_ylen, int r, int lp) {
+    if (sc.ge > 0 || sc.match < 0) return false;
+    const int64_t g = -16ll * sc.ge, nsteps = (int64_t)max_ylen + lp - 1;
+    return 16ll * sc.match * max_ylen + pk16_frame_bias(sc) + g * (r + nsteps) + 15 < 0x8000;
+}
 
 struct SwGeom {
     uint32_t lp, r, nsteps, nstrips, m_cap, n_cap, aux_stride;
diff --git a/rust/biogpu-sys/src/lib.rs b/rust/biogpu-sys/src/lib.rs
--- a/rust/biogpu-sys/src/lib.rs
+++ b/rust/biogpu-sys/src/lib.rs
@@ -254,5 +254,6 @@
     pub fn bg_get_timing(ctx: *mut bg_ctx, out: *mut bg_timing_t) -> c_int;
     pub fn bg_band_redo_pairs(ctx: *mut bg_ctx, out: *mut u64) -> c_int;
     pub fn bg_last_fill_kernels(ctx: *mut bg_ctx, mask: *mut u32) -> c_int;
+    pub fn bg_last_fill_framed(ctx: *mut bg_ctx, framed: *mut c_int) -> c_int;
     pub fn bg_enable_timing(ctx: *mut bg_ctx, on: c_int) -> c_int;
 }
```

Result: faster. 2150 GCUPS (median of 6 runs) (+1.8%).
